# jianfenglihg/Unsupervised_depth_OpticalFlow_egomotion

Measured on AMD Instinct MI355X. Metric: frame-pairs/sec (832x256, geom mode), higher is better.
Workload: dtype f32; 1 GPU; train_step: mode=geom, 832x256, batch=4/GPU, num_scales=3, fwd+bwd+Adam; global_batch=4, parallelism=dp1, hw_queues=4, stream_priorities=auto

## Files before the change

include/dfe_hip.h:

```cpp
#ifndef DFE_HIP_H
#define DFE_HIP_H

#ifdef __cplusplus
extern "C" {
#endif

#define DFE_OK 0
#define DFE_ERR_NULL (-1)
#define DFE_ERR_DIMS (-2)
#define DFE_ERR_LAUNCH (-3)
#define DFE_ERR_UNSUPPORTED (-4)
#define DFE_ERR_WORKSPACE (-5)

#define DFE_MAX_SCALES 8
#define DFE_ABI_VERSION 3

int dfe_abi_version(void);
const char* dfe_error_string(int code);

int dfe_camera_floats(void);
int dfe_prepare_cameras(const float* pose, const float* K, float* cams, int B, int ndir, int nscale,
                        const float* downscale_host, void* stream);

int dfe_pose_vec2mat_fwd(const float* vec, float* T34, float* E, int n, void* stream);
int dfe_pose_vec2mat_bwd(const float* vec, const float* gT34, const float* gE, float* gvec, int n, void* stream);

int dfe_adam_chunk(void);
int dfe_adam_step(const void* table, const int* blockmap, int nblocks, double lr, double beta1, double beta2, double eps,
                  double bias_correction1, double bias_correction2, void* stream);
int dfe_adam_step_dev(const void* table, const int* blockmap, int nblocks, double lr, double beta1, double beta2, double eps,
                      double* step_count, float* coef, void* stream);

long dfe_scatter_ws_bytes(long n);

int dfe_warp_flow_fwd(const float* x, const float* flow, float* out, int B, int C, int H, int W, int use_mask,
                      int align_corners, void* stream);
int dfe_warp_flow_bwd(const float* x, const float* flow, const float* gout, float* gflow, float* gx, void* gx_ws, int B,
                      int C, int H, int W, int use_mask, int align_corners, void* stream);

int dfe_pose_partials_floats(int B, int H, int W);
int dfe_inverse_warp2_fwd(const float* img, const float* depth, const float* ref_depth, const float* cams,
                          float* out_img, float* out_valid, float* out_pdepth, float* out_cdepth, int B, int H, int W,
                          int align_corners, void* stream);
int dfe_inverse_warp2_bwd(const float* img, const float* depth, const float* ref_depth, const float* cams,
                          const float* g_img, const float* g_pdepth, const float* g_cdepth, float* g_depth,
                          float* g_refdepth, void* g_refdepth_ws, float* g_pose, float* partials, int B, int H, int W,
                          int align_corners, void* stream);

int dfe_rigid_flow_fwd(const float* depth, const float* cams, float* out, int B, int H, int W, void* stream);
int dfe_rigid_flow_bwd(const float* depth, const float* cams, const float* gout, float* g_depth, float* g_pose,
                       float* partials, int B, int H, int W, void* stream);

int dfe_occ_masks(const float* from_l, const float* tgt, const float* from_r, float* occ_bwd, float* occ_fwd,
                  float* valid_bwd, float* valid_fwd, int B, int H, int W, void* stream);
int dfe_texture_mask(const float* img, const float* warped, const float* source, float* out, int B, int H, int W,
                     void* stream);
int dfe_dynamic_mask(const float* flow, const float* rigid, float* mask, float* score, float alpha, float beta, int B,
                     int H, int W, void* stream);

int dfe_prepare_triplets(const unsigned char* in_u8, const unsigned char* flip, float* out, int B, int H0, int W0,
                         int H, int W, void* stream);

typedef struct {
  long long offset;
  int h0, w0;
  int xtab, ytab;
  int flip, pad;
} dfe_u8_desc;
// ... 68 lines not shown
                        void* stream);
int dfe_planeconv_wgrad(const float* gy, const float* x, float* gweight, float* ws, int B, int Ci, int Co, int H, int W,
                        void* stream);

long dfe_wino_weight_floats(int Ci, int Co);
long dfe_wino_scratch_floats(int B, int Ci, int Co, int H, int W, int P);
int dfe_wino_conv3x3(const float* x, const float* weight, float* y, long y_batch_stride, float* wbuf, long wbuf_floats, int B, int Ci,
                     int Co, int H, int W, int P, int transposed_weight, void* stream);
long dfe_wino_wgrad_floats(int B, int Ci, int Co, int H, int W, int P);
int dfe_wino_wgrad_tune(int tile, int blocks1, int blocks2, int chunk);
int dfe_wino_wgrad3x3(const float* x, long x_batch_stride, const float* gy, long gy_batch_stride, float* gweight, float* ws, int B,
                      int Ci, int Co, int H, int W, int P, void* stream);
int dfe_sconv_tune(int blocks, int rows);
long dfe_sconv_wgrad_floats(int B, int Ci, int Co, int H, int W, int K, int stride, int P);
int dfe_sconv_wgrad(const float* x, long x_batch_stride, const float* gy, long gy_batch_stride, float* gweight, float* ws, int B,
                    int Ci, int Co, int H, int W, int K, int stride, int P, void* stream);
int dfe_wino_conv3x3_dilated(const float* x, const float* weight, float* y, long y_batch_stride, float* wbuf, int B, int Ci, int Co,
                             int H, int W, int dilation, int transposed_weight, void* stream);
long dfe_wino_transform_blocks(int Ci, int Co);
int dfe_wino_transform_weights_multi(const long* table, const int* blockmap, int n_blocks, void* stream);
int dfe_wino_conv3x3_u(const float* x, const float* U, float* y, long y_batch_stride, float* part, long part_floats, int B, int Ci,
                       int Co, int H, int W, int P, int dilation, void* stream);
int dfe_wino_conv3x3_u_act(const float* x, const float* U, const float* bias, float slope, float* y, long y_batch_stride, float* y2,
                           long y2_batch_stride, float* part, long part_floats, int B, int Ci, int Co, int H, int W, int P,
                           int dilation, void* stream);

int dfe_conv1x1_small_supported(int B, int Ci, int Co, int H, int W);
int dfe_conv1x1_small_fwd(const float* x, const float* weight, const float* bias, float slope, float* y, int B, int Ci, int Co,
                          int H, int W, void* stream);
int dfe_conv1x1_small_bwd(const float* gy, const float* x, const float* weight, float* gx, float* gweight, int B, int Ci, int Co,
                          int H, int W, void* stream);

long dfe_bn_partials_floats(int G, int Bg, int C, int H, int W);
int dfe_bn_fwd(const float* x, const float* residual, const float* weight, const float* bias, float* running_mean,
               float* running_var, float* y, float* save_mean, float* save_invstd, float* partials, int G, int Bg, int C,
               int H, int W, float eps, float momentum, int relu, void* stream);
int dfe_bn_bwd(const float* x, const float* y, const float* gy, const float* weight, const float* save_mean,
               const float* save_invstd, float* gx, float* gres, float* gweight, float* gbias, float* partials,
               float* scratch_means, int G, int Bg, int C, int H, int W, int relu, void* stream);

long dfe_bias_act_partials_floats(int B, int C, int H, int W);
int dfe_bias_act_fwd(float* z, const float* bias, int B, int C, int H, int W, float slope, void* stream);
int dfe_bias_act_bwd(const float* y, const float* gy, long gy_batch_stride, float* gz, float* gbias, float* partials,
                     int B, int C, int H, int W, float slope, void* stream);

int dfe_bias_act_fwd2(const float* z, const float* bias, float* dst1, long dst1_batch_stride, float* dst2,
                      long dst2_batch_stride, int B, int C, int H, int W, float slope, void* stream);
int dfe_bias_act_bwd2(const float* y, long y_batch_stride, const float* g1, long g1_batch_stride, const float* g2,
                      long g2_batch_stride, float* gz, float* gbias, float* partials, int B, int C, int H, int W,
                      float slope, void* stream);
int dfe_bias_grad_final_multi(const float* const* partials, float* const* gbias, const int* C, int n, int B, int H, int W,
                              void* stream);

#define DFE_LOSS_DEPTH_PIXEL 0
#define DFE_LOSS_DEPTH_SMOOTH 1
#define DFE_LOSS_FLOW_PIXEL 2
#define DFE_LOSS_FLOW_SSIM 3
#define DFE_LOSS_FLOW_SMOOTH 4
#define DFE_LOSS_FLOW_CONSIS 5
#define DFE_LOSS_DEPTH_FLOW_CONSIS 6
#define DFE_LOSS_EPIPOLAR 7
#define DFE_LOSS_DEPTH_SSIM 8
#define DFE_LOSS_DEPTH_CONSIS 9
#define DFE_NUM_LOSSES 10
#define DFE_DEPTH_TERM_SSIM 1
#define DFE_DEPTH_TERM_CONSIS 2

#define DFE_MASK_VALID_BWD 0x01
#define DFE_MASK_VALID_FWD 0x02
#define DFE_MASK_OCC_BWD 0x04
#define DFE_MASK_OCC_FWD 0x08
#define DFE_MASK_DYNA_BWD 0x10
#define DFE_MASK_DYNA_FWD 0x20
#define DFE_MASK_TEX_BWD 0x40
#define DFE_MASK_TEX_FWD 0x80

typedef struct dfe_geom_args {
  int B, H, W;
  int num_scales;
  int align_corners;
  int mode;
  float alpha, beta;
  const float* img[3];
  const float* disp[3][DFE_MAX_SCALES];
  const float* flow[2][DFE_MAX_SCALES];
  const float* pose;
  const float* K;
  const float* K_inv;
  float* workspace;
  long workspace_floats;
  float* losses;
  const float* grad_losses;
  float* grad_disp[3][DFE_MAX_SCALES];
  float* grad_flow[2][DFE_MAX_SCALES];
  float* grad_pose;
  int depth_terms;
} dfe_geom_args;

long dfe_geom_workspace_floats(const dfe_geom_args* args);
long dfe_geom_maskpack_offset_bytes(const dfe_geom_args* args, int scale);
int dfe_geom_loss_fwd(const dfe_geom_args* args, void* stream);
int dfe_geom_loss_bwd(const dfe_geom_args* args, void* stream);

#define DFE_GEOM_FWD_SEGMENTS 7
#define DFE_GEOM_BWD_SEGMENTS 6
int dfe_geom_loss_fwd_profiled(const dfe_geom_args* args, void* stream, float* ms_host);
// ... 11 lines not shown
```

unsupervised_depth_opticalflow_egomotion_amd/_lib.py:

```python
from __future__ import annotations

import ctypes
import os
import re
import threading

import torch

_HERE = os.path.dirname(os.path.abspath(__file__))
LIB_PATH = os.environ.get("DFE_HIP_LIB") or os.path.join(_HERE, "libdfe_hip.so")
HEADER_PATH = os.path.join(os.path.dirname(_HERE), "include", "dfe_hip.h")

_lib = None
_lock = threading.Lock()

_P = ctypes.c_void_p
_I = ctypes.c_int

_SIGNATURES = {
    "dfe_abi_version": [],
    "dfe_error_string": [_I],
    "dfe_camera_floats": [],
    "dfe_prepare_cameras": [_P, _P, _P, _I, _I, _I, _P, _P],
    "dfe_pose_vec2mat_fwd": [_P, _P, _P, _I, _P],
    "dfe_pose_vec2mat_bwd": [_P, _P, _P, _P, _I, _P],
    "dfe_warp_flow_fwd": [_P, _P, _P, _I, _I, _I, _I, _I, _I, _P],
    "dfe_scatter_ws_bytes": [ctypes.c_long],
    "dfe_adam_chunk": [],
    "dfe_adam_step": [_P, _P, _I, ctypes.c_double, ctypes.c_double, ctypes.c_double, ctypes.c_double, ctypes.c_double, ctypes.c_double, _P],
    "dfe_adam_step_dev": [_P, _P, _I, ctypes.c_double, ctypes.c_double, ctypes.c_double, ctypes.c_double, _P, _P, _P],
    "dfe_warp_flow_bwd": [_P, _P, _P, _P, _P, _P, _I, _I, _I, _I, _I, _I, _P],
    "dfe_pose_partials_floats": [_I, _I, _I],
    "dfe_inverse_warp2_fwd": [_P, _P, _P, _P, _P, _P, _P, _P, _I, _I, _I, _I, _P],
    "dfe_inverse_warp2_bwd": [_P, _P, _P, _P, _P, _P, _P, _P, _P, _P, _P, _P, _I, _I, _I, _I, _P],
    "dfe_wgrad3x3_partials_floats": [_I, _I, _I, _I, _I],
    "dfe_wgrad3x3_fwd": [_P, _P, _P, _P, _I, _I, _I, _I, _I, _P],
    "dfe_wino_weight_floats": [_I, _I],
    "dfe_wino_conv3x3": [_P, _P, _P, ctypes.c_long, _P, ctypes.c_long, _I, _I, _I, _I, _I, _I, _I, _P],
    "dfe_wino_scratch_floats": [_I, _I, _I, _I, _I, _I],
    "dfe_wino_wgrad_floats": [_I, _I, _I, _I, _I, _I],
    "dfe_wino_wgrad_tune": [_I, _I, _I, _I],
    "dfe_sconv_tune": [_I, _I],
    "dfe_sconv_wgrad_floats": [_I, _I, _I, _I, _I, _I, _I, _I],
    "dfe_sconv_wgrad": [_P, ctypes.c_long, _P, ctypes.c_long, _P, _P, _I, _I, _I, _I, _I, _I, _I, _I, _P],
    "dfe_wino_wgrad3x3": [_P, ctypes.c_long, _P, ctypes.c_long, _P, _P, _I, _I, _I, _I, _I, _I, _P],
    "dfe_wino_conv3x3_dilated": [_P, _P, _P, ctypes.c_long, _P, _I, _I, _I, _I, _I, _I, _I, _P],
    "dfe_wino_transform_blocks": [_I, _I],
    "dfe_wino_transform_weights_multi": [_P, _P, _I, _P],
    "dfe_wino_conv3x3_u": [_P, _P, _P, ctypes.c_long, _P, ctypes.c_long, _I, _I, _I, _I, _I, _I, _I, _P],
    "dfe_wino_conv3x3_u_act": [_P, _P, _P, ctypes.c_float, _P, ctypes.c_long, _P, ctypes.c_long, _P, ctypes.c_long, _I, _I, _I, _I, _I, _I, _I, _P],
    "dfe_conv1x1_small_supported": [_I, _I, _I, _I, _I],
    "dfe_conv1x1_small_fwd": [_P, _P, _P, ctypes.c_float, _P, _I, _I, _I, _I, _I, _P],
    "dfe_conv1x1_small_bwd": [_P, _P, _P, _P, _P, _I, _I, _I, _I, _I, _P],
    "dfe_planeconv_supported": [_I, _I, _I, _I, _I],
    "dfe_planeconv_ws_floats": [_I, _I, _I, _I, _I],
    "dfe_planeconv_fwd": [_P, _P, _P, ctypes.c_float, _P, ctypes.c_long, _P, ctypes.c_long, _P, _I, _I, _I, _I, _I, _P],
    "dfe_planeconv_dgrad": [_P, _P, _P, _P, _I, _I, _I, _I, _I, _P],
    "dfe_planeconv_wgrad": [_P, _P, _P, _P, _I, _I, _I, _I, _I, _P],
    "dfe_disp_head_partials_floats": [_I, _I, _I, _I],
    "dfe_disp_head_fwd": [_P, _P, _P, _P, _I, _I, _I, _I, _P],
    "dfe_disp_head_bwd": [_P, _P, _P, _P, _P, _P, _P, _P, _I, _I, _I, _I, _P],
    "dfe_flow_head_partials_floats": [_I, _I, _I, _I],
    "dfe_flow_head_fwd": [_P, _P, _P, _P, _I, _I, _I, _I, _P],
    "dfe_flow_head_bwd": [_P, _P, _P, _P, _P, _P, _P, _I, _I, _I, _I, _P],
    "dfe_bn_partials_floats": [_I, _I, _I, _I, _I],
    "dfe_bn_fwd": [_P] * 10 + [_I] * 5 + [ctypes.c_float, ctypes.c_float, _I, _P],
    "dfe_bn_bwd": [_P] * 12 + [_I] * 6 + [_P],
    "dfe_bias_act_partials_floats": [_I, _I, _I, _I],
    "dfe_bias_act_fwd": [_P, _P, _I, _I, _I, _I, ctypes.c_float, _P],
    "dfe_bias_act_bwd": [_P, _P, ctypes.c_long, _P, _P, _P, _I, _I, _I, _I, ctypes.c_float, _P],
    "dfe_bias_act_fwd2": [_P, _P, _P, ctypes.c_long, _P, ctypes.c_long, _I, _I, _I, _I, ctypes.c_float, _P],
    "dfe_bias_act_bwd2": [_P, ctypes.c_long, _P, ctypes.c_long, _P, ctypes.c_long, _P, _P, _P, _I, _I, _I, _I, ctypes.c_float, _P],
    "dfe_bias_grad_final_multi": [_P, _P, _P, _I, _I, _I, _I, _P],
    "dfe_glue_partials_floats": [_I, _I, _I, _I],
    "dfe_elu_pad_fwd": [_P, _P, _P, _I, _I, _I, _I, _I, _P],
    "dfe_elu_pad_bwd": [_P, _P, _P, _P, _P, _P, _I, _I, _I, _I, _I, _P],
    "dfe_elu_up2_cat_pad_fwd": [_P, _P, _P, _P, _I, _I, _I, _I, _I, _P],
    "dfe_elu_up2_cat_pad_bwd": [_P, _P, _P, _P, _P, _P, _P, _I, _I, _I, _I, _I, _P],
    "dfe_rigid_flow_fwd": [_P, _P, _P, _I, _I, _I, _P],
    "dfe_rigid_flow_bwd": [_P, _P, _P, _P, _P, _P, _I, _I, _I, _P],
    "dfe_occ_masks": [_P] * 7 + [_I, _I, _I, _P],
    "dfe_texture_mask": [_P, _P, _P, _P, _I, _I, _I, _P],
    "dfe_dynamic_mask": [_P, _P, _P, _P, ctypes.c_float, ctypes.c_float, _I, _I, _I, _P],
    "dfe_exact_math_selftest": [_P, ctypes.c_ulonglong, _P],
    "dfe_prepare_triplets": [_P, _P, _P, _I, _I, _I, _I, _I, _P],
    "dfe_prepare_triplets_u8": [_P, _P, _P, _P, _P, _P, _I, _I, _I, _I, _I, _P],
    "dfe_forward_splat_ones": [_P, _P, _P, _I, _I, _I, _I, _P],
    "dfe_ssim_fwd": [_P, _P, _P, _I, _I, _I, _I, _P],
    "dfe_ssim_bwd": [_P, _P, _P, _P, _P, _I, _I, _I, _I, _P],
    "dfe_corr_fwd": [_P, _P, _P, _I, _I, _I, _I, _I, _P],
    "dfe_corr_bwd": [_P, _P, _P, _P, _P, _I, _I, _I, _I, _I, _P],
    "dfe_maxpool3x3s2_out": [_I],
    "dfe_maxpool3x3s2_fwd": [_P, _P, _P, _I, _I, _I, _P],
    "dfe_maxpool3x3s2_bwd": [_P, _P, _P, _I, _I, _I, _P],
    "dfe_pwc_level_channels": [_I],
    "dfe_pwc_level_fwd": [_P, _P, _P, _P, _P, _I, _I, _I, _I, _I, _P],
    "dfe_pwc_level_bwd": [_P, _P, _P, _P, _P, _P, _P, _P, _P, _P, _I, _I, _I, _I, _I, _P],
    "dfe_pwc_level_map_bytes": [_I, _I, _I],
    "dfe_pwc_level_fwd_map": [_P, _P, _P, _P, _P, _P, _I, _I, _I, _I, _I, _P],
    "dfe_pwc_level_bwd_map": [_P, _P, _P, _P, _P, _P, _P, _P, _P, _P, _I, _I, _I, _I, _I, _P],
    "dfe_resize": [_P, _P, _I, _I, _I, _I, _I, _I, _P],
    "dfe_resize_bilinear_fwd": [_P, _P, _I, _I, _I, _I, _I, ctypes.c_float, _I, _P],
    "dfe_resize_bilinear_bwd": [_P, _P, _I, _I, _I, _I, _I, ctypes.c_float, _I, _P],
    "dfe_geom_workspace_floats": [_P],
    "dfe_geom_maskpack_offset_bytes": [_P, _I],
    "dfe_geom_loss_fwd": [_P, _P],
    "dfe_geom_loss_bwd": [_P, _P],
    "dfe_geom_loss_fwd_profiled": [_P, _P, _P],
    "dfe_geom_loss_bwd_profiled": [_P, _P, _P],
    "dfe_geom_loss_fwd_timed": [_P, _P, _P],
    "dfe_geom_loss_bwd_timed": [_P, _P, _P],
    "dfe_geom_timed_collect": [_P, _P],
}
_RESTYPES = {"dfe_error_string": ctypes.c_char_p, "dfe_geom_workspace_floats": ctypes.c_long,
             "dfe_bias_act_partials_floats": ctypes.c_long, "dfe_glue_partials_floats": ctypes.c_long,
             "dfe_bn_partials_floats": ctypes.c_long, "dfe_disp_head_partials_floats": ctypes.c_long,
             "dfe_flow_head_partials_floats": ctypes.c_long, "dfe_pwc_level_map_bytes": ctypes.c_long,
             "dfe_wgrad3x3_partials_floats": ctypes.c_long, "dfe_planeconv_ws_floats": ctypes.c_long, "dfe_wino_weight_floats": ctypes.c_long, "dfe_wino_scratch_floats": ctypes.c_long, "dfe_wino_wgrad_floats": ctypes.c_long, "dfe_sconv_wgrad_floats": ctypes.c_long, "dfe_wino_transform_blocks": ctypes.c_long,
             "dfe_geom_maskpack_offset_bytes": ctypes.c_long, "dfe_scatter_ws_bytes": ctypes.c_long}


class DfeError(RuntimeError):
    pass


def header_symbols(path: str = HEADER_PATH):
    with open(path) as fh:
        text = re.sub(r"/\*.*?\*/", "", fh.read(), flags=re.S)
    return sorted(set(re.findall(r"\b(dfe_[a-z0-9_]+)\s*\(", text)))


def header_abi_version(path: str = HEADER_PATH) -> int:
    with open(path) as fh:
        return int(re.search(r"#define\s+DFE_ABI_VERSION\s+(\d+)", fh.read()).group(1))


def get_lib():
    global _lib
    if _lib is not None:
        return _lib
    with _lock:
        if _lib is None:
            if not os.path.exists(LIB_PATH):
                raise DfeError(
                    "libdfe_hip.so not found at %s: build it with `python -c 'import __graft_entry__ as g; "
                    "g.build()'` (hipcc --offload-arch=gfx950). There is no CPU fallback." % LIB_PATH)
            lib = ctypes.CDLL(LIB_PATH)
            for name in header_symbols():
                fn = getattr(lib, name)
                if name in _SIGNATURES:
                    fn.argtypes = _SIGNATURES[name]
                fn.restype = _RESTYPES.get(name, ctypes.c_int)
            if lib.dfe_abi_version() != header_abi_version():
                raise DfeError("libdfe_hip.so ABI version %d != include/dfe_hip.h's DFE_ABI_VERSION %d: a stale build; "
                               "rebuild with __graft_entry__.build()" % (lib.dfe_abi_version(), header_abi_version()))
            _lib = lib
    return _lib


def check(code: int, what: str = ""):
    if code != 0:
        msg = get_lib().dfe_error_string(code)
        raise DfeError("%s failed: %s (code %d)" % (what or "dfe call", msg.decode() if msg else "?", code))


def ptr(t, strided=False):
    if t is None:
        return None
    if not isinstance(t, torch.Tensor):
        raise DfeError("expected a torch.Tensor, got %r" % type(t))
    if not t.is_cuda:
        raise DfeError("the HIP loss stack only accepts tensors on a HIP device (got %s); there is no CPU "
# ... 21 lines not shown
```

unsupervised_depth_opticalflow_egomotion_amd/csrc/dfe_wgrad_sum.h:

```cpp
#pragma once
#include <hip/hip_runtime.h>

namespace dfe {

template <int SG>
__global__ void __launch_bounds__(32 * SG) k_wgrad_sum(const float* __restrict__ part, float* __restrict__ gw, int S, long n) {
  __shared__ float sm[SG][32];
  const int o = threadIdx.x & 31, g = threadIdx.x >> 5;
  const long idx = static_cast<long>(blockIdx.x) * 32 + o;
  const int per = (S + SG - 1) / SG, s0 = g * per, s1 = min(S, s0 + per);
  float s = 0.0f;
  if (idx < n)
    for (int k = s0; k < s1; ++k) s += part[k * n + idx];
  sm[g][o] = s;
  __syncthreads();
  if (g == 0 && idx < n) {
    float t = sm[0][o];
#pragma unroll
    for (int j = 1; j < SG; ++j) t += sm[j][o];
    gw[idx] = t;
  }
}

}
```

unsupervised_depth_opticalflow_egomotion_amd/csrc/ops_decoder.hip:

```cpp
#include "dfe_internal.h"
#include "dfe_device.h"
#include <hip/hip_runtime.h>
#include <cstdlib>

namespace dfe {

__device__ __forceinline__ float elu1(float v) { return v > 0.0f ? v : __expf(v) - 1.0f; }
__device__ __forceinline__ float elu1_grad(float v) { return v > 0.0f ? 1.0f : __expf(v); }
__device__ __forceinline__ int reflect1(int i, int n) { return i < 0 ? -i : (i >= n ? 2 * n - 2 - i : i); }

__device__ __forceinline__ void up2_tap(int d, int n, int& i0, int& i1, float& l0, float& l1) {
  const float s = fmaxf(0.5f * (static_cast<float>(d) + 0.5f) - 0.5f, 0.0f);
  i0 = static_cast<int>(s);
  i1 = min(i0 + 1, n - 1);
  l1 = s - static_cast<float>(i0);
  l0 = 1.0f - l1;
}

__device__ __forceinline__ float pad_adjoint(const float* __restrict__ gp, int y, int x, int H, int W) {
  const int Wp = W + 2;
  int ry[3], rx[3], ny = 1, nx = 1;
  ry[0] = y + 1; rx[0] = x + 1;
  if (y == 1) ry[ny++] = 0;
  if (y == H - 2) ry[ny++] = H + 1;
  if (x == 1) rx[nx++] = 0;
  if (x == W - 2) rx[nx++] = W + 1;
  float s = 0.0f;
  for (int a = 0; a < ny; ++a)
    for (int b = 0; b < nx; ++b) s += gp[static_cast<long>(ry[a]) * Wp + rx[b]];
  return s;
}

__global__ void __launch_bounds__(256) k_elu_pad_fwd(const float* __restrict__ x, const float* __restrict__ bias,
                                                     float* __restrict__ out, int C, int H, int W, int elu) {
  const unsigned e = blockIdx.x * blockDim.x + threadIdx.x;
  if (e >= static_cast<unsigned>((H + 2) * (W + 2))) return;
  const int oy = e / static_cast<unsigned>(W + 2), ox = e - oy * (W + 2);
  const long pl = plane_id();
  const float v = x[(pl * H + reflect1(oy - 1, H)) * W + reflect1(ox - 1, W)] + (bias ? bias[plane_id() % C] : 0.0f);
  out[(pl * (H + 2) + oy) * (W + 2) + ox] = elu ? elu1(v) : v;
}

__global__ void __launch_bounds__(256) k_elu_pad_bwd(const float* __restrict__ x, const float* __restrict__ bias,
                                                     const float* __restrict__ gp, float* __restrict__ gx,
                                                     float* __restrict__ part, int C, int H, int W, int elu) {
  __shared__ float red[4 * 4];
  const unsigned e = blockIdx.x * blockDim.x + threadIdx.x;
  float acc[1] = {0.0f};
  if (e < static_cast<unsigned>(H * W)) {
    const int iy = e / static_cast<unsigned>(W), ix = e - iy * W;
    const long pl = plane_id();
    float g = pad_adjoint(gp + pl * (H + 2) * (W + 2), iy, ix, H, W);
    const long o = (pl * H + iy) * W + ix;
    if (elu) g *= elu1_grad(x[o] + (bias ? bias[plane_id() % C] : 0.0f));
// ... 293 lines not shown
        const int xq = 2 * j0 - 1 + t;
        if (xq >= 0 && xq < W) tile[rs[k] * LW + t] = pad_adjoint(g, ys[k], xq, H, W);
      }
      if (cs[k] >= 0 && cs[k] < LW && t < LH) {
        const int y = 2 * i0 - 1 + t;
        if (y >= 0 && y < H) tile[t * LW + cs[k]] = pad_adjoint(g, y, xs[k], H, W);
      }
    }
  }
  __syncthreads();
  float wx[4] = {0.25f, 0.75f, 0.75f, 0.25f};
  if (!inner) up2_adjoint_weights(min(j, w - 1), w, wx);
  float f[2 * R + 2];
  const float* trow = tile + (2 * grp * R) * LW + 2 * jl;
#pragma unroll
  for (int rr = 0; rr < 2 * R + 2; ++rr) {
    const AF2 a = *reinterpret_cast<const AF2*>(trow + rr * LW), d = *reinterpret_cast<const AF2*>(trow + rr * LW + 2);
    if (inner) f[rr] = ((0.25f * a.a + 0.75f * a.b) + 0.75f * d.a) + 0.25f * d.b;
    else {
      float s = 0.0f;
      if (wx[0] != 0.0f) s += wx[0] * a.a;
      if (wx[1] != 0.0f) s += wx[1] * a.b;
      if (wx[2] != 0.0f) s += wx[2] * d.a;
      if (wx[3] != 0.0f) s += wx[3] * d.b;
      f[rr] = s;
    }
  }
  const float bv = bias ? bias[c] : 0.0f;
  float acc[1] = {0.0f};
#pragma unroll
  for (int q = 0; q < R; ++q) {
    const int i = i0 + grp * R + q;
    float total = 0.0f;
    if (inner) {
      total += 0.25f * f[2 * q]; total += 0.75f * f[2 * q + 1]; total += 0.75f * f[2 * q + 2]; total += 0.25f * f[2 * q + 3];
    } else {
      float wy[4];
      up2_adjoint_weights(min(i, h - 1), h, wy);
#pragma unroll
      for (int ky = 0; ky < 4; ++ky)
        if (wy[ky] != 0.0f) total += wy[ky] * f[2 * q + ky];
    }
    if (i < h && j < w) {
      const float v = total * elu1_grad(xv[q] + bv);
      gx[obase + static_cast<long>(i) * w + j] = v;
      acc[0] += v;
    }
  }
  if (part) block_sum<1>(acc, red, part + static_cast<long>(plane_id()) * gridDim.x + blockIdx.x);
}

__global__ void __launch_bounds__(64) k_glue_bias_final(const float* __restrict__ part, float* __restrict__ gbias,
                                                        int B, int C, int nblk) {
  const int c = blockIdx.x, lane = threadIdx.x;
  float s = 0.0f;
  for (int b = 0; b < B; ++b) {
    const float* p = part + (static_cast<long>(b) * C + c) * nblk;
    for (int k = lane; k < nblk; k += 64) s += p[k];
  }
  s = dpp_add<0xB1>(s); s = dpp_add<0x4E>(s); s = dpp_add<0x141>(s); s = dpp_add<0x140>(s);
  const float r0 = __int_as_float(__builtin_amdgcn_readlane(__float_as_int(s), 0));
  const float r1 = __int_as_float(__builtin_amdgcn_readlane(__float_as_int(s), 16));
  const float r2 = __int_as_float(__builtin_amdgcn_readlane(__float_as_int(s), 32));
  const float r3 = __int_as_float(__builtin_amdgcn_readlane(__float_as_int(s), 48));
  if (lane == 0) gbias[c] = (r0 + r1) + (r2 + r3);
}

__global__ void __launch_bounds__(256) k_cat_pad_bwd_skip(const float* __restrict__ gp, float* __restrict__ gskip,
                                                          int C1, int C2, int H, int W) {
  const unsigned e = blockIdx.x * blockDim.x + threadIdx.x;
  if (e >= static_cast<unsigned>(H * W)) return;
  const int iy = e / static_cast<unsigned>(W), ix = e - iy * W;
  const int b = plane_id() / C2, c = plane_id() - b * C2;
  const float* g = gp + (static_cast<long>(b) * (C1 + C2) + C1 + c) * (H + 2) * (W + 2);
  gskip[(static_cast<long>(plane_id()) * H + iy) * W + ix] = pad_adjoint(g, iy, ix, H, W);
}

}

#define DFE_LAUNCH_CHECK() do { if (hipGetLastError() != hipSuccess) return DFE_ERR_LAUNCH; } while (0)

using namespace dfe;

static inline bool grid_ok(long plane_elems, long batch, long channels) { return plane_elems < (1L << 31) && batch <= 65535 && channels <= 65535; }
static inline bool al8(const void* p) { return (reinterpret_cast<uintptr_t>(p) & 7) == 0; }
static inline bool al16(const void* p) { return (reinterpret_cast<uintptr_t>(p) & 15) == 0; }
static inline unsigned nblk(long n) { return static_cast<unsigned>((n + 255) / 256); }

extern "C" long dfe_glue_partials_floats(int B, int C, int H, int W) {
  if (B <= 0 || C <= 0 || H <= 0 || W <= 0) return 0;
  return static_cast<long>(B) * C * nblk(static_cast<long>(H) * W);
}

extern "C" int dfe_elu_pad_fwd(const float* x, const float* bias, float* out, int B, int C, int H, int W, int apply_elu,
                               void* stream) {
  if (!x || !out) return DFE_ERR_NULL;
  if (B <= 0 || C <= 0 || H < 2 || W < 2 || !grid_ok((H + 2L) * (W + 2L), B, C)) return DFE_ERR_DIMS;
  hipStream_t st = static_cast<hipStream_t>(stream);
  if (W % 2 == 0 && W >= 4 && al8(out)) k_elu_pad_fwd_pair<<<dim3(nblk((H + 2L) * ((W + 2L) / 2)), C, B), 256, 0, st>>>(x, bias, out, C, H, W, apply_elu);
  else k_elu_pad_fwd<<<dim3(nblk((H + 2L) * (W + 2L)), C, B), 256, 0, st>>>(x, bias, out, C, H, W, apply_elu);
  DFE_LAUNCH_CHECK();
  return DFE_OK;
}

extern "C" int dfe_elu_pad_bwd(const float* x, const float* bias, const float* gout, float* gx, float* gbias, float* partials,
                               int B, int C, int H, int W, int apply_elu, void* stream) {
  if (!gout || !gx || (apply_elu && !x) || (gbias && !partials)) return DFE_ERR_NULL;
  if (B <= 0 || C <= 0 || H < 2 || W < 2 || !grid_ok((H + 2L) * (W + 2L), B, C)) return DFE_ERR_DIMS;
  hipStream_t st = static_cast<hipStream_t>(stream);
  const bool pair = W % 2 == 0 && W >= 4 && al8(gx) && (!apply_elu || al8(x));
  const bool quad = W % 4 == 0 && W >= 8 && al16(gx) && (!apply_elu || al16(x));
  const unsigned nb = nblk(quad ? static_cast<long>(H) * (W / 4) : pair ? static_cast<long>(H) * (W / 2) : static_cast<long>(H) * W);
  if (quad) k_elu_pad_bwd_quad<<<dim3(nb, C, B), 256, 0, st>>>(x, bias, gout, gx, gbias ? partials : nullptr, C, H, W, apply_elu);
  else if (pair) k_elu_pad_bwd_pair<<<dim3(nb, C, B), 256, 0, st>>>(x, bias, gout, gx, gbias ? partials : nullptr, C, H, W, apply_elu);
  else k_elu_pad_bwd<<<dim3(nb, C, B), 256, 0, st>>>(x, bias, gout, gx, gbias ? partials : nullptr, C, H, W, apply_elu);
  DFE_LAUNCH_CHECK();
  if (gbias) {
    k_glue_bias_final<<<C, 64, 0, st>>>(partials, gbias, B, C, static_cast<int>(nb));
    DFE_LAUNCH_CHECK();
  }
  return DFE_OK;
}

extern "C" int dfe_elu_up2_cat_pad_fwd(const float* x, const float* bias, const float* skip, float* out, int B, int C1, int C2,
                                       int h, int w, void* stream) {
  if (!x || !out || (C2 > 0 && !skip)) return DFE_ERR_NULL;
  if (B <= 0 || C1 <= 0 || C2 < 0 || h < 1 || w < 1 || !grid_ok((2L * h + 2) * (2L * w + 2), B, C1 + C2)) return DFE_ERR_DIMS;
  hipStream_t st = static_cast<hipStream_t>(stream);
  if (w >= 2 && al8(out)) k_elu_up2_cat_pad_fwd_pair<<<dim3(nblk((2L * h + 2) * (w + 1L)), C1 + C2, B), 256, 0, st>>>(x, bias, skip, out, C1, C2, h, w);
  else k_elu_up2_cat_pad_fwd<<<dim3(nblk((2L * h + 2) * (2L * w + 2)), C1 + C2, B), 256, 0, st>>>(x, bias, skip, out, C1, C2, h, w);
  DFE_LAUNCH_CHECK();
  return DFE_OK;
}

extern "C" int dfe_elu_up2_cat_pad_bwd(const float* x, const float* bias, const float* gout, float* gx, float* gskip,
                                       float* gbias, float* partials, int B, int C1, int C2, int h, int w, void* stream) {
  if (!x || !gout || (!gx && !gskip) || (gbias && (!partials || !gx))) return DFE_ERR_NULL;
  if (B <= 0 || C1 <= 0 || C2 < 0 || h < 1 || w < 1 || !grid_ok((2L * h + 2) * (2L * w + 2), B, C1 + C2)) return DFE_ERR_DIMS;
  hipStream_t st = static_cast<hipStream_t>(stream);
  if (gx) {
    unsigned nb = nblk(static_cast<long>(h) * w);
    const int tw = w <= 32 ? 32 : 64;
    const int tiles_x = (w + tw - 1) / tw, tiles_y = (h + UT_H - 1) / UT_H;
    if (al8(gout) && static_cast<unsigned>(tiles_x * tiles_y) <= nb) {
      nb = static_cast<unsigned>(tiles_x * tiles_y);
      if (tw == 32) k_elu_up2_cat_pad_bwd_x_tile<32><<<dim3(nb, C1, B), 256, 0, st>>>(x, bias, gout, gx, gbias ? partials : nullptr, C1, C2, h, w, tiles_x);
      else k_elu_up2_cat_pad_bwd_x_tile<64><<<dim3(nb, C1, B), 256, 0, st>>>(x, bias, gout, gx, gbias ? partials : nullptr, C1, C2, h, w, tiles_x);
    } else {
      k_elu_up2_cat_pad_bwd_x<<<dim3(nb, C1, B), 256, 0, st>>>(x, bias, gout, gx, gbias ? partials : nullptr, C1, C2, h, w);
    }
    DFE_LAUNCH_CHECK();
    if (gbias) {
      k_glue_bias_final<<<C1, 64, 0, st>>>(partials, gbias, B, C1, static_cast<int>(nb));
      DFE_LAUNCH_CHECK();
    }
  }
  if (gskip && C2 > 0) {
    if (w % 2 == 0 && w >= 4 && al16(gskip)) k_cat_pad_bwd_skip_quad<<<dim3(nblk(1L * h * w), C2, B), 256, 0, st>>>(gout, gskip, C1, C2, 2 * h, 2 * w);
    else if (w >= 2 && al8(gskip)) k_cat_pad_bwd_skip_pair<<<dim3(nblk(2L * h * w), C2, B), 256, 0, st>>>(gout, gskip, C1, C2, 2 * h, 2 * w);
    else k_cat_pad_bwd_skip<<<dim3(nblk(4L * h * w), C2, B), 256, 0, st>>>(gout, gskip, C1, C2, 2 * h, 2 * w);
    DFE_LAUNCH_CHECK();
  }
  return DFE_OK;
}
```

unsupervised_depth_opticalflow_egomotion_amd/csrc/ops_disphead.hip:

```cpp
#include "dfe_internal.h"
#include "dfe_device.h"
#include <hip/hip_runtime.h>

namespace dfe {

constexpr int DH_COLS = 62;
constexpr int DH_ROWS = 16;
constexpr int DH_CI = 16;
constexpr int FH_CI = 8;


template <bool VPAD>
__device__ __forceinline__ float head_load(const float* __restrict__ pc, int r, int xx, int H, int W, bool ld) {
  if (VPAD) return (ld && r >= 1 && r <= H && xx >= 1 && xx <= W) ? pc[static_cast<long>(r - 1) * W + (xx - 1)] : 0.0f;
  return ld ? pc[static_cast<long>(r) * (W + 2) + xx] : 0.0f;
}

template <int CO, bool SIG, bool VPAD, int CI>
__global__ void __launch_bounds__(64) k_head_fwd(const float* __restrict__ p, const float* __restrict__ w,
                                                 const float* __restrict__ bias, float* __restrict__ out, int C, int H,
                                                 int W, int nstrips, int R) {
  const int lane = threadIdx.x, b = blockIdx.y;
  const int strip = blockIdx.x % nstrips, rb = blockIdx.x / nstrips;
  const int Hp = H + 2, Wp = W + 2;
  const int xx = strip * DH_COLS + lane;
  const bool ld = xx < Wp, st = lane < DH_COLS && xx < W;
  const int y0 = rb * R;
  const long plane = VPAD ? static_cast<long>(H) * W : static_cast<long>(Hp) * Wp;
  const float* pb = p + static_cast<long>(b) * C * plane;
  float acc[CO][3];
#pragma unroll
  for (int co = 0; co < CO; ++co) { acc[co][0] = 0.0f; acc[co][1] = 0.0f; acc[co][2] = 0.0f; }
  const int rend = min(y0 + R + 2, Hp);
  for (int r = y0; r < rend; ++r) {
    for (int c0 = 0; c0 < C; c0 += CI) {
      float v[CI];
#pragma unroll
      for (int k = 0; k < CI; ++k) v[k] = head_load<VPAD>(pb + (c0 + k) * plane, r, xx, H, W, ld);
#pragma unroll
      for (int k = 0; k < CI; ++k) {
        const float v1 = wave_shl1(v[k]), v2 = wave_shl1(v1);
#pragma unroll
        for (int co = 0; co < CO; ++co) {
          const float* wp = w + (static_cast<long>(co) * C + c0 + k) * 9;
          acc[co][0] = fmaf(wp[0], v[k], acc[co][0]); acc[co][0] = fmaf(wp[1], v1, acc[co][0]); acc[co][0] = fmaf(wp[2], v2, acc[co][0]);
          acc[co][1] = fmaf(wp[3], v[k], acc[co][1]); acc[co][1] = fmaf(wp[4], v1, acc[co][1]); acc[co][1] = fmaf(wp[5], v2, acc[co][1]);
          acc[co][2] = fmaf(wp[6], v[k], acc[co][2]); acc[co][2] = fmaf(wp[7], v1, acc[co][2]); acc[co][2] = fmaf(wp[8], v2, acc[co][2]);
        }
      }
    }
    const int yo = r - 2;
    if (st && yo >= y0 && yo < H) {
#pragma unroll
      for (int co = 0; co < CO; ++co) {
        const float z = acc[co][2] + (bias ? bias[co] : 0.0f);
        out[((static_cast<long>(b) * CO + co) * H + yo) * W + xx] = SIG ? 1.0f / (1.0f + __expf(-z)) : z;
      }
    }
#pragma unroll
    for (int co = 0; co < CO; ++co) { acc[co][2] = acc[co][1]; acc[co][1] = acc[co][0]; acc[co][0] = 0.0f; }
  }
}
// ... 25 lines not shown
  for (int rr = 0; rr < FP_R + 2; ++rr) {
    const int r = y0 + rr;
    if (r < Hp) {
      float v[CI];
#pragma unroll
      for (int k = 0; k < CI; ++k) v[k] = head_load<VPAD>(pb + k * plane, r, xx, H, W, ld);
#pragma unroll
      for (int k = 0; k < CI; ++k) {
        const float v1 = wave_shl1(v[k]), v2 = wave_shl1(v1);
#pragma unroll
        for (int co = 0; co < CO; ++co) {
          const float* wp = w + (static_cast<long>(co) * C + c0 + k) * 9;
          acc[co][0] = fmaf(wp[0], v[k], acc[co][0]); acc[co][0] = fmaf(wp[1], v1, acc[co][0]); acc[co][0] = fmaf(wp[2], v2, acc[co][0]);
          acc[co][1] = fmaf(wp[3], v[k], acc[co][1]); acc[co][1] = fmaf(wp[4], v1, acc[co][1]); acc[co][1] = fmaf(wp[5], v2, acc[co][1]);
          acc[co][2] = fmaf(wp[6], v[k], acc[co][2]); acc[co][2] = fmaf(wp[7], v1, acc[co][2]); acc[co][2] = fmaf(wp[8], v2, acc[co][2]);
        }
      }
    }
    if (rr >= 2) {
#pragma unroll
      for (int co = 0; co < CO; ++co) res[rr - 2][co] = acc[co][2];
    }
#pragma unroll
    for (int co = 0; co < CO; ++co) { acc[co][2] = acc[co][1]; acc[co][1] = acc[co][0]; acc[co][0] = 0.0f; }
  }
#pragma unroll
  for (int q = 0; q < FP_R; ++q)
#pragma unroll
    for (int co = 0; co < CO; ++co) red[((wv * FP_R + q) * CO + co) * 64 + lane] = res[q][co];
  __syncthreads();
  if (wv < FP_R) {
    const int yo = y0 + wv;
    if (st && yo < H) {
#pragma unroll
      for (int co = 0; co < CO; ++co) {
        float z = red[((0 * FP_R + wv) * CO + co) * 64 + lane];
        for (int k = 1; k < nwv; ++k) z += red[((k * FP_R + wv) * CO + co) * 64 + lane];
        z += bias ? bias[co] : 0.0f;
        out[((static_cast<long>(b) * CO + co) * H + yo) * W + xx] = SIG ? 1.0f / (1.0f + __expf(-z)) : z;
      }
    }
  }
}

template <bool SIG>
__device__ __forceinline__ float dh_grad(const float* __restrict__ gout, const float* __restrict__ out, int y, int x, int H, int W) {
  if (y < 0 || y >= H || x < 0 || x >= W) return 0.0f;
  const long o = static_cast<long>(y) * W + x;
  if (!SIG) return gout[o];
  const float d = out[o];
  return gout[o] * (d * (1.0f - d));
}

__device__ __forceinline__ float wave_total(float v) {
  v = dpp_add<0xB1>(v); v = dpp_add<0x4E>(v); v = dpp_add<0x141>(v); v = dpp_add<0x140>(v);
  const float r0s = __int_as_float(__builtin_amdgcn_readlane(__float_as_int(v), 0));
  const float r1s = __int_as_float(__builtin_amdgcn_readlane(__float_as_int(v), 16));
  const float r2s = __int_as_float(__builtin_amdgcn_readlane(__float_as_int(v), 32));
  const float r3s = __int_as_float(__builtin_amdgcn_readlane(__float_as_int(v), 48));
  return (r0s + r1s) + (r2s + r3s);
}

template <int CO, bool SIG, bool VPAD, int CI>
__global__ void __launch_bounds__(64) k_head_bwd(const float* __restrict__ p, const float* __restrict__ w,
                                                 const float* __restrict__ out, const float* __restrict__ gout,
                                                 float* __restrict__ gp, float* __restrict__ part, int C, int H, int W,
                                                 int nstrips) {
  constexpr int NACC = CI * CO * 9 + CO;
  const int lane = threadIdx.x, b = blockIdx.y, c0 = blockIdx.z * CI;
  const int strip = blockIdx.x % nstrips, rb = blockIdx.x / nstrips;
  const int Hp = H + 2, Wp = W + 2;
  const int xx = strip * DH_COLS + lane - 2;
  const bool own = lane >= 2 && xx < Wp;
  const int r0 = rb * DH_ROWS, rend = min(r0 + DH_ROWS, Hp);
  const long oplane = static_cast<long>(H) * W;
  const long plane = VPAD ? oplane : static_cast<long>(Hp) * Wp;
  const float* pb = p + (static_cast<long>(b) * C + c0) * plane;
  float* gb_ = gp + (static_cast<long>(b) * C + c0) * plane;
  float acc[CI][CO][9];
#pragma unroll
  for (int k = 0; k < CI; ++k)
#pragma unroll
    for (int co = 0; co < CO; ++co)
#pragma unroll
      for (int t = 0; t < 9; ++t) acc[k][co][t] = 0.0f;
  float accb[CO];
  float G[CO][9];
#pragma unroll
  for (int co = 0; co < CO; ++co) {
    const float* go = gout + (static_cast<long>(b) * CO + co) * oplane;
    const float* oo = SIG ? out + (static_cast<long>(b) * CO + co) * oplane : nullptr;
    accb[co] = 0.0f;
    G[co][3] = dh_grad<SIG>(go, oo, r0 - 1, xx, H, W); G[co][6] = dh_grad<SIG>(go, oo, r0 - 2, xx, H, W);
    G[co][4] = wave_shr1(G[co][3]); G[co][5] = wave_shr1(G[co][4]); G[co][7] = wave_shr1(G[co][6]); G[co][8] = wave_shr1(G[co][7]);
  }
  float pn1[CI], pn2[CI];
#pragma unroll
  for (int k = 0; k < CI; ++k) {
    pn1[k] = head_load<VPAD>(pb + k * plane, r0, xx, H, W, own);
    pn2[k] = head_load<VPAD>(pb + k * plane, r0 + 1 < rend ? r0 + 1 : r0, xx, H, W, own);
  }
  for (int r = r0; r < rend; ++r) {
#pragma unroll
    for (int co = 0; co < CO; ++co) {
      const float* go = gout + (static_cast<long>(b) * CO + co) * oplane;
      const float* oo = SIG ? out + (static_cast<long>(b) * CO + co) * oplane : nullptr;
      G[co][0] = dh_grad<SIG>(go, oo, r, xx, H, W);
      G[co][1] = wave_shr1(G[co][0]); G[co][2] = wave_shr1(G[co][1]);
    }
    float pv[CI];
    const int rn = r + 2 < rend ? r + 2 : r0;
#pragma unroll
    for (int k = 0; k < CI; ++k) { pv[k] = pn1[k]; pn1[k] = pn2[k]; pn2[k] = head_load<VPAD>(pb + k * plane, rn, xx, H, W, own); }
    const bool wr = VPAD ? (own && r >= 1 && r <= H && xx >= 1 && xx <= W) : own;
#pragma unroll
    for (int k = 0; k < CI; ++k) {
      float s = 0.0f;
#pragma unroll
      for (int co = 0; co < CO; ++co) {
        const float* wp = w + (static_cast<long>(co) * C + c0 + k) * 9;
        if (co == 0) s = wp[0] * G[co][0]; else s = fmaf(wp[0], G[co][0], s);
#pragma unroll
        for (int t = 1; t < 9; ++t) s = fmaf(wp[t], G[co][t], s);
#pragma unroll
        for (int t = 0; t < 9; ++t) acc[k][co][t] = fmaf(pv[k], G[co][t], acc[k][co][t]);
      }
      if (wr) {
        if (VPAD) gb_[k * plane + static_cast<long>(r - 1) * W + (xx - 1)] = s;
        else gb_[k * plane + static_cast<long>(r) * Wp + xx] = s;
      }
    }
#pragma unroll
    for (int co = 0; co < CO; ++co) {
      if (own) accb[co] += G[co][0];
      G[co][6] = G[co][3]; G[co][7] = G[co][4]; G[co][8] = G[co][5]; G[co][3] = G[co][0]; G[co][4] = G[co][1]; G[co][5] = G[co][2];
    }
  }
  float* po = part + ((static_cast<long>(b) * gridDim.x + blockIdx.x) * gridDim.z + blockIdx.z) * NACC;
#pragma unroll
  for (int k = 0; k < CI; ++k)
#pragma unroll
    for (int co = 0; co < CO; ++co)
#pragma unroll
      for (int t = 0; t < 9; ++t) {
        const float v = wave_total(acc[k][co][t]);
        if (lane == 0) po[(k * CO + co) * 9 + t] = v;
      }
#pragma unroll
  for (int co = 0; co < CO; ++co) {
    const float v = wave_total(accb[co]);
    if (lane == 0) po[CI * CO * 9 + co] = v;
  }
}

template <int CO, int CI>
__global__ void __launch_bounds__(64) k_head_final(const float* __restrict__ part, float* __restrict__ gw,
                                                   float* __restrict__ gb, int C, int nunits, int nz) {
  constexpr int NACC = CI * CO * 9 + CO;
  const int o = blockIdx.x, lane = threadIdx.x;
  const bool isb = o >= CO * C * 9;
  int z = 0, idx;
  if (isb) idx = CI * CO * 9 + (o - CO * C * 9);
  else {
    const int co = o / (C * 9), c = (o - co * C * 9) / 9, t = o % 9;
    z = c / CI;
    idx = ((c - z * CI) * CO + co) * 9 + t;
  }
  float s = 0.0f;
  for (int u = lane; u < nunits; u += 64) s += part[(static_cast<long>(u) * nz + z) * NACC + idx];
  const float tot = wave_total(s);
  if (lane == 0) {
    if (isb) { if (gb) gb[o - CO * C * 9] = tot; } else if (gw) gw[o] = tot;
  }
}

}

#define DFE_LAUNCH_CHECK() do { if (hipGetLastError() != hipSuccess) return DFE_ERR_LAUNCH; } while (0)
using namespace dfe;

static int dh_dims(int B, int C, int H, int W, int ci = DH_CI) {
  if (B <= 0 || C <= 0 || H < 1 || W < 1 || B > 65535) return DFE_ERR_DIMS;
  if (C % ci != 0 || C / ci > 65535) return DFE_ERR_UNSUPPORTED;
  if ((static_cast<long>(H) + 2) * (W + 2) * C >= (1L << 31)) return DFE_ERR_DIMS;
  return DFE_OK;
}
static inline int dh_strips(int cols) { return (cols + DH_COLS - 1) / DH_COLS; }
static inline int dh_rowblocks(int rows) { return (rows + DH_ROWS - 1) / DH_ROWS; }

extern "C" long dfe_disp_head_partials_floats(int B, int C, int H, int W) {
  if (dh_dims(B, C, H, W) != DFE_OK) return 0;
  return static_cast<long>(B) * dh_strips(W + 2) * dh_rowblocks(H + 2) * (C / DH_CI) * (DH_CI * 9 + 1);
}

extern "C" int dfe_disp_head_fwd(const float* p, const float* weight, const float* bias, float* out, int B, int C, int H, int W,
                                 void* stream) {
  if (!p || !weight || !out) return DFE_ERR_NULL;
  const int rc = dh_dims(B, C, H, W);
  if (rc != DFE_OK) return rc;
  const int ns = dh_strips(W);
  int R = DH_ROWS;
  while (R > 2 && static_cast<long>(B) * ns * ((H + R - 1) / R) < 2048) R /= 2;
  k_head_fwd<1, true, false, DH_CI><<<dim3(ns * ((H + R - 1) / R), B), 64, 0, static_cast<hipStream_t>(stream)>>>(p, weight, bias, out, C, H, W, ns, R);
  DFE_LAUNCH_CHECK();
  return DFE_OK;
}

extern "C" int dfe_disp_head_bwd(const float* p, const float* weight, const float* out, const float* gout, float* gp,
                                 float* gweight, float* gbias, float* partials, int B, int C, int H, int W, void* stream) {
  if (!p || !weight || !out || !gout || !gp || !partials) return DFE_ERR_NULL;
  const int rc = dh_dims(B, C, H, W);
  if (rc != DFE_OK) return rc;
  hipStream_t st = static_cast<hipStream_t>(stream);
  const int ns = dh_strips(W + 2), nrb = dh_rowblocks(H + 2), nz = C / DH_CI;
  k_head_bwd<1, true, false, DH_CI><<<dim3(ns * nrb, B, nz), 64, 0, st>>>(p, weight, out, gout, gp, partials, C, H, W, ns);
  DFE_LAUNCH_CHECK();
  if (gweight || gbias) {
    k_head_final<1, DH_CI><<<C * 9 + 1, 64, 0, st>>>(partials, gweight, gbias, C, B * ns * nrb, nz);
    DFE_LAUNCH_CHECK();
  }
  return DFE_OK;
}

extern "C" long dfe_flow_head_partials_floats(int B, int C, int H, int W) {
  if (dh_dims(B, C, H, W, FH_CI) != DFE_OK) return 0;
  return static_cast<long>(B) * dh_strips(W + 2) * dh_rowblocks(H + 2) * (C / FH_CI) * (FH_CI * 2 * 9 + 2);
}

extern "C" int dfe_flow_head_fwd(const float* x, const float* weight, const float* bias, float* out, int B, int C, int H, int W,
                                 void* stream) {
  if (!x || !weight || !out) return DFE_ERR_NULL;
  const int rc = dh_dims(B, C, H, W, FH_CI);
  if (rc != DFE_OK) return rc;
  const int ns = dh_strips(W), nwv = C / FH_CI;
  if (nwv >= FP_R && nwv <= 16) {
    const size_t lds = sizeof(float) * nwv * FP_R * 2 * 64;
    k_head_fwd_par<2, false, true, FH_CI><<<dim3(ns * ((H + FP_R - 1) / FP_R), B), 64 * nwv, lds, static_cast<hipStream_t>(stream)>>>(x, weight, bias, out, C, H, W, ns);
  } else {
    int R = DH_ROWS;
    while (R > 2 && static_cast<long>(B) * ns * ((H + R - 1) / R) < 2048) R /= 2;
    k_head_fwd<2, false, true, FH_CI><<<dim3(ns * ((H + R - 1) / R), B), 64, 0, static_cast<hipStream_t>(stream)>>>(x, weight, bias, out, C, H, W, ns, R);
  }
  DFE_LAUNCH_CHECK();
  return DFE_OK;
}

extern "C" int dfe_flow_head_bwd(const float* x, const float* weight, const float* gout, float* gx, float* gweight, float* gbias,
                                 float* partials, int B, int C, int H, int W, void* stream) {
  if (!x || !weight || !gout || !gx || !partials) return DFE_ERR_NULL;
  const int rc = dh_dims(B, C, H, W, FH_CI);
  if (rc != DFE_OK) return rc;
  hipStream_t st = static_cast<hipStream_t>(stream);
  const int ns = dh_strips(W + 2), nrb = dh_rowblocks(H + 2), nz = C / FH_CI;
  k_head_bwd<2, false, true, FH_CI><<<dim3(ns * nrb, B, nz), 64, 0, st>>>(x, weight, nullptr, gout, gx, partials, C, H, W, ns);
  DFE_LAUNCH_CHECK();
  if (gweight || gbias) {
    k_head_final<2, FH_CI><<<2 * C * 9 + 2, 64, 0, st>>>(partials, gweight, gbias, C, B * ns * nrb, nz);
    DFE_LAUNCH_CHECK();
  }
  return DFE_OK;
}
```

unsupervised_depth_opticalflow_egomotion_amd/csrc/ops_epilogue.hip:

```cpp
#include "dfe_internal.h"
#include "dfe_device.h"
#include <hip/hip_runtime.h>

namespace dfe {

constexpr int EP_BLOCK = 256;
constexpr int EP_PER_THREAD = 8;
constexpr int EP_CHUNK = EP_BLOCK * EP_PER_THREAD;

template <bool VEC>
__global__ void __launch_bounds__(EP_BLOCK) k_bias_act_fwd(float* __restrict__ z, const float* __restrict__ bias,
                                                           int C, int HW, float slope) {
  const int c = plane_id() % C;
  const float bv = bias ? bias[c] : 0.0f;
  float* p = z + static_cast<long>(plane_id()) * HW;
  const int base = blockIdx.x * EP_CHUNK;
  if (VEC) {
#pragma unroll
    for (int k = 0; k < EP_PER_THREAD / 4; ++k) {
      const int e = base + (k * EP_BLOCK + threadIdx.x) * 4;
      if (e < HW) {
        float4 v = *reinterpret_cast<float4*>(p + e);
        v.x += bv; v.y += bv; v.z += bv; v.w += bv;
        v.x = v.x > 0.0f ? v.x : v.x * slope; v.y = v.y > 0.0f ? v.y : v.y * slope;
        v.z = v.z > 0.0f ? v.z : v.z * slope; v.w = v.w > 0.0f ? v.w : v.w * slope;
        *reinterpret_cast<float4*>(p + e) = v;
      }
    }
  } else {
#pragma unroll
    for (int k = 0; k < EP_PER_THREAD; ++k) {
      const int e = base + k * EP_BLOCK + threadIdx.x;
      if (e < HW) { const float v = p[e] + bv; p[e] = v > 0.0f ? v : v * slope; }
    }
  }
}

template <bool VEC>
__global__ void __launch_bounds__(EP_BLOCK) k_bias_act_bwd(const float* __restrict__ y, const float* __restrict__ gy,
                                                           float* __restrict__ gz, float* __restrict__ part,
                                                           int HW, long gy_plane_stride, long gy_batch_stride, int C,
                                                           float slope) {
  __shared__ float red[4 * (EP_BLOCK / 64)];
  const int b = plane_id() / C, c = plane_id() - b * C;
  const float* py = y + static_cast<long>(plane_id()) * HW;
  const float* pg = gy + b * gy_batch_stride + c * gy_plane_stride;
  float* pz = gz + static_cast<long>(plane_id()) * HW;
  const int base = blockIdx.x * EP_CHUNK;
  float acc[1] = {0.0f};
  if (VEC) {
#pragma unroll
    for (int k = 0; k < EP_PER_THREAD / 4; ++k) {
      const int e = base + (k * EP_BLOCK + threadIdx.x) * 4;
      if (e < HW) {
        const float4 yv = *reinterpret_cast<const float4*>(py + e);
        float4 g = *reinterpret_cast<const float4*>(pg + e);
        g.x = yv.x > 0.0f ? g.x : g.x * slope; g.y = yv.y > 0.0f ? g.y : g.y * slope;
        g.z = yv.z > 0.0f ? g.z : g.z * slope; g.w = yv.w > 0.0f ? g.w : g.w * slope;
        *reinterpret_cast<float4*>(pz + e) = g;
        acc[0] += (g.x + g.y) + (g.z + g.w);
      }
    }
  } else {
#pragma unroll
    for (int k = 0; k < EP_PER_THREAD; ++k) {
      const int e = base + k * EP_BLOCK + threadIdx.x;
      if (e < HW) { const float g = py[e] > 0.0f ? pg[e] : pg[e] * slope; pz[e] = g; acc[0] += g; }
    }
  }
  if (part) block_sum<1>(acc, red, part + static_cast<long>(plane_id()) * gridDim.x + blockIdx.x);
}

__global__ void __launch_bounds__(64) k_bias_grad_final(const float* __restrict__ part, float* __restrict__ gbias,
                                                        int B, int C, int nchunk) {
  const int c = blockIdx.x, lane = threadIdx.x;
  float s = 0.0f;
  for (int b = 0; b < B; ++b) {
    const float* p = part + (static_cast<long>(b) * C + c) * nchunk;
    for (int k = lane; k < nchunk; k += 64) s += p[k];
  }
  s = dpp_add<0xB1>(s); s = dpp_add<0x4E>(s); s = dpp_add<0x141>(s); s = dpp_add<0x140>(s);
  const float r0 = __int_as_float(__builtin_amdgcn_readlane(__float_as_int(s), 0));
  const float r1 = __int_as_float(__builtin_amdgcn_readlane(__float_as_int(s), 16));
  const float r2 = __int_as_float(__builtin_amdgcn_readlane(__float_as_int(s), 32));
  const float r3 = __int_as_float(__builtin_amdgcn_readlane(__float_as_int(s), 48));
  if (lane == 0) gbias[c] = (r0 + r1) + (r2 + r3);
}

constexpr int EP_MAXL = 8;
struct BiasFinalJobs { const float* part[EP_MAXL]; float* gbias[EP_MAXL]; int C[EP_MAXL]; int nchunk[EP_MAXL]; int first[EP_MAXL + 1]; int n; };

__global__ void __launch_bounds__(64) k_bias_grad_final_multi(BiasFinalJobs j, int B) {
  int l = 0;
  while (l + 1 < j.n && static_cast<int>(blockIdx.x) >= j.first[l + 1]) ++l;
  const int c = blockIdx.x - j.first[l], lane = threadIdx.x, C = j.C[l], nchunk = j.nchunk[l];
  float s = 0.0f;
  for (int b = 0; b < B; ++b) {
    const float* p = j.part[l] + (static_cast<long>(b) * C + c) * nchunk;
    for (int k = lane; k < nchunk; k += 64) s += p[k];
  }
  s = dpp_add<0xB1>(s); s = dpp_add<0x4E>(s); s = dpp_add<0x141>(s); s = dpp_add<0x140>(s);
  const float r0 = __int_as_float(__builtin_amdgcn_readlane(__float_as_int(s), 0));
  const float r1 = __int_as_float(__builtin_amdgcn_readlane(__float_as_int(s), 16));
  const float r2 = __int_as_float(__builtin_amdgcn_readlane(__float_as_int(s), 32));
  const float r3 = __int_as_float(__builtin_amdgcn_readlane(__float_as_int(s), 48));
  if (lane == 0) j.gbias[l][c] = (r0 + r1) + (r2 + r3);
}

template <bool VEC>
__global__ void __launch_bounds__(EP_BLOCK) k_bias_act_fwd2(const float* z, const float* __restrict__ bias,
                                                            float* d1, long d1_bs, float* d2,
                                                            long d2_bs, int C, int HW, float slope) {
  const int b = plane_id() / C, c = plane_id() - b * C;
  const float bv = bias ? bias[c] : 0.0f;
  const float* p = z + static_cast<long>(plane_id()) * HW;
  float* o1 = d1 + b * d1_bs + static_cast<long>(c) * HW;
  float* o2 = d2 ? d2 + b * d2_bs + static_cast<long>(c) * HW : nullptr;
  const int base = blockIdx.x * EP_CHUNK;
  if (VEC) {
#pragma unroll
    for (int k = 0; k < EP_PER_THREAD / 4; ++k) {
      const int e = base + (k * EP_BLOCK + threadIdx.x) * 4;
      if (e < HW) {
        float4 v = *reinterpret_cast<const float4*>(p + e);
        v.x += bv; v.y += bv; v.z += bv; v.w += bv;
        v.x = v.x > 0.0f ? v.x : v.x * slope; v.y = v.y > 0.0f ? v.y : v.y * slope;
        v.z = v.z > 0.0f ? v.z : v.z * slope; v.w = v.w > 0.0f ? v.w : v.w * slope;
        *reinterpret_cast<float4*>(o1 + e) = v;
        if (o2) *reinterpret_cast<float4*>(o2 + e) = v;
      }
    }
  } else {
#pragma unroll
    for (int k = 0; k < EP_PER_THREAD; ++k) {
      const int e = base + k * EP_BLOCK + threadIdx.x;
      if (e < HW) { float v = p[e] + bv; v = v > 0.0f ? v : v * slope; o1[e] = v; if (o2) o2[e] = v; }
    }
  }
}

template <bool VEC>
__global__ void __launch_bounds__(EP_BLOCK) k_bias_act_bwd2(const float* y, long y_bs, const float* g1,
                                                            long g1_bs, const float* g2, long g2_bs,
                                                            float* gz, float* __restrict__ part, int C, int HW,
                                                            float slope) {
  __shared__ float red[4 * (EP_BLOCK / 64)];
  const int b = plane_id() / C, c = plane_id() - b * C;
  const long co = static_cast<long>(c) * HW;
  const float* py = y + b * y_bs + co;
  const float* pa = g1 + b * g1_bs + co;
  const float* pb = g2 ? g2 + b * g2_bs + co : nullptr;
  float* pz = gz + static_cast<long>(plane_id()) * HW;
  const int base = blockIdx.x * EP_CHUNK;
  float acc[1] = {0.0f};
  if (VEC) {
#pragma unroll
    for (int k = 0; k < EP_PER_THREAD / 4; ++k) {
      const int e = base + (k * EP_BLOCK + threadIdx.x) * 4;
      if (e < HW) {
// ... 11 lines not shown
    for (int k = 0; k < EP_PER_THREAD; ++k) {
      const int e = base + k * EP_BLOCK + threadIdx.x;
      if (e < HW) {
        float g = pa[e];
        if (pb) g += pb[e];
        g = py[e] > 0.0f ? g : g * slope;
        pz[e] = g; acc[0] += g;
      }
    }
  }
  if (part) block_sum<1>(acc, red, part + static_cast<long>(plane_id()) * gridDim.x + blockIdx.x);
}

}

#define DFE_LAUNCH_CHECK() do { if (hipGetLastError() != hipSuccess) return DFE_ERR_LAUNCH; } while (0)
using namespace dfe;

static inline bool aligned16(const void* p) { return (reinterpret_cast<uintptr_t>(p) & 15) == 0; }

extern "C" long dfe_bias_act_partials_floats(int B, int C, int H, int W) {
  if (B <= 0 || C <= 0 || H <= 0 || W <= 0) return 0;
  const long hw = static_cast<long>(H) * W;
  return static_cast<long>(B) * C * ((hw + EP_CHUNK - 1) / EP_CHUNK);
}

extern "C" int dfe_bias_act_fwd(float* z, const float* bias, int B, int C, int H, int W, float slope, void* stream) {
  if (!z) return DFE_ERR_NULL;
  const long hw = static_cast<long>(H) * W;
  if (B <= 0 || C <= 0 || H <= 0 || W <= 0 || hw >= (1L << 31) || C > 65535 || B > 65535) return DFE_ERR_DIMS;
  const dim3 g(static_cast<unsigned>((hw + EP_CHUNK - 1) / EP_CHUNK), C, B);
  hipStream_t st = static_cast<hipStream_t>(stream);
  if (hw % 4 == 0 && aligned16(z)) k_bias_act_fwd<true><<<g, EP_BLOCK, 0, st>>>(z, bias, C, static_cast<int>(hw), slope);
  else k_bias_act_fwd<false><<<g, EP_BLOCK, 0, st>>>(z, bias, C, static_cast<int>(hw), slope);
  DFE_LAUNCH_CHECK();
  return DFE_OK;
}

extern "C" int dfe_bias_act_bwd(const float* y, const float* gy, long gy_batch_stride, float* gz, float* gbias,
                                float* partials, int B, int C, int H, int W, float slope, void* stream) {
  if (!y || !gy || !gz || (gbias && !partials)) return DFE_ERR_NULL;
  const long hw = static_cast<long>(H) * W;
  if (B <= 0 || C <= 0 || H <= 0 || W <= 0 || hw >= (1L << 31) || C > 65535 || B > 65535) return DFE_ERR_DIMS;
  if (gy_batch_stride < static_cast<long>(C) * hw) return DFE_ERR_DIMS;
  const int nchunk = static_cast<int>((hw + EP_CHUNK - 1) / EP_CHUNK);
  const dim3 g(nchunk, C, B);
  hipStream_t st = static_cast<hipStream_t>(stream);
  float* part = partials;
  const bool vec = hw % 4 == 0 && aligned16(y) && aligned16(gy) && aligned16(gz) && gy_batch_stride % 4 == 0;
  if (vec) k_bias_act_bwd<true><<<g, EP_BLOCK, 0, st>>>(y, gy, gz, part, static_cast<int>(hw), hw, gy_batch_stride, C, slope);
  else k_bias_act_bwd<false><<<g, EP_BLOCK, 0, st>>>(y, gy, gz, part, static_cast<int>(hw), hw, gy_batch_stride, C, slope);
  DFE_LAUNCH_CHECK();
  if (gbias) {
    k_bias_grad_final<<<C, 64, 0, st>>>(partials, gbias, B, C, nchunk);
    DFE_LAUNCH_CHECK();
  }
  return DFE_OK;
}

extern "C" int dfe_bias_act_fwd2(const float* z, const float* bias, float* dst1, long dst1_batch_stride, float* dst2,
                                 long dst2_batch_stride, int B, int C, int H, int W, float slope, void* stream) {
  if (!z || !dst1) return DFE_ERR_NULL;
  const long hw = static_cast<long>(H) * W;
  if (B <= 0 || C <= 0 || H <= 0 || W <= 0 || hw >= (1L << 31) || C > 65535 || B > 65535) return DFE_ERR_DIMS;
  if (dst1_batch_stride < C * hw || (dst2 && dst2_batch_stride < C * hw)) return DFE_ERR_DIMS;
  const dim3 g(static_cast<unsigned>((hw + EP_CHUNK - 1) / EP_CHUNK), C, B);
  hipStream_t st = static_cast<hipStream_t>(stream);
  const bool vec = hw % 4 == 0 && aligned16(z) && aligned16(dst1) && dst1_batch_stride % 4 == 0 &&
                   (!dst2 || (aligned16(dst2) && dst2_batch_stride % 4 == 0));
  if (vec) k_bias_act_fwd2<true><<<g, EP_BLOCK, 0, st>>>(z, bias, dst1, dst1_batch_stride, dst2, dst2_batch_stride, C, static_cast<int>(hw), slope);
  else k_bias_act_fwd2<false><<<g, EP_BLOCK, 0, st>>>(z, bias, dst1, dst1_batch_stride, dst2, dst2_batch_stride, C, static_cast<int>(hw), slope);
  DFE_LAUNCH_CHECK();
  return DFE_OK;
}

extern "C" int dfe_bias_act_bwd2(const float* y, long y_batch_stride, const float* g1, long g1_batch_stride, const float* g2,
                                 long g2_batch_stride, float* gz, float* gbias, float* partials, int B, int C, int H, int W,
                                 float slope, void* stream) {
  if (!y || !g1 || !gz || (gbias && !partials)) return DFE_ERR_NULL;
  const long hw = static_cast<long>(H) * W;
  if (B <= 0 || C <= 0 || H <= 0 || W <= 0 || hw >= (1L << 31) || C > 65535 || B > 65535) return DFE_ERR_DIMS;
  if (y_batch_stride < C * hw || g1_batch_stride < C * hw || (g2 && g2_batch_stride < C * hw)) return DFE_ERR_DIMS;
  const int nchunk = static_cast<int>((hw + EP_CHUNK - 1) / EP_CHUNK);
  const dim3 g(nchunk, C, B);
  hipStream_t st = static_cast<hipStream_t>(stream);
  float* part = partials;
  const bool vec = hw % 4 == 0 && aligned16(y) && aligned16(g1) && aligned16(gz) && y_batch_stride % 4 == 0 &&
                   g1_batch_stride % 4 == 0 && (!g2 || (aligned16(g2) && g2_batch_stride % 4 == 0));
  if (vec) k_bias_act_bwd2<true><<<g, EP_BLOCK, 0, st>>>(y, y_batch_stride, g1, g1_batch_stride, g2, g2_batch_stride, gz, part, C, static_cast<int>(hw), slope);
  else k_bias_act_bwd2<false><<<g, EP_BLOCK, 0, st>>>(y, y_batch_stride, g1, g1_batch_stride, g2, g2_batch_stride, gz, part, C, static_cast<int>(hw), slope);
  DFE_LAUNCH_CHECK();
  if (gbias) {
    k_bias_grad_final<<<C, 64, 0, st>>>(partials, gbias, B, C, nchunk);
    DFE_LAUNCH_CHECK();
  }
  return DFE_OK;
}

extern "C" int dfe_bias_grad_final_multi(const float* const* partials, float* const* gbias, const int* C, int n, int B, int H, int W,
                                         void* stream) {
  if (!partials || !gbias || !C) return DFE_ERR_NULL;
  const long hw = static_cast<long>(H) * W;
  if (n <= 0 || n > EP_MAXL || B <= 0 || H <= 0 || W <= 0 || hw >= (1L << 31)) return DFE_ERR_DIMS;
  BiasFinalJobs j;
  j.n = n; j.first[0] = 0;
  for (int l = 0; l < n; ++l) {
    if (!partials[l] || !gbias[l]) return DFE_ERR_NULL;
    if (C[l] <= 0 || C[l] > 65535) return DFE_ERR_DIMS;
    j.part[l] = partials[l]; j.gbias[l] = gbias[l]; j.C[l] = C[l];
    j.nchunk[l] = static_cast<int>((hw + EP_CHUNK - 1) / EP_CHUNK);
    j.first[l + 1] = j.first[l] + C[l];
  }
  k_bias_grad_final_multi<<<j.first[n], 64, 0, static_cast<hipStream_t>(stream)>>>(j, B);
  DFE_LAUNCH_CHECK();
  return DFE_OK;
}
```

unsupervised_depth_opticalflow_egomotion_amd/csrc/ops_planeconv.hip:

```cpp
#include "dfe_internal.h"
#include <hip/hip_runtime.h>
#include <algorithm>
#include <cstdlib>

namespace dfe {

typedef float f32x4 __attribute__((ext_vector_type(4)));

constexpr int PC_CC = 16;
constexpr int PC_MT = 64;
constexpr int PC_KW = PC_CC * 9;
constexpr int PC_XT_MAX = 18;
constexpr int PW_U = 8;

__device__ __forceinline__ int fdiv(int idx, float inv) { return static_cast<int>((static_cast<float>(idx) + 0.5f) * inv); }

template <int NSUB, bool DGRAD, int XT>
__global__ void __launch_bounds__(256) k_planeconv(const float* __restrict__ x, const float* __restrict__ w, float* __restrict__ part,
                                                   int B, int Ck, int N, int H, int W, int KS, int cps, int RB, int XP, int KP,
                                                   float inv_wp) {
  extern __shared__ float lds[];
  constexpr int NT = 16 * NSUB, WT = NT * PC_KW / 256;
  float* xs = lds;
  float* wl = lds + PC_CC * XP;
  const int tid = threadIdx.x, lane = tid & 63, wv = tid >> 6, m = lane & 15, kq = lane >> 4;
  const int HW = H * W, Wp = W + 2;
  const int m0 = blockIdx.x * PC_MT, n0 = blockIdx.y * NT;
  const int b = blockIdx.z / KS, ks = blockIdx.z - b * KS;
  const int cbeg = ks * cps, cend = min(Ck, cbeg + cps);
  const int r0 = m0 / W;
  const int p = min(m0 + 16 * wv + m, HW - 1);
  const int py = p / W, px = p - py * W;
  const int abase = kq * XP + (py - r0) * Wp + px;
  const int bbase = m * KP + kq * 9;
  f32x4 acc[NSUB][2];
#pragma unroll
  for (int s = 0; s < NSUB; ++s) { acc[s][0] = f32x4{0.0f, 0.0f, 0.0f, 0.0f}; acc[s][1] = f32x4{0.0f, 0.0f, 0.0f, 0.0f}; }
  const int rbwp = RB * Wp;
  const int sc = tid >> 4, l16 = tid & 15;
  int xoff[XT];
#pragma unroll
  for (int i = 0; i < XT; ++i) {
    const int rem = l16 + 16 * i;
    const int r = fdiv(rem, inv_wp), col = rem - r * Wp;
    const int gy = r0 - 1 + r, gx = col - 1;
    xoff[i] = (rem < rbwp && gy >= 0 && gy < H && gx >= 0 && gx < W) ? gy * W + gx : -1;
  }
  const unsigned xbase = static_cast<unsigned>(b) * Ck * HW;
  float xv[XT], wr[WT];
  auto fetch = [&](int c0) {
    const int nc = min(PC_CC, cend - c0);
    const unsigned cb = xbase + static_cast<unsigned>(c0 + min(sc, nc - 1)) * HW;
#pragma unroll
// ... 26 lines not shown
        for (int i = 0; i < 9; ++i)
          wl[(sc + 16 * q) * KP + l16 + 16 * i] = (okn && l16 + 16 * i < nc * 9) ? wr[q * 9 + i] : 0.0f;
      }
    } else {
#pragma unroll
      for (int i = 0; i < WT; ++i) {
        const int r = l16 + 16 * i, n = r / 9, t = r - n * 9;
        wl[n * KP + sc * 9 + 8 - t] = (sc < nc && n0 + n < N) ? wr[i] : 0.0f;
      }
    }
  };
  if (cbeg < cend) fetch(cbeg);
  for (int c0 = cbeg; c0 < cend; c0 += PC_CC) {
    const int nc = min(PC_CC, cend - c0);
    stage(c0);
    __syncthreads();
    if (c0 + PC_CC < cend) fetch(c0 + PC_CC);
#pragma unroll
    for (int cq = 0; cq < PC_CC / 4; ++cq) {
      if (cq * 4 < nc) {
        const float* xa = xs + abase + cq * 4 * XP;
        const float* wb = wl + bbase + cq * 36;
#pragma unroll
        for (int t = 0; t < 9; ++t) {
          const float a = xa[(t / 3) * Wp + (t % 3)];
#pragma unroll
          for (int s = 0; s < NSUB; ++s)
            acc[s][t & 1] = __builtin_amdgcn_mfma_f32_16x16x4f32(a, wb[s * 16 * KP + t], acc[s][t & 1], 0, 0, 0);
        }
      }
    }
    __syncthreads();
  }
  float* po = part + (static_cast<long>(ks) * B + b) * N * HW;
#pragma unroll
  for (int s = 0; s < NSUB; ++s) {
    const int n = n0 + 16 * s + m;
    if (n < N) {
#pragma unroll
      for (int r = 0; r < 4; ++r) {
        const int pp = m0 + 16 * wv + 4 * kq + r;
        if (pp < HW) po[static_cast<long>(n) * HW + pp] = acc[s][0][r] + acc[s][1][r];
      }
    }
  }
}

__global__ void __launch_bounds__(256) k_planeconv_finish(const float* __restrict__ part, const float* __restrict__ bias,
                                                          float* __restrict__ d1, long bs1, float* __restrict__ d2, long bs2,
                                                          int total, int NHW, int HW, int KS, float slope, float inv_nhw,
                                                          float inv_hw) {
  const int idx = blockIdx.x * 256 + threadIdx.x;
  if (idx >= total) return;
  float s = part[idx];
#pragma unroll 4
  for (int k = 1; k < KS; ++k) s += part[static_cast<long>(k) * total + idx];
  int b = fdiv(idx, inv_nhw);
  int r = idx - b * NHW;
  if (bias) s += bias[fdiv(r, inv_hw)];
  s = s > 0.0f ? s : s * slope;
  d1[b * bs1 + r] = s;
  if (d2) d2[b * bs2 + r] = s;
}

__global__ void __launch_bounds__(256) k_planeconv_wgrad(const float* __restrict__ gy, const float* __restrict__ x,
                                                         float* __restrict__ part, int Ci, int Co, int H, int W, int RS, int nband,
                                                         int Q4, int GP, int XE, int XP, float inv_q4, float inv_xe, float inv_wp) {
  extern __shared__ float lds[];
  float* gs = lds;
  float* xs = lds + 32 * GP;
  const int tid = threadIdx.x, lane = tid & 63, wv = tid >> 6, m = lane & 15, kq = lane >> 4;
  const int HW = H * W, Wp = W + 2;
  const int b = blockIdx.x / nband, band = blockIdx.x - b * nband;
  const int ci0 = blockIdx.y * 32, co0 = blockIdx.z * 32;
  const int y0 = band * RS, y1 = min(H, y0 + RS), Q = (y1 - y0) * Wp;
  const float* gb = gy + static_cast<long>(b) * Co * HW;
  const float* xb = x + static_cast<long>(b) * Ci * HW;
  auto gsite = [&](int idx, long& src, int& dst) -> bool {
    const int c = fdiv(idx, inv_q4), q = idx - c * Q4;
    const int yy = fdiv(q, inv_wp), xx = q - yy * Wp;
    const bool ok = co0 + c < Co && q < Q && xx < W;
    src = ok ? static_cast<long>(co0 + c) * HW + (y0 + yy) * W + xx : 0L;
    dst = c * GP + q;
    return ok;
  };
  auto xsite = [&](int idx, long& src, int& dst) -> bool {
    const int c = fdiv(idx, inv_xe), e = idx - c * XE;
    const int r = fdiv(e, inv_wp), col = e - r * Wp;
    const int yy = y0 - 1 + r, xx = col - 1;
    const bool ok = ci0 + c < Ci && yy >= 0 && yy < H && xx >= 0 && xx < W;
    src = ok ? static_cast<long>(ci0 + c) * HW + yy * W + xx : 0L;
    dst = c * XP + e;
    return ok;
  };
  const int EG = 32 * Q4, EX = 32 * XE;
  for (int base = tid; base < EG; base += 256 * PW_U) {
    float v[PW_U];
#pragma unroll
    for (int u = 0; u < PW_U; ++u) {
      long src; int dst;
      gsite(min(base + u * 256, EG - 1), src, dst);
      v[u] = gb[src];
    }
#pragma unroll
    for (int u = 0; u < PW_U; ++u) {
      long src; int dst;
      const bool ok = gsite(min(base + u * 256, EG - 1), src, dst);
      if (base + u * 256 < EG) gs[dst] = ok ? v[u] : 0.0f;
    }
// ... 171 lines not shown

extern "C" int dfe_planeconv_supported(int B, int Ci, int Co, int H, int W) {
  if (pc_dims(B, Ci, Co, H, W) != DFE_OK) return 0;
  return static_cast<long>(B) * Co * H * W < (1L << 20) && static_cast<long>(B) * Ci * H * W < (1L << 20) &&
         static_cast<long>(Co) * Ci * 9 < (1L << 20);
}

extern "C" long dfe_planeconv_ws_floats(int B, int Ci, int Co, int H, int W) {
  if (!dfe_planeconv_supported(B, Ci, Co, H, W)) return 0;
  const long HW = static_cast<long>(H) * W;
  const long f = pc_cfg(B, Ci, Co, H, W).KS * static_cast<long>(B) * Co * HW;
  const long d = pc_cfg(B, Co, Ci, H, W).KS * static_cast<long>(B) * Ci * HW;
  const long wg = pw_cfg(B, H, W).units * Co * Ci * 9;
  return std::max(f, std::max(d, wg));
}

extern "C" int dfe_planeconv_fwd(const float* x, const float* weight, const float* bias, float slope, float* dst1,
                                 long dst1_batch_stride, float* dst2, long dst2_batch_stride, float* ws, int B, int Ci, int Co,
                                 int H, int W, void* stream) {
  if (!x || !weight || !dst1 || !ws) return DFE_ERR_NULL;
  const int rc = pc_dims(B, Ci, Co, H, W);
  if (rc != DFE_OK) return rc;
  if (!dfe_planeconv_supported(B, Ci, Co, H, W)) return DFE_ERR_UNSUPPORTED;
  const long chw = static_cast<long>(Co) * H * W;
  if (dst1_batch_stride < chw || (dst2 && dst2_batch_stride < chw)) return DFE_ERR_DIMS;
  return pc_run(false, x, weight, bias, slope, dst1, dst1_batch_stride, dst2, dst2_batch_stride, ws, B, Ci, Co, H, W,
                static_cast<hipStream_t>(stream));
}

extern "C" int dfe_planeconv_dgrad(const float* gy, const float* weight, float* gx, float* ws, int B, int Ci, int Co, int H, int W,
                                   void* stream) {
  if (!gy || !weight || !gx || !ws) return DFE_ERR_NULL;
  const int rc = pc_dims(B, Ci, Co, H, W);
  if (rc != DFE_OK) return rc;
  if (!dfe_planeconv_supported(B, Ci, Co, H, W)) return DFE_ERR_UNSUPPORTED;
  return pc_run(true, gy, weight, nullptr, 1.0f, gx, static_cast<long>(Ci) * H * W, nullptr, 0, ws, B, Co, Ci, H, W,
                static_cast<hipStream_t>(stream));
}

extern "C" int dfe_planeconv_wgrad(const float* gy, const float* x, float* gweight, float* ws, int B, int Ci, int Co, int H, int W,
                                   void* stream) {
  if (!gy || !x || !gweight || !ws) return DFE_ERR_NULL;
  const int rc = pc_dims(B, Ci, Co, H, W);
  if (rc != DFE_OK) return rc;
  if (!dfe_planeconv_supported(B, Ci, Co, H, W)) return DFE_ERR_UNSUPPORTED;
  hipStream_t st = static_cast<hipStream_t>(stream);
  const PwCfg g = pw_cfg(B, H, W);
  const dim3 grid(static_cast<unsigned>(g.units), (Ci + 31) / 32, (Co + 31) / 32);
  k_planeconv_wgrad<<<grid, 256, g.lds, st>>>(gy, x, ws, Ci, Co, H, W, g.RS, g.nband, g.Q4, g.GP, g.XE, g.XP,
                                              1.0f / static_cast<float>(g.Q4), 1.0f / static_cast<float>(g.XE),
                                              1.0f / static_cast<float>(W + 2));
  DFE_LAUNCH_CHECK();
  const int total = Co * Ci * 9;
  k_planeconv_finish<<<(total + 255) / 256, 256, 0, st>>>(ws, nullptr, gweight, 0, nullptr, 0, total, total, total,
                                                          static_cast<int>(g.units), 1.0f, 1.0f / static_cast<float>(total),
                                                          1.0f / static_cast<float>(total));
  DFE_LAUNCH_CHECK();
  return DFE_OK;
}

static int c1_dims(int B, int Ci, int Co, int H, int W) {
  if (B <= 0 || Ci <= 0 || Co <= 0 || H <= 0 || W <= 0) return DFE_ERR_DIMS;
  if (static_cast<long>(H) * W > 256 || static_cast<long>(B) * H * W > 4096 || Ci > 4096 || Co > 4096) return DFE_ERR_UNSUPPORTED;
  return DFE_OK;
}

extern "C" int dfe_conv1x1_small_supported(int B, int Ci, int Co, int H, int W) { return c1_dims(B, Ci, Co, H, W) == DFE_OK; }

extern "C" int dfe_conv1x1_small_fwd(const float* x, const float* weight, const float* bias, float slope, float* y, int B, int Ci,
                                     int Co, int H, int W, void* stream) {
  if (!x || !weight || !y) return DFE_ERR_NULL;
  const int rc = c1_dims(B, Ci, Co, H, W);
  if (rc != DFE_OK) return rc;
  const int total = B * Co * H * W;
  k_conv1x1_small<false><<<(total + 255) / 256, 256, 0, static_cast<hipStream_t>(stream)>>>(x, weight, bias, y, Ci, Co, H * W, total, slope);
  DFE_LAUNCH_CHECK();
  return DFE_OK;
}

extern "C" int dfe_conv1x1_small_bwd(const float* gy, const float* x, const float* weight, float* gx, float* gweight, int B, int Ci,
                                     int Co, int H, int W, void* stream) {
  if (!gy || !x || !weight) return DFE_ERR_NULL;
  const int rc = c1_dims(B, Ci, Co, H, W);
  if (rc != DFE_OK) return rc;
  hipStream_t st = static_cast<hipStream_t>(stream);
  if (gx) {
    const int total = B * Ci * H * W;
    k_conv1x1_small<true><<<(total + 255) / 256, 256, 0, st>>>(gy, weight, nullptr, gx, Co, Ci, H * W, total, 1.0f);
    DFE_LAUNCH_CHECK();
  }
  if (gweight) {
    k_conv1x1_small_wgrad<<<(Co * Ci + 255) / 256, 256, 0, st>>>(gy, x, gweight, B, Ci, Co, H * W);
    DFE_LAUNCH_CHECK();
  }
  return DFE_OK;
}
```

unsupervised_depth_opticalflow_egomotion_amd/csrc/ops_sconv.hip:

```cpp
#include "dfe_internal.h"
#include "dfe_device.h"
#include "dfe_wgrad_sum.h"
#include <hip/hip_runtime.h>
#include <algorithm>
#include <cstdlib>

namespace dfe {

typedef float sc_f32x4 __attribute__((ext_vector_type(4)));
typedef float sc_f32x2 __attribute__((ext_vector_type(2)));
struct __attribute__((packed, aligned(4))) ScQuadU { float a, b, c, d; };

struct ScWg {
  long xbs, gbs;
  int Ci, Co, H, W, Ho, Wo, KH, KW, S, D, P, flat;
  int TH, TW;
  int RI, NSLOT, QW;
  int XRS, XCS, GCS;
  int DX;
  int CIB, COB;
  int XCH, GCH;
  int cpr, rpi, nchunks, cps, ncit, ntb;
};

template <int MT, int NT, int WM, int WN, int XSH, int NXL, int GSH, int NGL>
__global__ void __launch_bounds__(256, (NT <= 7 && NXL <= 9) ? 3 : 2)
k_sconv_wgrad(const float* __restrict__ x, const float* __restrict__ gy, float* __restrict__ part, const ScWg g) {
  extern __shared__ float lds[];
  const int tid = threadIdx.x, lane = tid & 63, wv = tid >> 6, i = lane & 15, kq = lane >> 4;
  const int wm = wv / WN, wn = wv % WN;
  const unsigned lid = xcd_swizzle(blockIdx.x, gridDim.x);
  const int tb = static_cast<int>(lid % static_cast<unsigned>(g.ntb)), split = static_cast<int>(lid / static_cast<unsigned>(g.ntb));
  const int cob0 = (tb / g.ncit) * g.COB, cib0 = (tb % g.ncit) * g.CIB;
  const int c_beg = split * g.cps, c_end = min(g.nchunks, c_beg + g.cps);
  const int KK = g.KH * g.KW, HW = g.H * g.W, gHW = g.Ho * g.Wo;
  const int XTOT = g.XCH * g.XCS;

  int boff[NT], oidx[NT], aoff[MT];
  bool any_col = false;
#pragma unroll
  for (int j = 0; j < NT; ++j) {
    const int tile = wn * NT + j;
    int ci_l, t;
    bool ok;
    if (g.flat) { const int col = tile * 16 + i; ci_l = col / KK; t = col - ci_l * KK; ok = ci_l < g.CIB; }
    else { t = tile % KK; ci_l = (tile / KK) * 16 + i; ok = ci_l < g.CIB; }
    ok = ok && cib0 + ci_l < g.Ci;
    const int ky = t / g.KW, kx = t - ky * g.KW, dk = g.D * kx + g.DX;
    const int o = ci_l * g.XCS + g.D * ky * g.XRS + (g.S == 2 ? (dk & 1) * g.QW + (dk >> 1) : dk) + kq;
    boff[j] = ok ? o : kq;
    oidx[j] = ok ? (cib0 + ci_l) * KK + t : -1;
    any_col = any_col || ok;
  }
#pragma unroll
  for (int mt = 0; mt < MT; ++mt) aoff[mt] = XTOT + ((wm * MT + mt) * 16 + i) * g.GCS + kq;
// ... 238 lines not shown
  const int ncot = (Co + g.COB - 1) / g.COB;
  g.ncit = (Ci + g.CIB - 1) / g.CIB;
  g.ntb = ncot * g.ncit;
  const int target = g_sc_blocks > 0 ? g_sc_blocks : ((c == 1 || c == 2) ? 768 : 512);
  long Sp = (target + g.ntb / 2) / g.ntb;
  Sp = std::max(1L, std::min<long>(Sp, g.nchunks));
  g.cps = static_cast<int>((g.nchunks + Sp - 1) / Sp);
  *nsplit = (g.nchunks + g.cps - 1) / g.cps;
  *out = g; *cfg = c;
  return true;
}

template <int MT, int NT, int WM, int WN, int XSH, int NXL, int GSH, int NGL>
void sc_wg_launch(const ScWg& g, int nsplit, const float* x, const float* gy, float* ws, hipStream_t st) {
  const size_t lds_bytes = sizeof(float) * (static_cast<size_t>(g.XCH) * g.XCS + static_cast<size_t>(g.GCH) * g.GCS + 16);
  auto kern = k_sconv_wgrad<MT, NT, WM, WN, XSH, NXL, GSH, NGL>;
  static bool attr_set = false;
  if (!attr_set) { (void)hipFuncSetAttribute(reinterpret_cast<const void*>(kern), hipFuncAttributeMaxDynamicSharedMemorySize, 80 * 1024); attr_set = true; }
  kern<<<static_cast<unsigned>(g.ntb) * nsplit, 256, lds_bytes, st>>>(x, gy, ws, g);
}
}

extern "C" int dfe_sconv_tune(int blocks, int rows) {
  if (blocks >= 0) g_sc_blocks = blocks;
  if (rows >= 0) g_sc_th = rows;
  return DFE_OK;
}

extern "C" long dfe_sconv_wgrad_floats(int B, int Ci, int Co, int H, int W, int K, int stride, int P) {
  ScWg g; int cfg, ns;
  if (!sc_wg_plan(B, Ci, Co, H, W, K, stride, P, &g, &cfg, &ns)) return 0;
  return static_cast<long>(ns) * Co * Ci * K * K;
}

extern "C" int dfe_sconv_wgrad(const float* x, long x_batch_stride, const float* gy, long gy_batch_stride, float* gweight, float* ws, int B,
                               int Ci, int Co, int H, int W, int K, int stride, int P, void* stream) {
  if (!x || !gy || !gweight || !ws) return DFE_ERR_NULL;
  if (B <= 0 || Ci <= 0 || Co <= 0 || H <= 0 || W <= 0) return DFE_ERR_DIMS;
  ScWg g; int cfg, ns;
  if (!sc_wg_plan(B, Ci, Co, H, W, K, stride, P, &g, &cfg, &ns)) return DFE_ERR_UNSUPPORTED;
  const long gplane = static_cast<long>(g.Ho) * g.Wo;
  if (x_batch_stride < static_cast<long>(Ci) * H * W || gy_batch_stride < Co * gplane) return DFE_ERR_DIMS;
  if (static_cast<long>(Ci) * H * W >= (1L << 30) || Co * gplane >= (1L << 30) || static_cast<long>(Co) * Ci * K * K >= (1L << 30)) return DFE_ERR_DIMS;
  g.xbs = x_batch_stride; g.gbs = gy_batch_stride;
  hipStream_t st = static_cast<hipStream_t>(stream);
  switch (cfg) {
    case 0: sc_wg_launch<1, 9, 4, 1, 7, 8, 4, 4>(g, ns, x, gy, ws, st); break;
    case 1: sc_wg_launch<2, 5, 2, 2, 8, 3, 4, 4>(g, ns, x, gy, ws, st); break;
    case 2: sc_wg_launch<1, 7, 1, 4, 8, 9, 4, 1>(g, ns, x, gy, ws, st); break;
    default: sc_wg_launch<2, 7, 1, 4, 8, 16, 4, 2>(g, ns, x, gy, ws, st); break;
  }
  DFE_LAUNCH_CHECK();
  const long n = static_cast<long>(Co) * Ci * K * K;
  if (ns > 64) k_wgrad_sum<32><<<static_cast<unsigned>((n + 31) / 32), 1024, 0, st>>>(ws, gweight, ns, n);
  else k_wgrad_sum<8><<<static_cast<unsigned>((n + 31) / 32), 256, 0, st>>>(ws, gweight, ns, n);
  DFE_LAUNCH_CHECK();
  return DFE_OK;
}
```

unsupervised_depth_opticalflow_egomotion_amd/csrc/ops_wgrad.hip:

```cpp
#include "dfe_internal.h"
#include <hip/hip_runtime.h>

namespace dfe {

typedef float f32x4 __attribute__((ext_vector_type(4)));
struct __attribute__((packed, aligned(8))) F2 { float a, b; };

template <int NCO, int NCI>
__global__ void __launch_bounds__(64) k_wgrad3x3_thin(const float* __restrict__ p, const float* __restrict__ gy,
                                                      float* __restrict__ part, int Ci, int Co, int H, int W, int R, int nrg,
                                                      int nseg) {
  const int lane = threadIdx.x, m = lane & 15, kq = lane >> 4;
  const int seg = blockIdx.x % nseg, br = blockIdx.x / nseg;
  const int b = br / nrg, rg = br - b * nrg;
  const int ci0 = blockIdx.y * 16 * NCI, co0 = blockIdx.z * 16 * NCO;
  const int Hp = H + 2, Wp = W + 2;
  const int y0 = rg * R, y1 = min(y0 + R, H);
  const int nch = W / 16, cps = (nch + nseg - 1) / nseg;
  const int xa = seg * cps * 16, xb = min((seg + 1) * cps, nch) * 16;
  const float* ga = gy + (static_cast<long>(b) * Co + co0 + m) * H * W + 4 * kq;
  const float* pa = p + (static_cast<long>(b) * Ci + ci0 + m) * Hp * Wp + 4 * kq;
  const long gtile = 16L * H * W, ptile = 16L * Hp * Wp;
  f32x4 acc[NCO][NCI][9];
#pragma unroll
  for (int o = 0; o < NCO; ++o)
#pragma unroll
    for (int t = 0; t < NCI; ++t)
#pragma unroll
      for (int k = 0; k < 9; ++k) acc[o][t][k] = f32x4{0.0f, 0.0f, 0.0f, 0.0f};
  const int per_row = (xb - xa) / 16, nsteps = max(y1 - y0, 0) * per_row;
  f32x4 a4[NCO];
  F2 e[NCI][3][3];
  auto fetch = [&](int step, f32x4 (&av)[NCO], F2 (&ev)[NCI][3][3]) {
    const int yy = y0 + step / per_row, x0 = xa + (step % per_row) * 16;
#pragma unroll
    for (int o = 0; o < NCO; ++o) av[o] = *reinterpret_cast<const f32x4*>(ga + o * gtile + static_cast<long>(yy) * W + x0);
#pragma unroll
    for (int t = 0; t < NCI; ++t)
#pragma unroll
      for (int ky = 0; ky < 3; ++ky) {
        const float* q = pa + t * ptile + static_cast<long>(yy + ky) * Wp + x0;
        ev[t][ky][0] = *reinterpret_cast<const F2*>(q); ev[t][ky][1] = *reinterpret_cast<const F2*>(q + 2);
        ev[t][ky][2] = *reinterpret_cast<const F2*>(q + 4);
      }
  };
#pragma unroll
  for (int o = 0; o < NCO; ++o) a4[o] = f32x4{0.0f, 0.0f, 0.0f, 0.0f};
  if (nsteps > 0) fetch(0, a4, e);
  for (int step = 0; step < nsteps; ++step) {
    f32x4 an[NCO];
    F2 en[NCI][3][3];
#pragma unroll
    for (int o = 0; o < NCO; ++o) an[o] = a4[o];
#pragma unroll
    for (int t = 0; t < NCI; ++t)
#pragma unroll
      for (int ky = 0; ky < 3; ++ky)
#pragma unroll
        for (int j = 0; j < 3; ++j) en[t][ky][j] = e[t][ky][j];
    if (step + 1 < nsteps) fetch(step + 1, an, en);
#pragma unroll
    for (int s = 0; s < 4; ++s)
#pragma unroll
      for (int t = 0; t < NCI; ++t)
#pragma unroll
        for (int ky = 0; ky < 3; ++ky) {
          const float v[6] = {e[t][ky][0].a, e[t][ky][0].b, e[t][ky][1].a, e[t][ky][1].b, e[t][ky][2].a, e[t][ky][2].b};
#pragma unroll
          for (int kx = 0; kx < 3; ++kx)
#pragma unroll
            for (int o = 0; o < NCO; ++o)
              acc[o][t][ky * 3 + kx] = __builtin_amdgcn_mfma_f32_16x16x4f32(a4[o][s], v[s + kx], acc[o][t][ky * 3 + kx], 0, 0, 0);
        }
#pragma unroll
    for (int o = 0; o < NCO; ++o) a4[o] = an[o];
#pragma unroll
    for (int t = 0; t < NCI; ++t)
#pragma unroll
      for (int ky = 0; ky < 3; ++ky)
#pragma unroll
        for (int j = 0; j < 3; ++j) e[t][ky][j] = en[t][ky][j];
  }
  float* po = part + static_cast<long>(blockIdx.x) * Co * Ci * 9;
#pragma unroll
  for (int o = 0; o < NCO; ++o)
#pragma unroll
    for (int t = 0; t < NCI; ++t)
#pragma unroll
      for (int k = 0; k < 9; ++k)
#pragma unroll
        for (int r = 0; r < 4; ++r)
          po[(static_cast<long>(k) * Co + co0 + 16 * o + 4 * kq + r) * Ci + ci0 + 16 * t + m] = acc[o][t][k][r];
}

constexpr int WF_LANES = 64;
__global__ void __launch_bounds__(16 * WF_LANES) k_wgrad_final(const float* __restrict__ part, float* __restrict__ gw, int n,
                                                               int nunits, int coci) {
  __shared__ float sm[WF_LANES][17];
  const int ii = threadIdx.x & 15, ul = threadIdx.x >> 4;
  const int i = blockIdx.x * 16 + ii;
  float s0 = 0.0f, s1 = 0.0f, s2 = 0.0f, s3 = 0.0f;
  if (i < n) {
    const float* q = part + i;
    int u = ul;
    for (; u + 3 * WF_LANES < nunits; u += 4 * WF_LANES) {
      s0 += q[static_cast<long>(u) * n]; s1 += q[static_cast<long>(u + WF_LANES) * n];
      s2 += q[static_cast<long>(u + 2 * WF_LANES) * n]; s3 += q[static_cast<long>(u + 3 * WF_LANES) * n];
    }
    for (; u < nunits; u += WF_LANES) s0 += q[static_cast<long>(u) * n];
  }
  sm[ul][ii] = (s0 + s1) + (s2 + s3);
  __syncthreads();
  if (ul == 0 && i < n) {
    float t = 0.0f;
    for (int k = 0; k < WF_LANES; ++k) t += sm[k][ii];
    const int tap = i / coci, cc = i - tap * coci;
    gw[static_cast<long>(cc) * 9 + tap] = t;
  }
}

}

#define DFE_LAUNCH_CHECK() do { if (hipGetLastError() != hipSuccess) return DFE_ERR_LAUNCH; } while (0)
using namespace dfe;

struct WgSplit { int R, nrg, nseg; long units; };
static WgSplit wg_split(int B, int H, int W, int tiles) {
  WgSplit s{1, H, 1, 0};
  const long total = tiles <= 2 ? 1024 : 4096;
  const long target = total / tiles > 0 ? total / tiles : 1;
  while (s.R < H && static_cast<long>(B) * ((H + s.R - 1) / s.R) > target) s.R *= 2;
  s.nrg = (H + s.R - 1) / s.R;
  while (s.nseg < 4 && s.nseg * 2 <= W / 16 && static_cast<long>(B) * s.nrg * s.nseg * 2 <= target) s.nseg *= 2;
  s.units = static_cast<long>(B) * s.nrg * s.nseg;
  return s;
}

static int wg_dims(int B, int Ci, int Co, int H, int W) {
  if (B <= 0 || Ci <= 0 || Co <= 0 || H <= 0 || W <= 0) return DFE_ERR_DIMS;
  if (Ci % 16 != 0 || Co % 16 != 0 || W % 16 != 0 || Ci / 16 > 65535 || Co / 16 > 65535) return DFE_ERR_UNSUPPORTED;
  if ((static_cast<long>(H) + 2) * (W + 2) * Ci >= (1L << 31) || static_cast<long>(H) * W * Co >= (1L << 31)) return DFE_ERR_DIMS;
  return DFE_OK;
}

static void wg_group(int Ci, int Co, int& nco, int& nci) {
  const int tci = Ci / 16, tco = Co / 16;
  nco = 1; nci = 1;
  if (tci * tco >= 6 && tco % 2 == 0 && tci % 3 == 0) { nco = 2; nci = 3; }
  else if (tci * tco >= 4 && tco % 2 == 0 && tci % 2 == 0) { nco = 2; nci = 2; }
}

extern "C" long dfe_wgrad3x3_partials_floats(int B, int Ci, int Co, int H, int W) {
  if (wg_dims(B, Ci, Co, H, W) != DFE_OK) return 0;
  int nco, nci;
  wg_group(Ci, Co, nco, nci);
  return wg_split(B, H, W, (Ci / (16 * nci)) * (Co / (16 * nco))).units * Co * Ci * 9;
}

extern "C" int dfe_wgrad3x3_fwd(const float* p, const float* gy, float* gweight, float* partials, int B, int Ci, int Co, int H,
                                int W, void* stream) {
  if (!p || !gy || !gweight || !partials) return DFE_ERR_NULL;
  const int rc = wg_dims(B, Ci, Co, H, W);
  if (rc != DFE_OK) return rc;
  if ((reinterpret_cast<uintptr_t>(p) & 7) || (reinterpret_cast<uintptr_t>(gy) & 15)) return DFE_ERR_UNSUPPORTED;
  hipStream_t st = static_cast<hipStream_t>(stream);
  int nco, nci;
  wg_group(Ci, Co, nco, nci);
  const WgSplit sp = wg_split(B, H, W, (Ci / (16 * nci)) * (Co / (16 * nco)));
  const dim3 grid(static_cast<unsigned>(sp.units), Ci / (16 * nci), Co / (16 * nco));
  if (nco == 2 && nci == 3) k_wgrad3x3_thin<2, 3><<<grid, 64, 0, st>>>(p, gy, partials, Ci, Co, H, W, sp.R, sp.nrg, sp.nseg);
  else if (nco == 2) k_wgrad3x3_thin<2, 2><<<grid, 64, 0, st>>>(p, gy, partials, Ci, Co, H, W, sp.R, sp.nrg, sp.nseg);
  else k_wgrad3x3_thin<1, 1><<<grid, 64, 0, st>>>(p, gy, partials, Ci, Co, H, W, sp.R, sp.nrg, sp.nseg);
  DFE_LAUNCH_CHECK();
  const int n = Co * Ci * 9;
  k_wgrad_final<<<(n + 15) / 16, 16 * WF_LANES, 0, st>>>(partials, gweight, n, static_cast<int>(sp.units), Co * Ci);
  DFE_LAUNCH_CHECK();
  return DFE_OK;
}
```

unsupervised_depth_opticalflow_egomotion_amd/csrc/ops_wino_wgrad.hip:

```cpp
#include "dfe_internal.h"
#include "dfe_device.h"
#include "dfe_wgrad_sum.h"
#include <hip/hip_runtime.h>
#include <algorithm>
#include <cstdlib>

namespace dfe {

typedef float wg_f32x4 __attribute__((ext_vector_type(4)));
typedef float wg_f32x2 __attribute__((ext_vector_type(2)));
struct __attribute__((packed, aligned(4))) WgQuadU { float a, b, c, d; };

template <int MH, int NH, int WM, int WN, int TWC>
struct WgCfg {
  static constexpr int COB = 16 * MH * WM, CIB = 16 * NH * WN;
  static constexpr int XU = TWC == 8 ? 6 : 8;
  static constexpr int XP = 4 * XU;
  static constexpr int XCS = 4 * XP + 4;
  static constexpr int GU = TWC / 2;
  static constexpr int GSL = TWC == 8 ? 4 : 8;
  static constexpr int GP = 2 * TWC;
  static constexpr int GCS = 2 * GP + 4;
  static constexpr int BUF = CIB * XCS + COB * GCS;
  static constexpr int GCH = 256 / (2 * GSL);
  static constexpr int NXT = (CIB + 7) / 8, NGT = (COB + GCH - 1) / GCH;
};

template <int MH, int NH, int WM, int WN, int TWC, int PP>
__global__ void __launch_bounds__(256, 2)
k_wino_wgrad2(const float* __restrict__ x, long xbs, const float* __restrict__ gy, long gbs, float* __restrict__ part, int C, int K,
              int W, int HW, int Hq, int Wq, int Ho, int Wo, int gW, int gHW, int TH, int cpr, int TWn, int nchunks, int cps, int ncit,
              int ntb) {
  typedef WgCfg<MH, NH, WM, WN, TWC> Cfg;
  constexpr int WG_XP = Cfg::XP, WG_XCS = Cfg::XCS, WG_GP = Cfg::GP, WG_GCS = Cfg::GCS, WG_TWC = TWC;
  constexpr int S = PP == 1 ? 3 : 0;
  constexpr int CS = PP == 1 ? 4 : 0;
  extern __shared__ float lds[];
  const int tid = threadIdx.x, lane = tid & 63, wv = tid >> 6, i = lane & 15, kq = lane >> 4;
  const int wm = wv / WN, wn = wv % WN;
  const unsigned lid = xcd_swizzle(blockIdx.x, gridDim.x);
  const int tb = static_cast<int>(lid % static_cast<unsigned>(ntb)), split = static_cast<int>(lid / static_cast<unsigned>(ntb));
  const int cob0 = (tb / ncit) * Cfg::COB, cib0 = (tb % ncit) * Cfg::CIB;
  const int c_beg = split * cps, c_end = min(nchunks, c_beg + cps);

  const int xq_ = tid & 7, xr_ = (tid >> 3) & 3, xc_ = tid >> 5;
  const int gq_ = tid & (Cfg::GSL - 1), gr_ = (tid / Cfg::GSL) & 1, gc_ = tid / (2 * Cfg::GSL);
  const int xl0 = xc_ * WG_XCS + xr_ * WG_XP + 4 * xq_;
  const int gl0 = Cfg::CIB * WG_XCS + gc_ * WG_GCS + gr_ * WG_GP + 4 * gq_;
  const int xg0 = (cib0 + xc_) * HW + (xr_ - PP) * W + (4 * xq_ - CS);
  const int gg0 = (cob0 + gc_) * gHW + gr_ * gW + 4 * gq_;
  wg_f32x4 xr[Cfg::NXT], gr[Cfg::NGT];
  int cx = c_beg % cpr, ty = (c_beg / cpr) % TH, img = c_beg / cpr / TH;
  auto load_chunk = [&]() {
    const long xb = img * xbs + static_cast<long>(2 * ty) * W + 2 * TWC * cx;
    const long gb = img * gbs + static_cast<long>(2 * ty) * gW + 2 * TWC * cx;
// ... 211 lines not shown
}

extern "C" int dfe_wino_wgrad_tune(int tile, int blocks1, int blocks2, int chunk) {
  if (tile != 0 && tile != 11 && tile != 12 && tile != 21) return DFE_ERR_UNSUPPORTED;
  if (chunk != 0 && chunk != 8 && chunk != 12) return DFE_ERR_UNSUPPORTED;
  g_wg_tune[0] = tile;
  if (blocks1 > 0) g_wg_tune[1] = blocks1;
  if (blocks2 > 0) g_wg_tune[2] = blocks2;
  if (chunk > 0) g_wg_tune[3] = chunk;
  return DFE_OK;
}

extern "C" long dfe_wino_wgrad_floats(int B, int Ci, int Co, int H, int W, int P) {
  WgPlan p;
  if (!wg_plan(B, Ci, Co, H, W, P, &p)) return 0;
  return static_cast<long>(p.S) * Co * Ci * 9;
}

template <int MH, int NH, int TWC, int PP>
static void wg_launch(const WgPlan& p, const float* x, long xbs, const float* gy, long gbs, float* ws, int Ci, int Co, int H, int W,
                      hipStream_t st) {
  typedef WgCfg<MH, NH, 2, 2, TWC> Cfg;
  const int ntb = p.ncot * p.ncit;
  const size_t lds_bytes = sizeof(float) * 2 * Cfg::BUF;
  auto kern = k_wino_wgrad2<MH, NH, 2, 2, TWC, PP>;
  static bool attr_set = false;
  if (!attr_set) { (void)hipFuncSetAttribute(reinterpret_cast<const void*>(kern), hipFuncAttributeMaxDynamicSharedMemorySize, static_cast<int>(lds_bytes)); attr_set = true; }
  kern<<<static_cast<unsigned>(ntb) * p.S, 256, lds_bytes, st>>>(x, xbs, gy, gbs, ws, Ci, Co, W, H * W, H, W, p.Ho, p.Wo, p.Wo, p.Ho * p.Wo, p.TH,
                                                                   p.cpr, p.TWn, p.nchunks, p.cps, p.ncit, ntb);
}

extern "C" int dfe_wino_wgrad3x3(const float* x, long x_batch_stride, const float* gy, long gy_batch_stride, float* gweight, float* ws, int B,
                                 int Ci, int Co, int H, int W, int P, void* stream) {
  if (!x || !gy || !gweight || !ws) return DFE_ERR_NULL;
  if (B <= 0 || Ci <= 0 || Co <= 0 || H <= 0 || W <= 0) return DFE_ERR_DIMS;
  if (P < 0 || P > 1) return DFE_ERR_UNSUPPORTED;
  WgPlan p;
  if (!wg_plan(B, Ci, Co, H, W, P, &p)) return DFE_ERR_DIMS;
  const long gplane = static_cast<long>(p.Ho) * p.Wo;
  if (x_batch_stride < static_cast<long>(Ci) * H * W || gy_batch_stride < Co * gplane) return DFE_ERR_DIMS;
  if (static_cast<long>(Ci) * H * W >= (1L << 30) || Co * gplane >= (1L << 30) || static_cast<long>(Co) * Ci * 9 >= (1L << 30)) return DFE_ERR_DIMS;
  hipStream_t st = static_cast<hipStream_t>(stream);
#define WG_GO(MHV, NHV, TWV) do { \
    if (P == 1) wg_launch<MHV, NHV, TWV, 1>(p, x, x_batch_stride, gy, gy_batch_stride, ws, Ci, Co, H, W, st); \
    else wg_launch<MHV, NHV, TWV, 0>(p, x, x_batch_stride, gy, gy_batch_stride, ws, Ci, Co, H, W, st); } while (0)
  if (p.mh == 2 && p.twc == 12) WG_GO(2, 1, 12);
  else if (p.mh == 2) WG_GO(2, 1, 8);
  else if (p.nh == 2) WG_GO(1, 2, 8);
  else if (p.twc == 12) WG_GO(1, 1, 12);
  else WG_GO(1, 1, 8);
#undef WG_GO
  DFE_LAUNCH_CHECK();
  const long n = static_cast<long>(Co) * Ci * 9;
  if (p.S > 64) k_wgrad_sum<32><<<static_cast<unsigned>((n + 31) / 32), 1024, 0, st>>>(ws, gweight, p.S, n);
  else k_wgrad_sum<8><<<static_cast<unsigned>((n + 31) / 32), 256, 0, st>>>(ws, gweight, p.S, n);
  DFE_LAUNCH_CHECK();
  return DFE_OK;
}
```

unsupervised_depth_opticalflow_egomotion_amd/ddp.py:

```python
import os

import torch
import torch.distributed as dist


def env_world():
    return int(os.environ.get("WORLD_SIZE", "1")), int(os.environ.get("RANK", "0")), int(os.environ.get("LOCAL_RANK", "0"))


def rccl_options():
    try:
        opts = dist.ProcessGroupNCCL.Options()
        opts.is_high_priority_stream = True
        return opts
    except AttributeError:
        return None


def init_process_group(backend=None, force=False):
    world, rank, local = env_world()
    if (world > 1 or force) and not dist.is_initialized():
        os.environ.setdefault("MASTER_ADDR", "127.0.0.1")
        os.environ.setdefault("MASTER_PORT", "29500")
        if backend is None:
# ... 83 lines not shown
    def _issue(self, k):
        idx = self._members[k]
        grads = [self._params[i].grad for i in idx]
        ref = next((g for g in grads if g is not None), self._params[idx[0]])
        flat, views = self._buffers_for(ref)
        ev = self._events.pop(k, None)
        if ev is not None:
            torch.cuda.current_stream().wait_event(ev)
        have = [j for j, g in enumerate(grads) if g is not None]
        if len(have) == len(idx):
            torch._foreach_copy_([views[i] for i in idx], grads)
            self._present[k].fill_(1.0)
        else:
            present = torch.zeros(len(idx))
            for j in have:
                present[j] = 1.0
            self._present[k].copy_(present)
            for j, i in enumerate(idx):
                if grads[j] is None:
                    views[i].zero_()
            if have:
                torch._foreach_copy_([views[idx[j]] for j in have], [grads[j] for j in have])
        beg, n = self._seg[k]
        seg = flat[beg:beg + n]
        if self.backend == "nccl":
            self._work[k] = (dist.all_reduce(seg, op=dist.ReduceOp.AVG, async_op=True), seg, len(have) == len(idx))
        else:
            self._work[k] = (dist.all_reduce(seg, async_op=True), seg, len(have) == len(idx))
        self._sig[k] = self._signature(k)
        self._issued.append(k)

    def _signature(self, k):
        idx = self._members[k]
        return tuple((id(g), g._version) if g is not None else None for g in (self._params[idx[0]].grad, self._params[idx[-1]].grad))

    def _pump(self):
        for k in self._order:
            if k in self._issued:
                continue
            if k not in self._ready:
                break
            self._issue(k)
            self.early_hits += 1

    def _trigger(self, k):
        if k in self._issued:
            self._dirty.add(k)
            return
        if any(self._params[i].grad is None for i in self._members[k]):
            return
        self._ready.add(k)
        g = self._params[self._members[k][0]].grad
        if g.is_cuda:
            ev = torch.cuda.Event()
            ev.record()
            self._events[k] = ev
        self._pump()

    def _agree(self):
        self.calibration_steps += 1
        pos = {i: n for n, i in enumerate(self._arrival)}
        last = {}
        for k in self.branches:
            seen = [i for i in self._members[k] if i in pos]
            if len(seen) == len(self._members[k]):
                last[k] = max(seen, key=lambda i: pos[i])
        dev = self._params[0].device if self.backend == "nccl" else torch.device("cpu")
        flag = torch.tensor([1 if len(last) == len(self.branches) else 0], dtype=torch.int64, device=dev)
        dist.all_reduce(flag, op=dist.ReduceOp.MIN)
        if int(flag.item()) == 0:
            self._arrival.clear()
            return
        mine = sorted(range(len(self.branches)), key=lambda b: pos[last[self.branches[b]]])
        order = torch.tensor(mine, dtype=torch.int64, device=dev)
        dist.broadcast(order, src=0)
        self._arm([self.branches[b] for b in order.tolist()], last)

    def _arm(self, order, last):
        for h in self._hooks:
            h.remove()
        self._hooks = []
        self._order = list(order)
        self.triggers = {k: self._names[i] for k, i in last.items()}
        for k, i in last.items():
            self._hooks.append(self._params[i].register_post_accumulate_grad_hook(lambda _p, k=k: self._trigger(k)))
        self._arrival = None

    @torch.no_grad()
    def reduce_gradients(self):
        if self.overlap and self._order is None:
            self._agree()
            armed_now = self._order is not None
        else:
            armed_now = False
        order = self.branches if (self._order is None or armed_now) else self._order
        for k in order:
            stale = False
            if k in self._issued:
                stale = k in self._dirty or self._signature(k) != self._sig[k]
                if stale:
                    self._work.pop(k)[0].wait()
                    self._issued.remove(k)
            if k not in self._issued:
                self._issue(k)
        for k in order:
            work, seg, complete = self._work.pop(k)
            work.wait()
            if self.backend != "nccl":
                seg.div_(self.world)
            idx = self._members[k]
            if complete:
                for i in idx:
                    self._params[i].grad = self._views[i]
            else:
                present = self._present[k].cpu()
                for j, i in enumerate(idx):
                    if float(present[j]) > 0.0:
                        self._params[i].grad = self._views[i]
        self._ready, self._issued, self._sig = set(), [], {}
        self._dirty, self._events = set(), {}


def wrap(model, device=None, bucket_cap_mb=25, force=False, strategy=None):
    world, _, local = env_world()
    if world == 1 and not force:
        return model
    strategy = os.environ.get("DFE_DP_STRATEGY", strategy or "flat")
    if strategy == "flat":
        return FlatAllReduce(model, unused_parameter_names(model))
    from torch.nn.parallel import DistributedDataParallel as DDP
    DDP._set_params_and_buffers_to_ignore_for_model(model, unused_parameter_names(model))
    kw = dict(bucket_cap_mb=bucket_cap_mb, static_graph=False, broadcast_buffers=False)
    for item in filter(None, os.environ.get("DFE_DDP_OPTS", "").split(",")):
        k, v = item.split("=")
        kw[k] = float(v) if k == "bucket_cap_mb" else bool(int(v))
    if device is not None and device.type == "cuda":
        kw.setdefault("gradient_as_bucket_view", True)
        return DDP(model, device_ids=[device.index], output_device=device.index, **kw)
    return DDP(model, **kw)


def shard_indices(n, world, rank):
# ... 6 lines not shown
```

unsupervised_depth_opticalflow_egomotion_amd/ops.py:

```python
from __future__ import annotations

import ctypes
import os
import threading

import torch

from . import _lib, convs
from ._lib import DfeError, check, f32c, get_lib, ptr, stream_ptr

_ALIGN_CORNERS = False


def set_align_corners(flag: bool):
    global _ALIGN_CORNERS
    _ALIGN_CORNERS = bool(flag)


def get_align_corners() -> bool:
    return _ALIGN_CORNERS


def _ac(flag):
    return int(_ALIGN_CORNERS if flag is None else bool(flag))


def scatter_ws(n, device):
    return torch.empty(get_lib().dfe_scatter_ws_bytes(int(n)), device=device, dtype=torch.uint8)


def prepare_cameras(pose, K, downscales):
    lib = get_lib()
    pose = f32c(pose.detach())
    if pose.dim() == 2:
        pose = pose.unsqueeze(1)
    B, ndir = pose.shape[0], pose.shape[1]
    K = f32c(K.detach())
    n = len(downscales)
    cams = torch.empty(B * ndir * n, lib.dfe_camera_floats(), device=pose.device, dtype=torch.float32)
    ds = (ctypes.c_float * n)(*[float(d) for d in downscales])
    check(lib.dfe_prepare_cameras(ptr(pose), ptr(K), ptr(cams), B, ndir, n, ctypes.cast(ds, ctypes.c_void_p),
                                  stream_ptr()), "dfe_prepare_cameras")
    return cams


class WarpFlowFn(torch.autograd.Function):
    @staticmethod
    def forward(ctx, x, flow, use_mask, align_corners):
        lib = get_lib()
        x, flow = f32c(x), f32c(flow)
        B, C, H, W = x.shape
        out = torch.empty_like(x)
        check(lib.dfe_warp_flow_fwd(ptr(x), ptr(flow), ptr(out), B, C, H, W, int(use_mask), align_corners,
                                    stream_ptr()), "dfe_warp_flow_fwd")
        ctx.save_for_backward(x, flow)
        ctx.cfg = (int(use_mask), align_corners)
        return out

    @staticmethod
    def backward(ctx, gout):
        lib = get_lib()
# ... 464 lines not shown

def texture_mask(img, warped, source):
    lib = get_lib()
    a, b, c = (f32c(t.detach()) for t in (img, warped, source))
    B, C, H, W = a.shape
    if C != 3 or b.shape != a.shape or c.shape != a.shape:
        raise ValueError("texture_mask expects three [B,3,H,W] tensors")
    out = torch.empty(B, 1, H, W, device=a.device)
    check(lib.dfe_texture_mask(ptr(a), ptr(b), ptr(c), ptr(out), B, H, W, stream_ptr()), "dfe_texture_mask")
    return out


def dynamic_mask(flow, rigid, alpha, beta):
    lib = get_lib()
    f, r = f32c(flow.detach()), f32c(rigid.detach())
    B, C, H, W = f.shape
    if C != 2 or r.shape != f.shape:
        raise ValueError("dynamic_mask expects two [B,2,H,W] tensors")
    mask, score = torch.empty(B, 1, H, W, device=f.device), torch.empty(B, 1, H, W, device=f.device)
    check(lib.dfe_dynamic_mask(ptr(f), ptr(r), ptr(mask), ptr(score), float(alpha), float(beta), B, H, W, stream_ptr()),
          "dfe_dynamic_mask")
    return mask, score


class EluPadFn(torch.autograd.Function):

    @staticmethod
    def forward(ctx, x, bias, apply_elu):
        lib = get_lib()
        x = f32c(x)
        bias = f32c(bias) if bias is not None else None
        B, C, H, W = x.shape
        out = torch.empty(B, C, H + 2, W + 2, device=x.device)
        check(lib.dfe_elu_pad_fwd(ptr(x), ptr(bias), ptr(out), B, C, H, W, int(apply_elu), stream_ptr()), "dfe_elu_pad_fwd")
        ctx.apply_elu = int(apply_elu)
        ctx.shape = (B, C, H, W)
        ctx.has_bias = bias is not None
        ctx.save_for_backward(x if apply_elu else x.new_empty(0), bias if bias is not None else x.new_empty(0))
        return out

    @staticmethod
    def backward(ctx, gout):
        lib = get_lib()
        x, bias = ctx.saved_tensors
        B, C, H, W = ctx.shape
        gout = f32c(gout)
        gx = torch.empty(B, C, H, W, device=gout.device)
        gb = part = None
        if ctx.has_bias and ctx.needs_input_grad[1]:
            gb = torch.empty(C, device=gout.device)
            part = torch.empty(lib.dfe_glue_partials_floats(B, C, H, W), device=gout.device)
        check(lib.dfe_elu_pad_bwd(ptr(x) if ctx.apply_elu else None, ptr(bias) if ctx.has_bias else None, ptr(gout), ptr(gx),
                                  ptr(gb), ptr(part), B, C, H, W, ctx.apply_elu, stream_ptr()), "dfe_elu_pad_bwd")
        return gx, gb, None


class EluUp2CatPadFn(torch.autograd.Function):

    @staticmethod
    def forward(ctx, x, bias, skip):
        lib = get_lib()
        x = f32c(x)
        bias = f32c(bias) if bias is not None else None
        B, C1, h, w = x.shape
        C2 = 0
        if skip is not None:
            skip = f32c(skip)
            C2 = skip.shape[1]
            if tuple(skip.shape) != (B, C2, 2 * h, 2 * w):
                raise ValueError("skip must be [B,C2,2h,2w] = %s, got %s" % ((B, C2, 2 * h, 2 * w), tuple(skip.shape)))
        out = torch.empty(B, C1 + C2, 2 * h + 2, 2 * w + 2, device=x.device)
        check(lib.dfe_elu_up2_cat_pad_fwd(ptr(x), ptr(bias), ptr(skip), ptr(out), B, C1, C2, h, w, stream_ptr()),
              "dfe_elu_up2_cat_pad_fwd")
        ctx.has_bias = bias is not None
        ctx.save_for_backward(x, bias if bias is not None else x.new_empty(0))
        ctx.dims = (B, C1, C2, h, w)
        return out

    @staticmethod
    def backward(ctx, gout):
        lib = get_lib()
        x, bias = ctx.saved_tensors
        B, C1, C2, h, w = ctx.dims
        gout = f32c(gout)
        want_b = ctx.has_bias and ctx.needs_input_grad[1]
        gx = torch.empty_like(x) if (ctx.needs_input_grad[0] or want_b) else None
        gskip = torch.empty(B, C2, 2 * h, 2 * w, device=x.device) if (C2 > 0 and ctx.needs_input_grad[2]) else None
        if gx is None and gskip is None:
            return None, None, None
        gb = part = None
        if want_b:
            gb = torch.empty(C1, device=x.device)
            part = torch.empty(lib.dfe_glue_partials_floats(B, C1, h, w), device=x.device)
        check(lib.dfe_elu_up2_cat_pad_bwd(ptr(x), ptr(bias) if ctx.has_bias else None, ptr(gout), ptr(gx), ptr(gskip), ptr(gb),
                                          ptr(part), B, C1, C2, h, w, stream_ptr()), "dfe_elu_up2_cat_pad_bwd")
        return gx, gb, gskip


def elu_pad(x, bias=None, apply_elu=True):
    return EluPadFn.apply(x, bias, bool(apply_elu))


def elu_up2_cat_pad(x, bias=None, skip=None):
    return EluUp2CatPadFn.apply(x, bias, skip)


class BiasActFn(torch.autograd.Function):

    @staticmethod
    def forward(ctx, z, bias, slope):
        lib = get_lib()
        if not z.is_contiguous() or z.dtype != torch.float32:
            raise _lib.DfeError("bias_act expects a contiguous fp32 convolution output")
        B, C, H, W = z.shape
        b = f32c(bias) if bias is not None else None
        check(lib.dfe_bias_act_fwd(ptr(z), ptr(b), B, C, H, W, float(slope), stream_ptr()), "dfe_bias_act_fwd")
        ctx.mark_dirty(z)
        ctx.save_for_backward(z)
        ctx.slope = float(slope)
        ctx.has_bias = bias is not None
        return z

    @staticmethod
    def backward(ctx, gy):
        lib = get_lib()
        (y,) = ctx.saved_tensors
        B, C, H, W = y.shape
        if gy.dtype != torch.float32:
            gy = gy.float()
        if not (gy.stride(3) == 1 and gy.stride(2) == W and gy.stride(1) == H * W and gy.stride(0) >= C * H * W):
            gy = gy.contiguous()
        gz = torch.empty_like(y)
        gb = part = None
        if ctx.has_bias and ctx.needs_input_grad[1]:
            gb = torch.empty(C, device=y.device, dtype=torch.float32)
            part = torch.empty(lib.dfe_bias_act_partials_floats(B, C, H, W), device=y.device, dtype=torch.float32)
        check(lib.dfe_bias_act_bwd(ptr(y), ptr(gy, strided=True), gy.stride(0), ptr(gz), ptr(gb), ptr(part), B, C, H, W, ctx.slope,
                                   stream_ptr()), "dfe_bias_act_bwd")
        return gz, gb, None


def bias_act(z, bias, slope):
    return BiasActFn.apply(z, bias, float(slope))


PLANECONV_MAX_HW = int(os.environ.get("DFE_PLANECONV_MAX_HW", "208"))
WINO_EPILOGUE = os.environ.get("DFE_WINO_EPILOGUE", "1") != "0"
FLOW_HEAD = os.environ.get("DFE_FLOW_HEAD", "1") != "0"
PWC_LEVEL_MAP = os.environ.get("DFE_PWC_LEVEL_MAP", "1") != "0"


def planeconv_eligible(x, w):
    if PLANECONV_MAX_HW <= 0 or not x.is_cuda or x.dim() != 4:
        return False
    B, Ci, H, W = x.shape
    return (x.dtype == torch.float32 and w.dtype == torch.float32 and tuple(w.shape[1:]) == (Ci, 3, 3)
            and H * W <= PLANECONV_MAX_HW and get_lib().dfe_planeconv_supported(B, Ci, int(w.shape[0]), H, W) == 1)


def _planeconv_ws(B, Ci, Co, H, W, dev):
    return torch.empty(get_lib().dfe_planeconv_ws_floats(B, Ci, Co, H, W), device=dev, dtype=torch.float32)


def planeconv_fwd_into(x, w, bias, slope, d1, d1_off=0, d2=None, d2_off=0):
    B, Ci, H, W = x.shape
    Co, HW = int(w.shape[0]), H * W
    p1 = ctypes.c_void_p(d1.data_ptr() + 4 * d1_off * HW)
    p2 = ctypes.c_void_p(d2.data_ptr() + 4 * d2_off * HW) if d2 is not None else None
    ws = _planeconv_ws(B, Ci, Co, H, W, x.device)
    check(get_lib().dfe_planeconv_fwd(ptr(x), ptr(w), ptr(bias), float(slope), p1, d1.stride(0), p2,
                                      d2.stride(0) if d2 is not None else 0, ptr(ws), B, Ci, Co, H, W, stream_ptr()),
          "dfe_planeconv_fwd")


def planeconv_forward(x, w, bias=None, slope=1.0):
    x, w = f32c(x), f32c(w)
    y = torch.empty(x.shape[0], w.shape[0], x.shape[2], x.shape[3], device=x.device, dtype=torch.float32)
    planeconv_fwd_into(x, w, None if bias is None else f32c(bias), slope, y)
    return y


def planeconv_backward(gy, x, w, want_x=True, want_w=True):
    gy, x, w = f32c(gy), f32c(x), f32c(w)
    B, Ci, H, W = x.shape
    Co = int(w.shape[0])
    lib = get_lib()
    ws = _planeconv_ws(B, Ci, Co, H, W, x.device)
    gx = gw = None
    if want_x:
        gx = torch.empty_like(x)
        check(lib.dfe_planeconv_dgrad(ptr(gy), ptr(w), ptr(gx), ptr(ws), B, Ci, Co, H, W, stream_ptr()), "dfe_planeconv_dgrad")
    if want_w:
        gw = torch.empty_like(w)
        check(lib.dfe_planeconv_wgrad(ptr(gy), ptr(x), ptr(gw), ptr(ws), B, Ci, Co, H, W, stream_ptr()), "dfe_planeconv_wgrad")
    return gx, gw


class WinoWeightCache:

    def __init__(self):
        self.enabled = os.environ.get("DFE_WINO_CACHE", "1") != "0"
        self.verify = os.environ.get("DFE_WINO_CACHE_VERIFY", "0") == "1"
        self.entries = {}
        self.table = None
        self.blockmap = None
        self.members = None
        self.hits = self.misses = 0
        if os.environ.get("DFE_WINO_CACHE_STATS"):
            import atexit
            import sys
            atexit.register(lambda: sys.stderr.write("[dfe] wino weight cache: %d filters, %d hits, %d misses\n"
                                                     % (len(self.entries), self.hits, self.misses)))

    def lookup(self, w, transposed):
        if not self.enabled or not w.is_cuda or w.dim() != 4:
            return None
        key = (w.data_ptr(), int(w.shape[0]), int(w.shape[1]))
        e = self.entries.get(key)
        if e is None:
            if isinstance(w, torch.nn.Parameter) and w.dtype == torch.float32 and w.is_contiguous():
                import weakref
                self.entries[key] = {"ref": weakref.ref(w), "version": -1, "U": None, "device": w.device}
                self.members = None
            self.misses += 1
            return None
        p = e["ref"]()
        if p is None or p.data_ptr() != key[0]:
            del self.entries[key]
            self.members = None
            self.misses += 1
            return None
        if e["U"] is None or e["version"] != w._version or e["version"] != p._version:
            self.misses += 1
            return None
        self.hits += 1
        U = e["U"][1 if transposed else 0]
        if self.verify and not torch.equal(U, self.transform_now(w, transposed)):
            raise _lib.DfeError("WinoWeightCache: the cached filters of a %s parameter are stale -- it was written without a version "
                                "bump (p.data.mul_/copy_, a raw-pointer kernel) after the last refresh; call "
                                "ops.wino_weights.invalidate() after such writes" % (tuple(w.shape),))
        return U

    @staticmethod
    def transform_now(w, transposed):
        lib = get_lib()
        Co, Ci = int(w.shape[0]), int(w.shape[1])
        K, C = (Ci, Co) if transposed else (Co, Ci)
# ... 72 lines not shown
            raise _lib.DfeError("wino_conv3x3: the output channels do not fit the destination buffer")
        p1 = ctypes.c_void_p(y.data_ptr() + 4 * int(out_off) * HWo)
        p2 = ctypes.c_void_p(out2.data_ptr() + 4 * int(out2_off) * HWo) if out2 is not None else None
        npart = 0 if d > 1 else lib.dfe_wino_scratch_floats(B, Ci, Co, H, W, P) - lib.dfe_wino_weight_floats(Ci, Co)
        part = torch.empty(npart, device=x.device, dtype=torch.float32) if npart > 0 else None
        check(lib.dfe_wino_conv3x3_u_act(ptr(x), ptr(U), ptr(f32c(bias)) if bias is not None else None, float(slope), p1, y.stride(0), p2,
                                         out2.stride(0) if out2 is not None else 0, ptr(part), npart, B, Ci, Co, H, W, P, d, stream_ptr()),
              "dfe_wino_conv3x3_u_act")
        return y
    y = torch.empty(B, Co, Ho, Wo, device=x.device, dtype=torch.float32)
    if U is not None:
        npart = 0 if d > 1 else lib.dfe_wino_scratch_floats(B, Ci, Co, H, W, P) - lib.dfe_wino_weight_floats(Ci, Co)
        part = torch.empty(npart, device=x.device, dtype=torch.float32) if npart > 0 else None
        check(lib.dfe_wino_conv3x3_u(ptr(x), ptr(U), ptr(y), y.stride(0), ptr(part), npart, B, Ci, Co, H, W, P, d, stream_ptr()),
              "dfe_wino_conv3x3_u")
        return y
    nws = lib.dfe_wino_weight_floats(Ci, Co) if d > 1 else lib.dfe_wino_scratch_floats(B, Ci, Co, H, W, P)
    wbuf = torch.empty(nws, device=x.device, dtype=torch.float32)
    if d > 1:
        check(lib.dfe_wino_conv3x3_dilated(ptr(x), ptr(w), ptr(y), y.stride(0), ptr(wbuf), B, Ci, Co, H, W, d, int(bool(transposed)),
                                           stream_ptr()), "dfe_wino_conv3x3_dilated")
        return y
    check(lib.dfe_wino_conv3x3(ptr(x), ptr(w), ptr(y), y.stride(0), ptr(wbuf), nws, B, Ci, Co, H, W, P, int(bool(transposed)),
                               stream_ptr()), "dfe_wino_conv3x3")
    return y


class ConvBiasActFn(torch.autograd.Function):

    @staticmethod
    def forward(ctx, x, w, bias, slope, padding, dilation):
        y = wino_conv3x3(x, w, padding, dilation=dilation, bias=bias, slope=slope)
        ctx.save_for_backward(x, w, y)
        ctx.cfg = (float(slope), int(padding), int(dilation), bias is not None)
        return y

    @staticmethod
    def backward(ctx, gy):
        lib = get_lib()
        x, w, y = ctx.saved_tensors
        slope, P, d, has_bias = ctx.cfg
        B, C, H, W = y.shape
        if gy.dtype != torch.float32:
            gy = gy.float()
        if not (gy.stride(3) == 1 and gy.stride(2) == W and gy.stride(1) == H * W and gy.stride(0) >= C * H * W):
            gy = gy.contiguous()
        gz = torch.empty_like(y)
        gb = part = None
        if has_bias and ctx.needs_input_grad[2]:
            gb = torch.empty(C, device=y.device, dtype=torch.float32)
            part = torch.empty(lib.dfe_bias_act_partials_floats(B, C, H, W), device=y.device, dtype=torch.float32)
        check(lib.dfe_bias_act_bwd(ptr(y), ptr(gy, strided=True), gy.stride(0), ptr(gz), ptr(gb), ptr(part), B, C, H, W, slope,
                                   stream_ptr()), "dfe_bias_act_bwd")
        pad = (d, d) if d > 1 else (P, P)
        gx, gw, _ = convs.raw_backward(gz, x, w, (1, 1), pad, (d, d), ctx.needs_input_grad[0], ctx.needs_input_grad[1])
        return gx, gw, gb, None, None, None


def conv_bias_act_eligible(x, conv):
    return (WINO_EPILOGUE and conv.bias is not None and conv.groups == 1
            and convs._wino_eligible(x, conv.weight.shape, conv.in_channels, conv.stride, conv.padding, conv.dilation, conv.groups)
            and conv.padding == ((1, 1) if conv.dilation == (1, 1) else conv.dilation))


def conv_bias_act(x, conv, slope):
    return ConvBiasActFn.apply(x, conv.weight, conv.bias, float(slope), int(conv.padding[0]), int(conv.dilation[0]))


def phase_images(t, d):
    B, C, H, W = t.shape
    return t.reshape(B, C, H // d, d, W // d, d).permute(0, 3, 5, 1, 2, 4).reshape(B * d * d, C, H // d, W // d)


def wino_wgrad3x3(x, gy, padding=1, dilation=1):
    d = int(dilation)
    if d > 1:
        if x.shape[2] % d or x.shape[3] % d or gy.shape[2:] != x.shape[2:]:
            raise _lib.DfeError("wino_wgrad3x3: a dilated layer needs H and W to be multiples of the dilation and padding = dilation")
        x, gy, padding = phase_images(x, d), phase_images(gy, d), 1
    def dense_chw(t):
        return t.dtype == torch.float32 and t.stride(3) == 1 and t.stride(2) == t.shape[3] and t.stride(1) == t.shape[2] * t.shape[3]
    x = x if dense_chw(x) else f32c(x)
    gy = gy if dense_chw(gy) else f32c(gy)
    B, Ci, H, W = x.shape
    Co, P = int(gy.shape[1]), int(padding)
    lib = get_lib()
    gw = torch.empty(Co, Ci, 3, 3, device=x.device, dtype=torch.float32)
    n = lib.dfe_wino_wgrad_floats(B, Ci, Co, H, W, P)
    if n <= 0:
        raise _lib.DfeError("dfe_wino_wgrad3x3: unsupported shape %s padding %d" % (tuple(x.shape), P))
    ws = torch.empty(n, device=x.device, dtype=torch.float32)
    check(lib.dfe_wino_wgrad3x3(ptr(x, strided=True), x.stride(0), ptr(gy, strided=True), gy.stride(0), ptr(gw), ptr(ws), B, Ci, Co, H, W, P,
                                stream_ptr()), "dfe_wino_wgrad3x3")
    return gw


def _dense_chw(t):
    return t.dtype == torch.float32 and t.stride(3) == 1 and t.stride(2) == t.shape[3] and t.stride(1) == t.shape[2] * t.shape[3]


def sconv_wgrad_supported(x_shape, co, k, stride, padding):
    B, Ci, H, W = (int(v) for v in x_shape)
    return get_lib().dfe_sconv_wgrad_floats(B, Ci, int(co), H, W, int(k), int(stride), int(padding)) > 0


def sconv_wgrad(x, gy, k, stride, padding):
    x = x if _dense_chw(x) else f32c(x)
    gy = gy if _dense_chw(gy) else f32c(gy)
    B, Ci, H, W = x.shape
    Co, k, s, P = int(gy.shape[1]), int(k), int(stride), int(padding)
    if tuple(gy.shape[2:]) != ((H + 2 * P - k) // s + 1, (W + 2 * P - k) // s + 1) or gy.shape[0] != B:
        raise _lib.DfeError("sconv_wgrad: gy %s does not belong to x %s with k %d stride %d padding %d" % (tuple(gy.shape), tuple(x.shape), k, s, P))
    lib = get_lib()
    n = lib.dfe_sconv_wgrad_floats(B, Ci, Co, H, W, k, s, P)
    if n <= 0:
        raise _lib.DfeError("dfe_sconv_wgrad: unsupported layer %s -> %d, k %d stride %d padding %d" % (tuple(x.shape), Co, k, s, P))
    gw = torch.empty(Co, Ci, k, k, device=x.device, dtype=torch.float32)
    ws = torch.empty(n, device=x.device, dtype=torch.float32)
    check(lib.dfe_sconv_wgrad(ptr(x, strided=True), x.stride(0), ptr(gy, strided=True), gy.stride(0), ptr(gw), ptr(ws), B, Ci, Co, H, W, k, s, P,
                              stream_ptr()), "dfe_sconv_wgrad")
    return gw


class PlaneConvActFn(torch.autograd.Function):

    @staticmethod
    def forward(ctx, x, w, bias, slope):
        x, w = f32c(x), f32c(w)
        y = torch.empty(x.shape[0], w.shape[0], x.shape[2], x.shape[3], device=x.device, dtype=torch.float32)
        planeconv_fwd_into(x, w, None if bias is None else f32c(bias), slope, y)
        ctx.save_for_backward(x, w, y)
        ctx.slope, ctx.has_bias = float(slope), bias is not None
        return y

    @staticmethod
    def backward(ctx, gy):
        lib = get_lib()
        x, w, y = ctx.saved_tensors
        B, C, H, W = y.shape
        gy = f32c(gy)
        gz = torch.empty_like(y)
        gb = part = None
        if ctx.has_bias and ctx.needs_input_grad[2]:
            gb = torch.empty(C, device=y.device, dtype=torch.float32)
            part = torch.empty(lib.dfe_bias_act_partials_floats(B, C, H, W), device=y.device, dtype=torch.float32)
        check(lib.dfe_bias_act_bwd(ptr(y), ptr(gy), gy.stride(0), ptr(gz), ptr(gb), ptr(part), B, C, H, W, ctx.slope,
                                   stream_ptr()), "dfe_bias_act_bwd")
        gx, gw = planeconv_backward(gz, x, w, ctx.needs_input_grad[0], ctx.needs_input_grad[1])
        return gx, gw, gb, None


def planeconv_act(x, w, bias, slope):
    return PlaneConvActFn.apply(x, w, bias, float(slope))


class Conv1x1SmallFn(torch.autograd.Function):

    @staticmethod
    def forward(ctx, x, w, bias, slope):
        x, w = f32c(x), f32c(w)
        B, Ci, H, W = x.shape
        Co = int(w.shape[0])
        y = torch.empty(B, Co, H, W, device=x.device, dtype=torch.float32)
        check(get_lib().dfe_conv1x1_small_fwd(ptr(x), ptr(w), ptr(None if bias is None else f32c(bias)), float(slope), ptr(y),
                                              B, Ci, Co, H, W, stream_ptr()), "dfe_conv1x1_small_fwd")
        ctx.save_for_backward(x, w, y)
        ctx.slope, ctx.has_bias = float(slope), bias is not None
        return y

    @staticmethod
    def backward(ctx, gy):
        lib = get_lib()
        x, w, y = ctx.saved_tensors
        B, Co, H, W = y.shape
        Ci = int(x.shape[1])
        gy = f32c(gy)
        gz = torch.empty_like(y)
        gb = part = None
        if ctx.has_bias and ctx.needs_input_grad[2]:
            gb = torch.empty(Co, device=y.device, dtype=torch.float32)
            part = torch.empty(lib.dfe_bias_act_partials_floats(B, Co, H, W), device=y.device, dtype=torch.float32)
        check(lib.dfe_bias_act_bwd(ptr(y), ptr(gy), gy.stride(0), ptr(gz), ptr(gb), ptr(part), B, Co, H, W, ctx.slope,
                                   stream_ptr()), "dfe_bias_act_bwd")
        gx = torch.empty_like(x) if ctx.needs_input_grad[0] else None
        gw = torch.empty_like(w) if ctx.needs_input_grad[1] else None
        check(lib.dfe_conv1x1_small_bwd(ptr(gz), ptr(x), ptr(w), ptr(gx), ptr(gw), B, Ci, Co, H, W, stream_ptr()),
              "dfe_conv1x1_small_bwd")
        return gx, gw, gb, None


def conv1x1_small_eligible(x, conv):
    return (PLANECONV_MAX_HW > 0 and x.is_cuda and x.dim() == 4 and x.dtype == torch.float32
            and conv.kernel_size == (1, 1) and conv.stride == (1, 1) and conv.padding == (0, 0) and conv.groups == 1
            and get_lib().dfe_conv1x1_small_supported(x.shape[0], x.shape[1], conv.out_channels, x.shape[2], x.shape[3]) == 1)


def conv1x1_small(x, conv, slope):
    return Conv1x1SmallFn.apply(x, conv.weight, conv.bias, float(slope))


class DenseDecodeFn(torch.autograd.Function):

    @staticmethod
    def forward(ctx, slope, x, *wb):
        import torch.nn.functional as F
        lib = get_lib()
        x = f32c(x)
        w, b = list(wb[0:12:2]), list(wb[1:12:2])
        B, _, H, W = x.shape
        HW = H * W
        co = [int(t.shape[0]) for t in w[:5]]
        dev = x.device
        cat = [torch.empty(B, co[k] + co[k + 1], H, W, device=dev, dtype=torch.float32) for k in range(4)]
        st = stream_ptr()

        def epilogue(z, k, d1, d1_off, d2, d2_off):
            c = co[k]
            p1 = ctypes.c_void_p(d1.data_ptr() + 4 * d1_off * HW)
            p2 = ctypes.c_void_p(d2.data_ptr() + 4 * d2_off * HW) if d2 is not None else None
            check(lib.dfe_bias_act_fwd2(ptr(z), ptr(b[k]), p1, d1.stride(0), p2, d2.stride(0) if d2 is not None else 0,
                                        B, c, H, W, slope, st), "dfe_bias_act_fwd2")

        plane = planeconv_eligible(x, w[0])
        if plane:
            z0 = torch.empty(B, co[0], H, W, device=dev, dtype=torch.float32)
            x4 = torch.empty(B, co[4], H, W, device=dev, dtype=torch.float32)
            planeconv_fwd_into(x, w[0], b[0], slope, z0, 0, cat[0], 0)
            planeconv_fwd_into(z0, w[1], b[1], slope, cat[0], co[0], cat[1], 0)
            planeconv_fwd_into(cat[0], w[2], b[2], slope, cat[1], co[1], cat[2], 0)
            planeconv_fwd_into(cat[1], w[3], b[3], slope, cat[2], co[2], cat[3], 0)
            planeconv_fwd_into(cat[2], w[4], b[4], slope, x4, 0, cat[3], co[3])
        else:
            fuse = WINO_EPILOGUE

            def layer(inp, k, d1, d1_off, d2, d2_off):
                if fuse and convs._wino_eligible(inp, w[k].shape, w[k].shape[1], (1, 1), (1, 1), (1, 1)):
# ... 27 lines not shown
        st = stream_ptr()
        need = ctx.needs_input_grad
        nw = lambda k: bool(need[2 + 2 * k])
        nb = lambda k: bool(need[3 + 2 * k])
        def cb(g, inp, wt, want_in, want_w, bias_sizes=None, want_b=False):
            if ctx.plane and not want_b:
                return planeconv_backward(g, inp, wt, want_in, want_w) + (None,)
            return convs.raw_backward(g, inp, wt, 1, 1, 1, want_in, want_w, want_b)

        def epilogue_bwd(k, ysrc, y_off, g1, g1_off, g2, g2_off):
            c = co[k]
            gz = torch.empty(B, c, H, W, device=dev, dtype=torch.float32)
            gb = part = None
            if nb(k):
                gb = torch.empty(c, device=dev, dtype=torch.float32)
                part = torch.empty(lib.dfe_bias_act_partials_floats(B, c, H, W), device=dev, dtype=torch.float32)
                pending.append((part, gb, c))
            sl = lambda t, off: ctypes.c_void_p(t.data_ptr() + 4 * off * HW)
            check(lib.dfe_bias_act_bwd2(sl(ysrc, y_off), ysrc.stride(0), sl(g1, g1_off), g1.stride(0),
                                        sl(g2, g2_off) if g2 is not None else None, g2.stride(0) if g2 is not None else 0,
                                        ptr(gz), None, ptr(part), B, c, H, W, slope, st), "dfe_bias_act_bwd2")
            return gz, gb

        pending = []

        gw, gbias = [None] * 6, [None] * 6
        if g_flow is not None:
            g_flow = f32c(g_flow)
            if flow_head_eligible(cat[3], w[5], True):
                g3, gw[5], gbias[5] = flow_head_bwd_raw(cat[3], f32c(w[5]), g_flow, nw(5), nb(5))
            else:
                g3, gw[5], gbias[5] = cb(g_flow, cat[3], w[5], True, nw(5), [2], nb(5))
        else:
            g3 = torch.zeros_like(cat[3])
        if g_x4 is not None:
            if g_x4.dtype != torch.float32 or not (g_x4.stride(3) == 1 and g_x4.stride(2) == W and g_x4.stride(1) == HW
                                                   and g_x4.stride(0) >= co[4] * HW):
                g_x4 = f32c(g_x4)
        gz, gbias[4] = epilogue_bwd(4, cat[3], co[3], g3, co[3], g_x4, 0)
        g2, gw[4], _ = cb(gz, cat[2], w[4], True, nw(4))
        gz, gbias[3] = epilogue_bwd(3, cat[3], 0, g3, 0, g2, co[2])
        g1, gw[3], _ = cb(gz, cat[1], w[3], True, nw(3))
        gz, gbias[2] = epilogue_bwd(2, cat[2], 0, g2, 0, g1, co[1])
        g0, gw[2], _ = cb(gz, cat[0], w[2], True, nw(2))
        gz, gbias[1] = epilogue_bwd(1, cat[1], 0, g1, 0, g0, co[0])
        gx0, gw[1], _ = cb(gz, x0, w[1], True, nw(1))
        gz, gbias[0] = epilogue_bwd(0, cat[0], 0, g0, 0, gx0, 0)
        if pending:
            n = len(pending)
            parts = (ctypes.c_void_p * n)(*[t[0].data_ptr() for t in pending])
            outs = (ctypes.c_void_p * n)(*[t[1].data_ptr() for t in pending])
            chans = (ctypes.c_int * n)(*[t[2] for t in pending])
            check(lib.dfe_bias_grad_final_multi(parts, outs, chans, n, B, H, W, st), "dfe_bias_grad_final_multi")
        gx, gw[0], _ = cb(gz, x, w[0], bool(need[1]), nw(0))
        out = [None, gx]
        for k in range(6):
            out += [gw[k], gbias[k]]
        return tuple(out)


def dense_decode(x, convs, predict_flow, slope=0.1):
    wb = []
    for c in list(convs) + [predict_flow]:
        wb += [c.weight, c.bias]
    return DenseDecodeFn.apply(float(slope), x, *wb)


class GroupedBatchNormFn(torch.autograd.Function):

    @staticmethod
    def forward(ctx, x, residual, weight, bias, running_mean, running_var, groups, eps, momentum, relu):
        lib = get_lib()
        x = f32c(x)
        N, C, H, W = x.shape
        G = int(groups)
        if N % G:
            raise ValueError("batch %d is not divisible into %d groups" % (N, G))
        Bg = N // G
        residual = f32c(residual) if residual is not None else None
        if residual is not None and residual.shape != x.shape:
            raise ValueError("residual must have the shape of x")
        dev = x.device
        y = torch.empty_like(x)
        mean = torch.empty(G * C, device=dev)
        invstd = torch.empty(G * C, device=dev)
        npart = lib.dfe_bn_partials_floats(G, Bg, C, H, W)
        part = torch.empty(max(npart, 1), device=dev)
        check(lib.dfe_bn_fwd(ptr(x), ptr(residual), ptr(weight), ptr(bias), ptr(running_mean), ptr(running_var), ptr(y),
                             ptr(mean), ptr(invstd), ptr(part), G, Bg, C, H, W, float(eps), float(momentum), int(relu),
                             stream_ptr()), "dfe_bn_fwd")
        ctx.save_for_backward(x, y if relu else x.new_empty(0), weight if weight is not None else x.new_empty(0), mean, invstd)
        ctx.cfg = (G, Bg, C, H, W, int(relu), residual is not None, weight is not None)
        ctx.mark_non_differentiable(mean, invstd)
        return y

    @staticmethod
    def backward(ctx, gy):
        lib = get_lib()
        x, y, weight, mean, invstd = ctx.saved_tensors
        G, Bg, C, H, W, relu, has_res, has_w = ctx.cfg
        gy = f32c(gy)
        dev = x.device
        gx = torch.empty_like(x)
        gres = (torch.empty_like(x) if relu else None) if (has_res and ctx.needs_input_grad[1]) else None
        gw = torch.empty(C, device=dev) if (has_w and ctx.needs_input_grad[2]) else None
        gb = torch.empty(C, device=dev) if ctx.needs_input_grad[3] else None
        part = torch.empty(max(lib.dfe_bn_partials_floats(G, Bg, C, H, W), 1), device=dev)
        scratch = torch.empty(2 * G * C, device=dev)
        check(lib.dfe_bn_bwd(ptr(x), ptr(y) if relu else None, ptr(gy), ptr(weight) if has_w else None, ptr(mean), ptr(invstd),
                             ptr(gx), ptr(gres), ptr(gw), ptr(gb), ptr(part), ptr(scratch), G, Bg, C, H, W, relu,
                             stream_ptr()), "dfe_bn_bwd")
        if has_res and ctx.needs_input_grad[1] and not relu:
            gres = gy
        return gx, gres, gw, gb, None, None, None, None, None, None


def grouped_batch_norm(x, weight, bias, running_mean, running_var, groups=1, eps=1e-5, momentum=0.1, residual=None,
                       relu=False):
    return GroupedBatchNormFn.apply(x, residual, weight, bias, running_mean, running_var, int(groups), float(eps),
                                    float(momentum), bool(relu))


class DispHeadFn(torch.autograd.Function):

    @staticmethod
    def forward(ctx, p, weight, bias):
        lib = get_lib()
        p, weight = f32c(p), f32c(weight)
        bias = f32c(bias) if bias is not None else None
        B, C, Hp, Wp = p.shape
        if tuple(weight.shape) != (1, C, 3, 3):
            raise ValueError("weight must be [1,%d,3,3], got %s" % (C, tuple(weight.shape)))
        H, W = Hp - 2, Wp - 2
        out = torch.empty(B, 1, H, W, device=p.device)
        check(lib.dfe_disp_head_fwd(ptr(p), ptr(weight), ptr(bias), ptr(out), B, C, H, W, stream_ptr()), "dfe_disp_head_fwd")
        ctx.save_for_backward(p, weight, out)
        ctx.has_bias = bias is not None
        return out

    @staticmethod
    def backward(ctx, gout):
        lib = get_lib()
        p, weight, out = ctx.saved_tensors
        B, C, Hp, Wp = p.shape
        H, W = Hp - 2, Wp - 2
        gout = f32c(gout)
        gp = torch.empty_like(p)
        gw = torch.empty_like(weight) if ctx.needs_input_grad[1] else None
        gb = torch.empty(1, device=p.device) if (ctx.has_bias and ctx.needs_input_grad[2]) else None
        part = torch.empty(lib.dfe_disp_head_partials_floats(B, C, H, W), device=p.device)
        check(lib.dfe_disp_head_bwd(ptr(p), ptr(weight), ptr(out), ptr(gout), ptr(gp), ptr(gw), ptr(gb), ptr(part), B, C, H, W,
                                    stream_ptr()), "dfe_disp_head_bwd")
        return gp, gw, gb


def disp_head(p, weight, bias):
    return DispHeadFn.apply(p, weight, bias)


def flow_head_fwd_raw(x, weight, bias):
    lib = get_lib()
    B, C, H, W = x.shape
    out = torch.empty(B, 2, H, W, device=x.device, dtype=torch.float32)
    check(lib.dfe_flow_head_fwd(ptr(x), ptr(weight), ptr(bias), ptr(out), B, C, H, W, stream_ptr()), "dfe_flow_head_fwd")
    return out


def flow_head_bwd_raw(x, weight, gout, want_w=True, want_b=True):
    lib = get_lib()
    B, C, H, W = x.shape
    gx = torch.empty_like(x)
    gw = torch.empty_like(weight) if want_w else None
    gb = torch.empty(2, device=x.device, dtype=torch.float32) if want_b else None
    part = torch.empty(lib.dfe_flow_head_partials_floats(B, C, H, W), device=x.device, dtype=torch.float32)
    check(lib.dfe_flow_head_bwd(ptr(x), ptr(weight), ptr(gout), ptr(gx), ptr(gw), ptr(gb), ptr(part), B, C, H, W,
                                stream_ptr()), "dfe_flow_head_bwd")
    return gx, gw, gb


def flow_head_eligible(x, weight, bias=None):
    return (FLOW_HEAD and x.is_cuda
            and x.dtype == torch.float32 and x.dim() == 4 and tuple(weight.shape[2:]) == (3, 3) and weight.shape[0] == 2
            and weight.shape[1] == x.shape[1] and x.shape[1] % 8 == 0 and bias is not None)


class FlowHeadFn(torch.autograd.Function):

    @staticmethod
    def forward(ctx, x, weight, bias):
        x, weight, bias = f32c(x), f32c(weight), f32c(bias)
        ctx.save_for_backward(x, weight)
        return flow_head_fwd_raw(x, weight, bias)

    @staticmethod
    def backward(ctx, gout):
        x, weight = ctx.saved_tensors
        gx, gw, gb = flow_head_bwd_raw(x, weight, f32c(gout), ctx.needs_input_grad[1], ctx.needs_input_grad[2])
        return (gx if ctx.needs_input_grad[0] else None), gw, gb


class ThinConv3x3Fn(torch.autograd.Function):

    @staticmethod
    def forward(ctx, p, weight):
        ctx.save_for_backward(p, weight)
        return convs.raw_forward(p, weight)

    @staticmethod
    def backward(ctx, gy):
        lib = get_lib()
        p, weight = ctx.saved_tensors
        gy = f32c(gy)
        B, Ci, Hp, Wp = p.shape
        Co, H, W = weight.shape[0], Hp - 2, Wp - 2
        gp = gw = None
        if ctx.needs_input_grad[0]:
            gp = convs.raw_backward(gy, p, weight, 1, 0, 1, True, False)[0]
        if ctx.needs_input_grad[1]:
            if Ci >= 32 and convs.WINO_WGRAD:
                gw = wino_wgrad3x3(p, gy, 0)
            else:
                gw = torch.empty_like(weight)
                part = torch.empty(lib.dfe_wgrad3x3_partials_floats(B, Ci, Co, H, W), device=p.device)
                check(lib.dfe_wgrad3x3_fwd(ptr(p), ptr(gy), ptr(gw), ptr(part), B, Ci, Co, H, W, stream_ptr()), "dfe_wgrad3x3_fwd")
        return gp, gw


def thin_conv3x3_eligible(p, weight):
    Co, Ci = weight.shape[0], weight.shape[1]
    H, W = p.shape[2] - 2, p.shape[3] - 2
    return (p.is_cuda and p.dtype == torch.float32 and p.is_contiguous() and tuple(weight.shape[2:]) == (3, 3)
            and Co <= 32 and Co % 16 == 0 and Ci % 16 == 0 and W % 16 == 0 and H * W >= 64 * 208)


def conv3x3_valid(p, weight):
    if thin_conv3x3_eligible(p, weight):
        return ThinConv3x3Fn.apply(p, weight)
    return convs.conv2d(p, weight)
```

unsupervised_depth_opticalflow_egomotion_amd/optim.py:

```python
import ctypes

import torch

from ._lib import check, get_lib, stream_ptr


class FusedAdam(torch.optim.Optimizer):
    def __init__(self, params, lr=1e-3, betas=(0.9, 0.999), eps=1e-8, capturable=False):
        if lr < 0.0 or eps < 0.0 or not (0.0 <= betas[0] < 1.0) or not (0.0 <= betas[1] < 1.0):
            raise ValueError("invalid Adam hyper-parameters")
        defaults = dict(lr=lr, betas=tuple(betas), eps=eps, weight_decay=0, amsgrad=False, maximize=False, foreach=None,
                        capturable=bool(capturable), differentiable=False, fused=None)
        super().__init__(params, defaults)
        self._plans = {}
        self._dev_count = {}
        self._captured = []
        self.capture_epoch = 0

    MAX_PLANS = 8

    def state_dict(self):
        for gi, (count, _) in self._dev_count.items():
            t = float(count.cpu()[0])
            for p in self.param_groups[gi]["params"]:
                st = self.state.get(p)
                if st and "step" in st:
                    st["step"] = torch.tensor(t, dtype=torch.float32)
        sd = super().state_dict()
        sd["state"] = {k: ({**v, "step": v["step"].clone()} if "step" in v else v) for k, v in sd["state"].items()}
        return sd

    def load_state_dict(self, state_dict):
        super().load_state_dict(state_dict)
        self._plans = {}
        self._dev_count = {}
        if self._captured:
            self.capture_epoch += 1

    def _fingerprint(self, params):
        a, b = params[0], params[-1]
        return (a.data_ptr(), b.data_ptr(), self.state[a]["exp_avg"].data_ptr(), self.state[b]["exp_avg_sq"].data_ptr())

    def _plan(self, gi, params):
        key = (gi, tuple(id(p) for p in params))
        plan = self._plans.get(key)
        if plan is not None and plan["fingerprint"] == self._fingerprint(params):
            return plan
        lib = get_lib()
        chunk = lib.dfe_adam_chunk()
        dev = params[0].device
        rows, blocks = [], []
        for t, p in enumerate(params):
            st = self.state[p]
            rows.append([p.data_ptr(), 0, st["exp_avg"].data_ptr(), st["exp_avg_sq"].data_ptr(), p.numel()])
            blocks += [[t, c] for c in range((p.numel() + chunk - 1) // chunk)]
        plan = {"host": torch.tensor(rows, dtype=torch.int64),
                "pinned": [torch.empty(len(rows), 5, dtype=torch.int64).pin_memory() for _ in range(4)],
                "graph_pinned": torch.empty(len(rows), 5, dtype=torch.int64).pin_memory(),
                "events": [None] * 4, "turn": 0,
                "table": torch.empty(len(rows), 5, dtype=torch.int64, device=dev),
                "blockmap": torch.tensor(blocks, dtype=torch.int32).to(dev), "nblocks": len(blocks),
                "fingerprint": self._fingerprint(params)}
        mine = [k for k in self._plans if k[0] == gi]
        for k in mine[:max(0, len(mine) - (self.MAX_PLANS - 1))]:
            del self._plans[k]
        self._plans[key] = plan
        return plan

    @torch.no_grad()
    def step(self, closure=None):
        loss = None
        if closure is not None:
            with torch.enable_grad():
                loss = closure()
        lib = get_lib()
        for gi, group in enumerate(self.param_groups):
            if group.get("weight_decay", 0) or group.get("amsgrad") or group.get("maximize"):
                raise NotImplementedError("FusedAdam implements the reference's plain Adam (no weight decay / amsgrad / maximize)")
            params = [p for p in group["params"] if p.grad is not None]
            if not params:
                continue
            dev = params[0].device
            grads = []
            for p in params:
                g = p.grad
                if (g.is_sparse or g.dtype != torch.float32 or p.dtype != torch.float32 or not p.is_cuda or p.device != dev
                        or not p.is_contiguous()):
                    raise NotImplementedError("FusedAdam needs dense fp32 parameters and gradients on one HIP device")
                grads.append(g if g.is_contiguous() else g.contiguous())
                st = self.state[p]
                if not st:
                    st["step"] = torch.tensor(0.0, dtype=torch.float32)
                    st["exp_avg"] = torch.zeros_like(p, memory_format=torch.preserve_format)
                    st["exp_avg_sq"] = torch.zeros_like(p, memory_format=torch.preserve_format)
            by_step = {}
            for p, g in zip(params, grads):
                by_step.setdefault(float(self.state[p]["step"]), []).append((p, g))
            for t0, pg in by_step.items():
                ps = [p for p, _ in pg]
                plan = self._plan(gi, ps)
                host = plan["host"]
                host[:, 1] = torch.tensor([g.data_ptr() for _, g in pg], dtype=torch.int64)
                capturing = torch.cuda.is_current_stream_capturing()
                if capturing:
                    plan["graph_pinned"].copy_(host)
                    plan["table"].copy_(plan["graph_pinned"], non_blocking=True)
                    self._captured.append(plan)
                else:
                    k = plan["turn"]
                    plan["turn"] = (k + 1) % len(plan["pinned"])
                    if plan["events"][k] is not None:
                        plan["events"][k].synchronize()
                    plan["pinned"][k].copy_(host)
                    plan["table"].copy_(plan["pinned"][k], non_blocking=True)
                    ev = torch.cuda.Event()
                    ev.record()
                    plan["events"][k] = ev
                t = t0 + 1.0
                b1, b2 = group["betas"]
                if group.get("capturable"):
                    if len(by_step) != 1:
                        raise NotImplementedError("FusedAdam(capturable=True): all parameters of a group must step together")
                    dc = self._dev_count.get(gi)
                    if dc is None:
                        dc = self._dev_count[gi] = (torch.full((1,), t0, dtype=torch.float64, device=dev),
                                                    torch.zeros(2, dtype=torch.float32, device=dev))
                    if capturing:
                        self._captured.append(dc)
# ... 26 lines not shown
```

unsupervised_depth_opticalflow_egomotion_amd/train_step.py:

```python
import types

DEFAULT_CFG = dict(
    dataset="kitti_depth", num_scales=3, num_input_frames=3, flow_consist_alpha=0.01, flow_consist_beta=0.5,
    h_flow_consist_alpha=0.01, h_flow_consist_beta=0.5, geometric_ratio=0.3, geometric_num=6000, pose_beta=1,
    w_flow_pixel=0.15, w_flow_ssim=0.85, w_flow_smooth=10.0, w_flow_consis=0.01, w_depth_pixel=1.0, w_depth_ssim=0.85,
    w_depth_smooth=0.5, w_depth_consis=0.1, w_depth_flow_consis=1.0, w_epipolar=0.1, w_triangle=0.001, w_pnp=0.1,
    w_8point=0.1, img_hw=(256, 832), lr=1e-4, mode="geom", enable_depth_ssim=False, enable_depth_consis=False)

LOSS_WEIGHT_ATTR = {
    "loss_flow_pixel": "w_flow_pixel", "loss_flow_ssim": "w_flow_ssim", "loss_flow_smooth": "w_flow_smooth",
    "loss_flow_consis": "w_flow_consis", "loss_depth_pixel": "w_depth_pixel", "loss_depth_ssim": "w_depth_ssim",
    "loss_depth_smooth": "w_depth_smooth", "loss_depth_consis": "w_depth_consis",
    "loss_depth_flow_consis": "w_depth_flow_consis", "loss_epipolar": "w_epipolar", "loss_triangle": "w_triangle",
    "loss_pnp": "w_pnp", "loss_eight_point": "w_8point"}


def make_cfg(**over):
    d = dict(DEFAULT_CFG)
    d.update(over)
    return types.SimpleNamespace(**d)


def make_optimizer(model, lr, capturable=False):
    import os
    import torch
    params = [p for p in model.parameters() if p.requires_grad]
    on_gpu = bool(params) and all(p.is_cuda and p.dtype == torch.float32 for p in params)
    if on_gpu and os.environ.get("DFE_FUSED_ADAM", "1") != "0":
        from .optim import FusedAdam
        opt = FusedAdam(params, lr=lr, capturable=capturable)
    else:
        opt = torch.optim.Adam(params, lr=lr, fused=True, capturable=capturable) if on_gpu else torch.optim.Adam(params, lr=lr)
    if hasattr(model, "reduce_gradients"):
        opt.register_step_pre_hook(lambda _opt, _args, _kwargs: model.reduce_gradients())
    return opt


_WEIGHT_ROWS = {}


def total_loss(loss_pack, cfg):
    import torch
    rows = getattr(loss_pack, "rows", None)
    total, fused = None, {}
    if rows is not None:
        losses, fused = rows
        key = (losses.device, losses.shape, tuple(sorted((i, float(getattr(cfg, LOSS_WEIGHT_ATTR[k]))) for k, i in fused.items())))
        w = _WEIGHT_ROWS.get(key)
        if w is None:
            host = torch.zeros(losses.shape[0])
            for k, i in fused.items():
                host[i] = float(getattr(cfg, LOSS_WEIGHT_ATTR[k])) / losses.shape[1]
            w = _WEIGHT_ROWS[key] = host.to(losses.device)
        total = torch.dot(losses.sum(1), w)
    for k, v in loss_pack.items():
        if k in fused or getattr(v, "_dfe_zero_placeholder", False):
            continue
        term = getattr(cfg, LOSS_WEIGHT_ATTR[k]) * v.mean()
        total = term if total is None else total + term
    return total


def train_step(model, optimizer, inputs, cfg, profiler=None):
    from . import profiling
    optimizer.zero_grad(set_to_none=True)
    with profiling.range("forward"):
        loss_pack, mask_pack = model(inputs)
        loss = total_loss(loss_pack, cfg)
    if profiler is not None:
        profiler.report_process("forward")
    with profiling.range("backward"):
        loss.backward()
    if profiler is not None:
        profiler.report_process("backward")
    with profiling.range("optimizer"):
        optimizer.step()
    if profiler is not None:
        profiler.report_process("optimizer")
    return loss, loss_pack, mask_pack


class GraphedTrainStep:

    def __init__(self, model, optimizer, inputs, cfg, warmup=3, restore=True):
        import torch
        if hasattr(model, "reduce_gradients") or type(model).__name__ == "DistributedDataParallel":
            raise NotImplementedError("GraphedTrainStep: single-process training only (collectives are not captured)")
        self.model, self.optimizer, self.cfg = model, optimizer, cfg
        self.static_inputs = [t.clone() for t in inputs]
        saved = self._snapshot() if restore else None
        side = torch.cuda.Stream()
        side.wait_stream(torch.cuda.current_stream())
        with torch.cuda.stream(side):
            for _ in range(max(int(warmup), 1)):
                train_step(model, optimizer, self.static_inputs, cfg)
        torch.cuda.current_stream().wait_stream(side)
        torch.cuda.synchronize()
        if saved is not None:
            self._restore(saved)
        optimizer.zero_grad(set_to_none=True)
        self.graph = torch.cuda.CUDAGraph()
        with torch.cuda.graph(self.graph):
            self.outputs = train_step(model, optimizer, self.static_inputs, cfg)
        from . import ops
        self._cache_tables = (ops.wino_weights.table, ops.wino_weights.blockmap)
        self._hyper = self._hyper_now()
        self._epoch = getattr(optimizer, "capture_epoch", 0)

    def _hyper_now(self):
        return [(float(g["lr"]), tuple(float(b) for b in g["betas"]), float(g["eps"])) for g in self.optimizer.param_groups]

    def _snapshot(self):
        opt = self.optimizer
        state = {}
        for group in opt.param_groups:
            for p in group["params"]:
                st = opt.state.get(p)
                if st:
                    state[p] = {k: (v.clone() if hasattr(v, "clone") else v) for k, v in st.items()}
        dev_count = {gi: [t.clone() for t in dc] for gi, dc in getattr(opt, "_dev_count", {}).items()}
        return ([p.detach().clone() for p in self.model.parameters()], [b.detach().clone() for b in self.model.buffers()],
                state, dev_count)

    def _restore(self, saved):
# ... 45 lines not shown
```

Before: 430.7 frame-pairs/s.

## Defer gradient-reduction finish kernels and batch them into grouped launches

Adds a deferred finish queue. The small final-reduction kernels for weight and bias gradients (bias sums, head finals, wgrad split sums) are recorded during backward instead of launched one by one, then flushed together in fewer launches before the optimizer step. The goal is to cut the launch count and tail latency of many tiny kernels. In exchange, the partial buffers must be kept alive on the Python side, and a flush is needed before any gradient is read, which adds bookkeeping and ordering risk across streams.

Measured after the change: 431.4 frame-pairs/s, median of 4. No clear change (+0.2%).

```diff
diff --git a/include/dfe_hip.h b/include/dfe_hip.h
--- a/include/dfe_hip.h
+++ b/include/dfe_hip.h
@@ -13,7 +13,7 @@
 #define DFE_ERR_WORKSPACE (-5)
 
 #define DFE_MAX_SCALES 8
-#define DFE_ABI_VERSION 3
+#define DFE_ABI_VERSION 4
 
 int dfe_abi_version(void);
 const char* dfe_error_string(int code);
@@ -188,6 +188,16 @@
 int dfe_bias_grad_final_multi(const float* const* partials, float* const* gbias, const int* C, int n, int B, int H, int W,
                               void* stream);
 
+int dfe_finish_set_deferred(int on);
+int dfe_finish_deferred(void);
+int dfe_finish_set_threshold(long bytes);
+int dfe_finish_flush(void* stream);
+int dfe_finish_flush_all(void* wait_stream);
+long dfe_finish_pending(void* stream);
+long dfe_finish_generation(void* stream);
+long dfe_finish_pending_total(void);
+long dfe_finish_launches(void);
+
 #define DFE_LOSS_DEPTH_PIXEL 0
 #define DFE_LOSS_DEPTH_SMOOTH 1
 #define DFE_LOSS_FLOW_PIXEL 2
diff --git a/unsupervised_depth_opticalflow_egomotion_amd/_lib.py b/unsupervised_depth_opticalflow_egomotion_amd/_lib.py
--- a/unsupervised_depth_opticalflow_egomotion_amd/_lib.py
+++ b/unsupervised_depth_opticalflow_egomotion_amd/_lib.py
@@ -72,6 +72,15 @@
     "dfe_bias_act_fwd2": [_P, _P, _P, ctypes.c_long, _P, ctypes.c_long, _I, _I, _I, _I, ctypes.c_float, _P],
     "dfe_bias_act_bwd2": [_P, ctypes.c_long, _P, ctypes.c_long, _P, ctypes.c_long, _P, _P, _P, _I, _I, _I, _I, ctypes.c_float, _P],
     "dfe_bias_grad_final_multi": [_P, _P, _P, _I, _I, _I, _I, _P],
+    "dfe_finish_set_deferred": [_I],
+    "dfe_finish_deferred": [],
+    "dfe_finish_set_threshold": [ctypes.c_long],
+    "dfe_finish_flush": [_P],
+    "dfe_finish_flush_all": [_P],
+    "dfe_finish_pending": [_P],
+    "dfe_finish_generation": [_P],
+    "dfe_finish_pending_total": [],
+    "dfe_finish_launches": [],
     "dfe_glue_partials_floats": [_I, _I, _I, _I],
     "dfe_elu_pad_fwd": [_P, _P, _P, _I, _I, _I, _I, _I, _P],
     "dfe_elu_pad_bwd": [_P, _P, _P, _P, _P, _P, _I, _I, _I, _I, _I, _P],
@@ -117,7 +126,8 @@
              "dfe_bn_partials_floats": ctypes.c_long, "dfe_disp_head_partials_floats": ctypes.c_long,
              "dfe_flow_head_partials_floats": ctypes.c_long, "dfe_pwc_level_map_bytes": ctypes.c_long,
              "dfe_wgrad3x3_partials_floats": ctypes.c_long, "dfe_planeconv_ws_floats": ctypes.c_long, "dfe_wino_weight_floats": ctypes.c_long, "dfe_wino_scratch_floats": ctypes.c_long, "dfe_wino_wgrad_floats": ctypes.c_long, "dfe_sconv_wgrad_floats": ctypes.c_long, "dfe_wino_transform_blocks": ctypes.c_long,
-             "dfe_geom_maskpack_offset_bytes": ctypes.c_long, "dfe_scatter_ws_bytes": ctypes.c_long}
+             "dfe_geom_maskpack_offset_bytes": ctypes.c_long, "dfe_scatter_ws_bytes": ctypes.c_long,
+             "dfe_finish_pending": ctypes.c_long, "dfe_finish_generation": ctypes.c_long, "dfe_finish_pending_total": ctypes.c_long, "dfe_finish_launches": ctypes.c_long}
 
 
 class DfeError(RuntimeError):
diff --git a/unsupervised_depth_opticalflow_egomotion_amd/csrc/dfe_finish.h b/unsupervised_depth_opticalflow_egomotion_amd/csrc/dfe_finish.h
--- /dev/null
+++ b/unsupervised_depth_opticalflow_egomotion_amd/csrc/dfe_finish.h
@@ -0,0 +1,105 @@
+#pragma once
+#include <hip/hip_runtime.h>
+#include "dfe_device.h"
+#include "dfe_wgrad_sum.h"
+
+namespace dfe {
+
+constexpr int DH_CI = 16;
+constexpr int FH_CI = 8;
+constexpr int WF_LANES = 64;
+
+__device__ __forceinline__ float wave_total(float v) {
+  v = dpp_add<0xB1>(v); v = dpp_add<0x4E>(v); v = dpp_add<0x141>(v); v = dpp_add<0x140>(v);
+  const float r0s = __int_as_float(__builtin_amdgcn_readlane(__float_as_int(v), 0));
+  const float r1s = __int_as_float(__builtin_amdgcn_readlane(__float_as_int(v), 16));
+  const float r2s = __int_as_float(__builtin_amdgcn_readlane(__float_as_int(v), 32));
+  const float r3s = __int_as_float(__builtin_amdgcn_readlane(__float_as_int(v), 48));
+  return (r0s + r1s) + (r2s + r3s);
+}
+
+__device__ __forceinline__ void bias_final_wave(const float* __restrict__ part, float* __restrict__ gbias, int B, int C, int nchunk,
+                                                int c, int lane) {
+  float s = 0.0f;
+  for (int b = 0; b < B; ++b) {
+    const float* p = part + (static_cast<long>(b) * C + c) * nchunk;
+    for (int k = lane; k < nchunk; k += 64) s += p[k];
+  }
+  const float tot = wave_total(s);
+  if (lane == 0) gbias[c] = tot;
+}
+
+template <int CO, int CI>
+__device__ __forceinline__ void head_final_wave(const float* __restrict__ part, float* __restrict__ gw, float* __restrict__ gb,
+                                                int C, int nunits, int nz, int o, int lane) {
+  constexpr int NACC = CI * CO * 9 + CO;
+  const bool isb = o >= CO * C * 9;
+  int z = 0, idx;
+  if (isb) idx = CI * CO * 9 + (o - CO * C * 9);
+  else {
+    const int co = o / (C * 9), c = (o - co * C * 9) / 9, t = o % 9;
+    z = c / CI;
+    idx = ((c - z * CI) * CO + co) * 9 + t;
+  }
+  float s = 0.0f;
+  for (int u = lane; u < nunits; u += 64) s += part[(static_cast<long>(u) * nz + z) * NACC + idx];
+  const float tot = wave_total(s);
+  if (lane == 0) {
+    if (isb) { if (gb) gb[o - CO * C * 9] = tot; } else if (gw) gw[o] = tot;
+  }
+}
+
+__device__ __forceinline__ void wgrad_final_block(const float* __restrict__ part, float* __restrict__ gw, int n, int nunits, int coci,
+                                                  int block, float (*sm)[17]) {
+  const int ii = threadIdx.x & 15, ul = threadIdx.x >> 4;
+  const int i = block * 16 + ii;
+  float s0 = 0.0f, s1 = 0.0f, s2 = 0.0f, s3 = 0.0f;
+  if (i < n) {
+    const float* q = part + i;
+    int u = ul;
+    for (; u + 3 * WF_LANES < nunits; u += 4 * WF_LANES) {
+      s0 += q[static_cast<long>(u) * n]; s1 += q[static_cast<long>(u + WF_LANES) * n];
+      s2 += q[static_cast<long>(u + 2 * WF_LANES) * n]; s3 += q[static_cast<long>(u + 3 * WF_LANES) * n];
+    }
+    for (; u < nunits; u += WF_LANES) s0 += q[static_cast<long>(u) * n];
+  }
+  sm[ul][ii] = (s0 + s1) + (s2 + s3);
+  __syncthreads();
+  if (ul == 0 && i < n) {
+    float t = 0.0f;
+    for (int k = 0; k < WF_LANES; ++k) t += sm[k][ii];
+    const int tap = i / coci, cc = i - tap * coci;
+    gw[static_cast<long>(cc) * 9 + tap] = t;
+  }
+}
+
+__device__ __forceinline__ float planeconv_slot_sum(const float* __restrict__ part, int total, int KS, int idx) {
+  float s = part[idx];
+#pragma unroll 4
+  for (int k = 1; k < KS; ++k) s += part[static_cast<long>(k) * total + idx];
+  return s;
+}
+
+enum FinishKind : int {
+  FIN_SUM8 = 0,
+  FIN_PLANE = 1,
+  FIN_SUM32 = 2,
+  FIN_WFINAL = 3,
+  FIN_BIAS = 4,
+  FIN_HEAD1 = 5,
+  FIN_HEAD2 = 6,
+};
+
+struct FinishJob {
+  const float* part;
+  float* out;
+  float* out2;
+  long n;
+  int kind, i0, i1, i2;
+};
+
+int finish_defer(const FinishJob& job, hipStream_t st, bool* taken);
+
+int finish_wgrad_sum(const float* ws, float* gw, int S, long n, hipStream_t st);
+
+}
diff --git a/unsupervised_depth_opticalflow_egomotion_amd/csrc/dfe_wgrad_sum.h b/unsupervised_depth_opticalflow_egomotion_amd/csrc/dfe_wgrad_sum.h
--- a/unsupervised_depth_opticalflow_egomotion_amd/csrc/dfe_wgrad_sum.h
+++ b/unsupervised_depth_opticalflow_egomotion_amd/csrc/dfe_wgrad_sum.h
@@ -4,10 +4,10 @@
 namespace dfe {
 
 template <int SG>
-__global__ void __launch_bounds__(32 * SG) k_wgrad_sum(const float* __restrict__ part, float* __restrict__ gw, int S, long n) {
-  __shared__ float sm[SG][32];
+__device__ __forceinline__ void wgrad_sum_block(const float* __restrict__ part, float* __restrict__ gw, int S, long n, long block,
+                                                float (*sm)[32]) {
   const int o = threadIdx.x & 31, g = threadIdx.x >> 5;
-  const long idx = static_cast<long>(blockIdx.x) * 32 + o;
+  const long idx = block * 32 + o;
   const int per = (S + SG - 1) / SG, s0 = g * per, s1 = min(S, s0 + per);
   float s = 0.0f;
   if (idx < n)
@@ -22,4 +22,12 @@
   }
 }
 
+template <int SG>
+__global__ void __launch_bounds__(32 * SG) k_wgrad_sum(const float* __restrict__ part, float* __restrict__ gw, int S, long n) {
+  __shared__ float sm[SG][32];
+  wgrad_sum_block<SG>(part, gw, S, n, static_cast<long>(blockIdx.x), sm);
 }
+
+inline bool wgrad_sum_wide(int S) { return S > 64; }
+
+}
diff --git a/unsupervised_depth_opticalflow_egomotion_amd/csrc/ops_decoder.hip b/unsupervised_depth_opticalflow_egomotion_amd/csrc/ops_decoder.hip
--- a/unsupervised_depth_opticalflow_egomotion_amd/csrc/ops_decoder.hip
+++ b/unsupervised_depth_opticalflow_egomotion_amd/csrc/ops_decoder.hip
@@ -1,5 +1,6 @@
 #include "dfe_internal.h"
 #include "dfe_device.h"
+#include "dfe_finish.h"
 #include <hip/hip_runtime.h>
 #include <cstdlib>
 
@@ -399,18 +400,7 @@
 
 __global__ void __launch_bounds__(64) k_glue_bias_final(const float* __restrict__ part, float* __restrict__ gbias,
                                                         int B, int C, int nblk) {
-  const int c = blockIdx.x, lane = threadIdx.x;
-  float s = 0.0f;
-  for (int b = 0; b < B; ++b) {
-    const float* p = part + (static_cast<long>(b) * C + c) * nblk;
-    for (int k = lane; k < nblk; k += 64) s += p[k];
-  }
-  s = dpp_add<0xB1>(s); s = dpp_add<0x4E>(s); s = dpp_add<0x141>(s); s = dpp_add<0x140>(s);
-  const float r0 = __int_as_float(__builtin_amdgcn_readlane(__float_as_int(s), 0));
-  const float r1 = __int_as_float(__builtin_amdgcn_readlane(__float_as_int(s), 16));
-  const float r2 = __int_as_float(__builtin_amdgcn_readlane(__float_as_int(s), 32));
-  const float r3 = __int_as_float(__builtin_amdgcn_readlane(__float_as_int(s), 48));
-  if (lane == 0) gbias[c] = (r0 + r1) + (r2 + r3);
+  bias_final_wave(part, gbias, B, C, nblk, blockIdx.x, threadIdx.x);
 }
 
 __global__ void __launch_bounds__(256) k_cat_pad_bwd_skip(const float* __restrict__ gp, float* __restrict__ gskip,
@@ -463,6 +453,9 @@
   else k_elu_pad_bwd<<<dim3(nb, C, B), 256, 0, st>>>(x, bias, gout, gx, gbias ? partials : nullptr, C, H, W, apply_elu);
   DFE_LAUNCH_CHECK();
   if (gbias) {
+    bool deferred = false;
+    const int qrc = finish_defer(FinishJob{partials, gbias, nullptr, 0, FIN_BIAS, B, C, static_cast<int>(nb)}, st, &deferred);
+    if (qrc != DFE_OK || deferred) return qrc;
     k_glue_bias_final<<<C, 64, 0, st>>>(partials, gbias, B, C, static_cast<int>(nb));
     DFE_LAUNCH_CHECK();
   }
@@ -498,8 +491,13 @@
     }
     DFE_LAUNCH_CHECK();
     if (gbias) {
-      k_glue_bias_final<<<C1, 64, 0, st>>>(partials, gbias, B, C1, static_cast<int>(nb));
-      DFE_LAUNCH_CHECK();
+      bool deferred = false;
+      const int qrc = finish_defer(FinishJob{partials, gbias, nullptr, 0, FIN_BIAS, B, C1, static_cast<int>(nb)}, st, &deferred);
+      if (qrc != DFE_OK) return qrc;
+      if (!deferred) {
+        k_glue_bias_final<<<C1, 64, 0, st>>>(partials, gbias, B, C1, static_cast<int>(nb));
+        DFE_LAUNCH_CHECK();
+      }
     }
   }
   if (gskip && C2 > 0) {
diff --git a/unsupervised_depth_opticalflow_egomotion_amd/csrc/ops_disphead.hip b/unsupervised_depth_opticalflow_egomotion_amd/csrc/ops_disphead.hip
--- a/unsupervised_depth_opticalflow_egomotion_amd/csrc/ops_disphead.hip
+++ b/unsupervised_depth_opticalflow_egomotion_amd/csrc/ops_disphead.hip
@@ -1,13 +1,12 @@
 #include "dfe_internal.h"
 #include "dfe_device.h"
+#include "dfe_finish.h"
 #include <hip/hip_runtime.h>
 
 namespace dfe {
 
 constexpr int DH_COLS = 62;
 constexpr int DH_ROWS = 16;
-constexpr int DH_CI = 16;
-constexpr int FH_CI = 8;
 
 
 template <bool VPAD>
@@ -139,14 +138,6 @@
   return gout[o] * (d * (1.0f - d));
 }
 
-__device__ __forceinline__ float wave_total(float v) {
-  v = dpp_add<0xB1>(v); v = dpp_add<0x4E>(v); v = dpp_add<0x141>(v); v = dpp_add<0x140>(v);
-  const float r0s = __int_as_float(__builtin_amdgcn_readlane(__float_as_int(v), 0));
-  const float r1s = __int_as_float(__builtin_amdgcn_readlane(__float_as_int(v), 16));
-  const float r2s = __int_as_float(__builtin_amdgcn_readlane(__float_as_int(v), 32));
-  const float r3s = __int_as_float(__builtin_amdgcn_readlane(__float_as_int(v), 48));
-  return (r0s + r1s) + (r2s + r3s);
-}
 
 template <int CO, bool SIG, bool VPAD, int CI>
 __global__ void __launch_bounds__(64) k_head_bwd(const float* __restrict__ p, const float* __restrict__ w,
@@ -243,22 +234,7 @@
 template <int CO, int CI>
 __global__ void __launch_bounds__(64) k_head_final(const float* __restrict__ part, float* __restrict__ gw,
                                                    float* __restrict__ gb, int C, int nunits, int nz) {
-  constexpr int NACC = CI * CO * 9 + CO;
-  const int o = blockIdx.x, lane = threadIdx.x;
-  const bool isb = o >= CO * C * 9;
-  int z = 0, idx;
-  if (isb) idx = CI * CO * 9 + (o - CO * C * 9);
-  else {
-    const int co = o / (C * 9), c = (o - co * C * 9) / 9, t = o % 9;
-    z = c / CI;
-    idx = ((c - z * CI) * CO + co) * 9 + t;
-  }
-  float s = 0.0f;
-  for (int u = lane; u < nunits; u += 64) s += part[(static_cast<long>(u) * nz + z) * NACC + idx];
-  const float tot = wave_total(s);
-  if (lane == 0) {
-    if (isb) { if (gb) gb[o - CO * C * 9] = tot; } else if (gw) gw[o] = tot;
-  }
+  head_final_wave<CO, CI>(part, gw, gb, C, nunits, nz, blockIdx.x, threadIdx.x);
 }
 
 }
@@ -303,6 +279,9 @@
   k_head_bwd<1, true, false, DH_CI><<<dim3(ns * nrb, B, nz), 64, 0, st>>>(p, weight, out, gout, gp, partials, C, H, W, ns);
   DFE_LAUNCH_CHECK();
   if (gweight || gbias) {
+    bool deferred = false;
+    const int qrc = finish_defer(FinishJob{partials, gweight, gbias, 0, FIN_HEAD1, C, B * ns * nrb, nz}, st, &deferred);
+    if (qrc != DFE_OK || deferred) return qrc;
     k_head_final<1, DH_CI><<<C * 9 + 1, 64, 0, st>>>(partials, gweight, gbias, C, B * ns * nrb, nz);
     DFE_LAUNCH_CHECK();
   }
@@ -342,6 +321,9 @@
   k_head_bwd<2, false, true, FH_CI><<<dim3(ns * nrb, B, nz), 64, 0, st>>>(x, weight, nullptr, gout, gx, partials, C, H, W, ns);
   DFE_LAUNCH_CHECK();
   if (gweight || gbias) {
+    bool deferred = false;
+    const int qrc = finish_defer(FinishJob{partials, gweight, gbias, 0, FIN_HEAD2, C, B * ns * nrb, nz}, st, &deferred);
+    if (qrc != DFE_OK || deferred) return qrc;
     k_head_final<2, FH_CI><<<2 * C * 9 + 2, 64, 0, st>>>(partials, gweight, gbias, C, B * ns * nrb, nz);
     DFE_LAUNCH_CHECK();
   }
diff --git a/unsupervised_depth_opticalflow_egomotion_amd/csrc/ops_epilogue.hip b/unsupervised_depth_opticalflow_egomotion_amd/csrc/ops_epilogue.hip
--- a/unsupervised_depth_opticalflow_egomotion_amd/csrc/ops_epilogue.hip
+++ b/unsupervised_depth_opticalflow_egomotion_amd/csrc/ops_epilogue.hip
@@ -1,5 +1,6 @@
 #include "dfe_internal.h"
 #include "dfe_device.h"
+#include "dfe_finish.h"
 #include <hip/hip_runtime.h>
 
 namespace dfe {
@@ -73,18 +74,7 @@
 
 __global__ void __launch_bounds__(64) k_bias_grad_final(const float* __restrict__ part, float* __restrict__ gbias,
                                                         int B, int C, int nchunk) {
-  const int c = blockIdx.x, lane = threadIdx.x;
-  float s = 0.0f;
-  for (int b = 0; b < B; ++b) {
-    const float* p = part + (static_cast<long>(b) * C + c) * nchunk;
-    for (int k = lane; k < nchunk; k += 64) s += p[k];
-  }
-  s = dpp_add<0xB1>(s); s = dpp_add<0x4E>(s); s = dpp_add<0x141>(s); s = dpp_add<0x140>(s);
-  const float r0 = __int_as_float(__builtin_amdgcn_readlane(__float_as_int(s), 0));
-  const float r1 = __int_as_float(__builtin_amdgcn_readlane(__float_as_int(s), 16));
-  const float r2 = __int_as_float(__builtin_amdgcn_readlane(__float_as_int(s), 32));
-  const float r3 = __int_as_float(__builtin_amdgcn_readlane(__float_as_int(s), 48));
-  if (lane == 0) gbias[c] = (r0 + r1) + (r2 + r3);
+  bias_final_wave(part, gbias, B, C, nchunk, blockIdx.x, threadIdx.x);
 }
 
 constexpr int EP_MAXL = 8;
@@ -93,18 +83,7 @@
 __global__ void __launch_bounds__(64) k_bias_grad_final_multi(BiasFinalJobs j, int B) {
   int l = 0;
   while (l + 1 < j.n && static_cast<int>(blockIdx.x) >= j.first[l + 1]) ++l;
-  const int c = blockIdx.x - j.first[l], lane = threadIdx.x, C = j.C[l], nchunk = j.nchunk[l];
-  float s = 0.0f;
-  for (int b = 0; b < B; ++b) {
-    const float* p = j.part[l] + (static_cast<long>(b) * C + c) * nchunk;
-    for (int k = lane; k < nchunk; k += 64) s += p[k];
-  }
-  s = dpp_add<0xB1>(s); s = dpp_add<0x4E>(s); s = dpp_add<0x141>(s); s = dpp_add<0x140>(s);
-  const float r0 = __int_as_float(__builtin_amdgcn_readlane(__float_as_int(s), 0));
-  const float r1 = __int_as_float(__builtin_amdgcn_readlane(__float_as_int(s), 16));
-  const float r2 = __int_as_float(__builtin_amdgcn_readlane(__float_as_int(s), 32));
-  const float r3 = __int_as_float(__builtin_amdgcn_readlane(__float_as_int(s), 48));
-  if (lane == 0) j.gbias[l][c] = (r0 + r1) + (r2 + r3);
+  bias_final_wave(j.part[l], j.gbias[l], B, j.C[l], j.nchunk[l], blockIdx.x - j.first[l], threadIdx.x);
 }
 
 template <bool VEC>
@@ -222,6 +201,9 @@
   else k_bias_act_bwd<false><<<g, EP_BLOCK, 0, st>>>(y, gy, gz, part, static_cast<int>(hw), hw, gy_batch_stride, C, slope);
   DFE_LAUNCH_CHECK();
   if (gbias) {
+    bool deferred = false;
+    const int qrc = finish_defer(FinishJob{partials, gbias, nullptr, 0, FIN_BIAS, B, C, nchunk}, st, &deferred);
+    if (qrc != DFE_OK || deferred) return qrc;
     k_bias_grad_final<<<C, 64, 0, st>>>(partials, gbias, B, C, nchunk);
     DFE_LAUNCH_CHECK();
   }
@@ -261,6 +243,9 @@
   else k_bias_act_bwd2<false><<<g, EP_BLOCK, 0, st>>>(y, y_batch_stride, g1, g1_batch_stride, g2, g2_batch_stride, gz, part, C, static_cast<int>(hw), slope);
   DFE_LAUNCH_CHECK();
   if (gbias) {
+    bool deferred = false;
+    const int qrc = finish_defer(FinishJob{partials, gbias, nullptr, 0, FIN_BIAS, B, C, nchunk}, st, &deferred);
+    if (qrc != DFE_OK || deferred) return qrc;
     k_bias_grad_final<<<C, 64, 0, st>>>(partials, gbias, B, C, nchunk);
     DFE_LAUNCH_CHECK();
   }
@@ -281,6 +266,15 @@
     j.nchunk[l] = static_cast<int>((hw + EP_CHUNK - 1) / EP_CHUNK);
     j.first[l + 1] = j.first[l] + C[l];
   }
+  int queued = 0;
+  for (; queued < n; ++queued) {
+    bool deferred = false;
+    const int qrc = finish_defer(FinishJob{j.part[queued], j.gbias[queued], nullptr, 0, FIN_BIAS, B, j.C[queued], j.nchunk[queued]},
+                                 static_cast<hipStream_t>(stream), &deferred);
+    if (qrc != DFE_OK) return qrc;
+    if (!deferred) break;
+  }
+  if (queued == n) return DFE_OK;
   k_bias_grad_final_multi<<<j.first[n], 64, 0, static_cast<hipStream_t>(stream)>>>(j, B);
   DFE_LAUNCH_CHECK();
   return DFE_OK;
diff --git a/unsupervised_depth_opticalflow_egomotion_amd/csrc/ops_finish.hip b/unsupervised_depth_opticalflow_egomotion_amd/csrc/ops_finish.hip
--- /dev/null
+++ b/unsupervised_depth_opticalflow_egomotion_amd/csrc/ops_finish.hip
@@ -0,0 +1,234 @@
+#include "dfe_internal.h"
+#include "dfe_finish.h"
+#include <hip/hip_runtime.h>
+#include <atomic>
+#include <mutex>
+#include <unordered_map>
+#include <vector>
+
+namespace dfe {
+
+constexpr int FQ_MAXJ = 64;
+struct FinishTable { FinishJob job[FQ_MAXJ]; int first[FQ_MAXJ + 1]; int n; };
+
+__device__ __forceinline__ int finish_find(const FinishTable& t, int block) {
+  int lo = 0, hi = t.n - 1;
+  while (lo < hi) {
+    const int mid = (lo + hi + 1) >> 1;
+    if (block >= t.first[mid]) lo = mid; else hi = mid - 1;
+  }
+  return lo;
+}
+
+__global__ void __launch_bounds__(256) k_finish_multi256(const FinishTable t) {
+  __shared__ float sm[8][32];
+  const int l = finish_find(t, blockIdx.x);
+  const int block = blockIdx.x - t.first[l];
+  const float* part = t.job[l].part;
+  float* out = t.job[l].out;
+  const long n = t.job[l].n;
+  const int i0 = t.job[l].i0;
+  if (t.job[l].kind == FIN_SUM8) {
+    wgrad_sum_block<8>(part, out, i0, n, block, sm);
+  } else {
+    const int idx = block * 256 + threadIdx.x;
+    if (idx < n) out[idx] = planeconv_slot_sum(part, static_cast<int>(n), i0, idx);
+  }
+}
+
+__global__ void __launch_bounds__(1024) k_finish_multi1024(const FinishTable t) {
+  __shared__ float sm[WF_LANES * 17];
+  const int l = finish_find(t, blockIdx.x);
+  const int block = blockIdx.x - t.first[l];
+  const float* part = t.job[l].part;
+  float* out = t.job[l].out;
+  const long n = t.job[l].n;
+  const int i0 = t.job[l].i0;
+  if (t.job[l].kind == FIN_SUM32) wgrad_sum_block<32>(part, out, i0, n, block, reinterpret_cast<float(*)[32]>(sm));
+  else wgrad_final_block(part, out, static_cast<int>(n), i0, t.job[l].i1, block, reinterpret_cast<float(*)[17]>(sm));
+}
+
+__global__ void __launch_bounds__(64) k_finish_multi_wave(const FinishTable t) {
+  const int l = finish_find(t, blockIdx.x);
+  const int o = blockIdx.x - t.first[l], lane = threadIdx.x;
+  const float* part = t.job[l].part;
+  float* out = t.job[l].out;
+  const int kind = t.job[l].kind, i0 = t.job[l].i0, i1 = t.job[l].i1, i2 = t.job[l].i2;
+  if (kind == FIN_BIAS) bias_final_wave(part, out, i0, i1, i2, o, lane);
+  else if (kind == FIN_HEAD1) head_final_wave<1, DH_CI>(part, out, t.job[l].out2, i0, i1, i2, o, lane);
+  else head_final_wave<2, FH_CI>(part, out, t.job[l].out2, i0, i1, i2, o, lane);
+}
+
+namespace {
+
+struct StreamQueue {
+  std::vector<FinishJob> jobs;
+  long bytes = 0;
+  long generation = 0;
+  hipEvent_t done = nullptr;
+};
+
+std::mutex g_mu;
+std::unordered_map<hipStream_t, StreamQueue> g_queues;
+std::atomic<int> g_deferred{0};
+long g_threshold = 0;
+long g_launches = 0;
+
+inline int job_family(const FinishJob& j) { return j.kind <= FIN_PLANE ? 0 : j.kind <= FIN_WFINAL ? 1 : 2; }
+
+long job_blocks(const FinishJob& j) {
+  switch (j.kind) {
+    case FIN_SUM8: case FIN_SUM32: return (j.n + 31) / 32;
+    case FIN_PLANE: return (j.n + 255) / 256;
+    case FIN_WFINAL: return (j.n + 15) / 16;
+    case FIN_BIAS: return j.i1;
+    case FIN_HEAD1: return static_cast<long>(j.i0) * 9 + 1;
+    default: return 2L * j.i0 * 9 + 2;
+  }
+}
+
+long job_bytes(const FinishJob& j) {
+  long floats;
+  switch (j.kind) {
+    case FIN_SUM8: case FIN_SUM32: case FIN_PLANE: case FIN_WFINAL: floats = j.i0 * j.n; break;
+    case FIN_BIAS: floats = static_cast<long>(j.i0) * j.i1 * j.i2; break;
+    case FIN_HEAD1: floats = static_cast<long>(j.i1) * j.i2 * (DH_CI * 9 + 1); break;
+    default: floats = static_cast<long>(j.i1) * j.i2 * (FH_CI * 2 * 9 + 2); break;
+  }
+  return 4 * floats;
+}
+
+int launch_table(int family, const FinishTable& t, hipStream_t st) {
+  const unsigned blocks = static_cast<unsigned>(t.first[t.n]);
+  if (family == 0) k_finish_multi256<<<blocks, 256, 0, st>>>(t);
+  else if (family == 1) k_finish_multi1024<<<blocks, 1024, 0, st>>>(t);
+  else k_finish_multi_wave<<<blocks, 64, 0, st>>>(t);
+  ++g_launches;
+  return hipGetLastError() == hipSuccess ? DFE_OK : DFE_ERR_LAUNCH;
+}
+
+int flush_locked(hipStream_t st, StreamQueue& q, bool sums_only = false) {
+  int rc = DFE_OK;
+  for (int family = 0; family < (sums_only ? 2 : 3) && rc == DFE_OK; ++family) {
+    FinishTable t;
+    t.n = 0; t.first[0] = 0;
+    for (const FinishJob& j : q.jobs) {
+      if (job_family(j) != family) continue;
+      const long nb = job_blocks(j);
+      if (t.n == FQ_MAXJ || t.first[t.n] + nb >= (1L << 30)) {
+        rc = launch_table(family, t, st);
+        if (rc != DFE_OK) break;
+        t.n = 0;
+      }
+      t.job[t.n] = j;
+      t.first[t.n + 1] = t.first[t.n] + static_cast<int>(nb);
+      ++t.n;
+    }
+    if (rc == DFE_OK && t.n > 0) rc = launch_table(family, t, st);
+  }
+  if (sums_only && rc == DFE_OK) {
+    size_t kept = 0;
+    for (const FinishJob& j : q.jobs)
+      if (job_family(j) == 2) q.jobs[kept++] = j;
+    q.jobs.resize(kept);
+  } else {
+    q.jobs.clear();
+  }
+  q.bytes = 0;
+  return rc;
+}
+
+}
+
+int finish_defer(const FinishJob& job, hipStream_t st, bool* taken) {
+  *taken = false;
+  if (!g_deferred.load(std::memory_order_relaxed)) return DFE_OK;
+  const long nb = job_blocks(job);
+  if (!job.part || (!job.out && !job.out2)) return DFE_ERR_NULL;
+  if (nb <= 0 || nb >= (1L << 30)) return DFE_ERR_DIMS;
+  std::lock_guard<std::mutex> lock(g_mu);
+  StreamQueue& q = g_queues[st];
+  q.jobs.push_back(job);
+  *taken = true;
+  if (job_family(job) == 2) return DFE_OK;
+  q.bytes += job_bytes(job);
+  if (g_threshold > 0 && q.bytes >= g_threshold) {
+    ++q.generation;
+    return flush_locked(st, q, true);
+  }
+  return DFE_OK;
+}
+
+int finish_wgrad_sum(const float* ws, float* gw, int S, long n, hipStream_t st) {
+  const bool wide = wgrad_sum_wide(S);
+  bool deferred = false;
+  const int rc = finish_defer(FinishJob{ws, gw, nullptr, n, wide ? FIN_SUM32 : FIN_SUM8, S, 0, 0}, st, &deferred);
+  if (rc != DFE_OK || deferred) return rc;
+  if (wide) k_wgrad_sum<32><<<static_cast<unsigned>((n + 31) / 32), 1024, 0, st>>>(ws, gw, S, n);
+  else k_wgrad_sum<8><<<static_cast<unsigned>((n + 31) / 32), 256, 0, st>>>(ws, gw, S, n);
+  return hipGetLastError() == hipSuccess ? DFE_OK : DFE_ERR_LAUNCH;
+}
+
+}
+
+using namespace dfe;
+
+extern "C" int dfe_finish_set_deferred(int on) {
+  g_deferred.store(on ? 1 : 0, std::memory_order_relaxed);
+  return DFE_OK;
+}
+
+extern "C" int dfe_finish_deferred(void) { return g_deferred.load(std::memory_order_relaxed); }
+
+extern "C" int dfe_finish_set_threshold(long bytes) {
+  if (bytes < 0) return DFE_ERR_DIMS;
+  std::lock_guard<std::mutex> lock(g_mu);
+  g_threshold = bytes;
+  return DFE_OK;
+}
+
+extern "C" long dfe_finish_pending(void* stream) {
+  std::lock_guard<std::mutex> lock(g_mu);
+  const auto it = g_queues.find(static_cast<hipStream_t>(stream));
+  return it == g_queues.end() ? 0 : static_cast<long>(it->second.jobs.size());
+}
+
+extern "C" long dfe_finish_generation(void* stream) {
+  std::lock_guard<std::mutex> lock(g_mu);
+  const auto it = g_queues.find(static_cast<hipStream_t>(stream));
+  return it == g_queues.end() ? 0 : it->second.generation;
+}
+
+extern "C" long dfe_finish_pending_total(void) {
+  std::lock_guard<std::mutex> lock(g_mu);
+  long n = 0;
+  for (const auto& kv : g_queues) n += static_cast<long>(kv.second.jobs.size());
+  return n;
+}
+
+extern "C" long dfe_finish_launches(void) {
+  std::lock_guard<std::mutex> lock(g_mu);
+  return g_launches;
+}
+
+extern "C" int dfe_finish_flush(void* stream) {
+  std::lock_guard<std::mutex> lock(g_mu);
+  const auto it = g_queues.find(static_cast<hipStream_t>(stream));
+  if (it == g_queues.end() || it->second.jobs.empty()) return DFE_OK;
+  return flush_locked(it->first, it->second);
+}
+
+extern "C" int dfe_finish_flush_all(void* wait_stream) {
+  hipStream_t waiter = static_cast<hipStream_t>(wait_stream);
+  std::lock_guard<std::mutex> lock(g_mu);
+  for (auto& kv : g_queues) {
+    StreamQueue& q = kv.second;
+    if (q.jobs.empty()) continue;
+    const int rc = flush_locked(kv.first, q);
+    if (rc != DFE_OK) return rc;
+    if (kv.first == waiter) continue;
+    if (!q.done && hipEventCreateWithFlags(&q.done, hipEventDisableTiming) != hipSuccess) return DFE_ERR_LAUNCH;
+    if (hipEventRecord(q.done, kv.first) != hipSuccess || hipStreamWaitEvent(waiter, q.done, 0) != hipSuccess) return DFE_ERR_LAUNCH;
+  }
+  return DFE_OK;
+}
diff --git a/unsupervised_depth_opticalflow_egomotion_amd/csrc/ops_planeconv.hip b/unsupervised_depth_opticalflow_egomotion_amd/csrc/ops_planeconv.hip
--- a/unsupervised_depth_opticalflow_egomotion_amd/csrc/ops_planeconv.hip
+++ b/unsupervised_depth_opticalflow_egomotion_amd/csrc/ops_planeconv.hip
@@ -1,4 +1,5 @@
 #include "dfe_internal.h"
+#include "dfe_finish.h"
 #include <hip/hip_runtime.h>
 #include <algorithm>
 #include <cstdlib>
@@ -131,9 +132,7 @@
                                                           float inv_hw) {
   const int idx = blockIdx.x * 256 + threadIdx.x;
   if (idx >= total) return;
-  float s = part[idx];
-#pragma unroll 4
-  for (int k = 1; k < KS; ++k) s += part[static_cast<long>(k) * total + idx];
+  float s = planeconv_slot_sum(part, total, KS, idx);
   int b = fdiv(idx, inv_nhw);
   int r = idx - b * NHW;
   if (bias) s += bias[fdiv(r, inv_hw)];
@@ -411,6 +410,9 @@
                                               1.0f / static_cast<float>(W + 2));
   DFE_LAUNCH_CHECK();
   const int total = Co * Ci * 9;
+  bool deferred = false;
+  const int qrc = finish_defer(FinishJob{ws, gweight, nullptr, total, FIN_PLANE, static_cast<int>(g.units), 0, 0}, st, &deferred);
+  if (qrc != DFE_OK || deferred) return qrc;
   k_planeconv_finish<<<(total + 255) / 256, 256, 0, st>>>(ws, nullptr, gweight, 0, nullptr, 0, total, total, total,
                                                           static_cast<int>(g.units), 1.0f, 1.0f / static_cast<float>(total),
                                                           1.0f / static_cast<float>(total));
diff --git a/unsupervised_depth_opticalflow_egomotion_amd/csrc/ops_sconv.hip b/unsupervised_depth_opticalflow_egomotion_amd/csrc/ops_sconv.hip
--- a/unsupervised_depth_opticalflow_egomotion_amd/csrc/ops_sconv.hip
+++ b/unsupervised_depth_opticalflow_egomotion_amd/csrc/ops_sconv.hip
@@ -1,6 +1,6 @@
 #include "dfe_internal.h"
 #include "dfe_device.h"
-#include "dfe_wgrad_sum.h"
+#include "dfe_finish.h"
 #include <hip/hip_runtime.h>
 #include <algorithm>
 #include <cstdlib>
@@ -345,8 +345,5 @@
   }
   DFE_LAUNCH_CHECK();
   const long n = static_cast<long>(Co) * Ci * K * K;
-  if (ns > 64) k_wgrad_sum<32><<<static_cast<unsigned>((n + 31) / 32), 1024, 0, st>>>(ws, gweight, ns, n);
-  else k_wgrad_sum<8><<<static_cast<unsigned>((n + 31) / 32), 256, 0, st>>>(ws, gweight, ns, n);
-  DFE_LAUNCH_CHECK();
-  return DFE_OK;
-}
+  return finish_wgrad_sum(ws, gweight, ns, n, st);
+}
diff --git a/unsupervised_depth_opticalflow_egomotion_amd/csrc/ops_wgrad.hip b/unsupervised_depth_opticalflow_egomotion_amd/csrc/ops_wgrad.hip
--- a/unsupervised_depth_opticalflow_egomotion_amd/csrc/ops_wgrad.hip
+++ b/unsupervised_depth_opticalflow_egomotion_amd/csrc/ops_wgrad.hip
@@ -1,4 +1,5 @@
 #include "dfe_internal.h"
+#include "dfe_finish.h"
 #include <hip/hip_runtime.h>
 
 namespace dfe {
@@ -93,30 +94,10 @@
           po[(static_cast<long>(k) * Co + co0 + 16 * o + 4 * kq + r) * Ci + ci0 + 16 * t + m] = acc[o][t][k][r];
 }
 
-constexpr int WF_LANES = 64;
 __global__ void __launch_bounds__(16 * WF_LANES) k_wgrad_final(const float* __restrict__ part, float* __restrict__ gw, int n,
                                                                int nunits, int coci) {
   __shared__ float sm[WF_LANES][17];
-  const int ii = threadIdx.x & 15, ul = threadIdx.x >> 4;
-  const int i = blockIdx.x * 16 + ii;
-  float s0 = 0.0f, s1 = 0.0f, s2 = 0.0f, s3 = 0.0f;
-  if (i < n) {
-    const float* q = part + i;
-    int u = ul;
-    for (; u + 3 * WF_LANES < nunits; u += 4 * WF_LANES) {
-      s0 += q[static_cast<long>(u) * n]; s1 += q[static_cast<long>(u + WF_LANES) * n];
-      s2 += q[static_cast<long>(u + 2 * WF_LANES) * n]; s3 += q[static_cast<long>(u + 3 * WF_LANES) * n];
-    }
-    for (; u < nunits; u += WF_LANES) s0 += q[static_cast<long>(u) * n];
-  }
-  sm[ul][ii] = (s0 + s1) + (s2 + s3);
-  __syncthreads();
-  if (ul == 0 && i < n) {
-    float t = 0.0f;
-    for (int k = 0; k < WF_LANES; ++k) t += sm[k][ii];
-    const int tap = i / coci, cc = i - tap * coci;
-    gw[static_cast<long>(cc) * 9 + tap] = t;
-  }
+  wgrad_final_block(part, gw, n, nunits, coci, blockIdx.x, sm);
 }
 
 }
@@ -173,6 +154,9 @@
   else k_wgrad3x3_thin<1, 1><<<grid, 64, 0, st>>>(p, gy, partials, Ci, Co, H, W, sp.R, sp.nrg, sp.nseg);
   DFE_LAUNCH_CHECK();
   const int n = Co * Ci * 9;
+  bool deferred = false;
+  const int qrc = finish_defer(FinishJob{partials, gweight, nullptr, n, FIN_WFINAL, static_cast<int>(sp.units), Co * Ci, 0}, st, &deferred);
+  if (qrc != DFE_OK || deferred) return qrc;
   k_wgrad_final<<<(n + 15) / 16, 16 * WF_LANES, 0, st>>>(partials, gweight, n, static_cast<int>(sp.units), Co * Ci);
   DFE_LAUNCH_CHECK();
   return DFE_OK;
diff --git a/unsupervised_depth_opticalflow_egomotion_amd/csrc/ops_wino_wgrad.hip b/unsupervised_depth_opticalflow_egomotion_amd/csrc/ops_wino_wgrad.hip
--- a/unsupervised_depth_opticalflow_egomotion_amd/csrc/ops_wino_wgrad.hip
+++ b/unsupervised_depth_opticalflow_egomotion_amd/csrc/ops_wino_wgrad.hip
@@ -1,6 +1,6 @@
 #include "dfe_internal.h"
 #include "dfe_device.h"
-#include "dfe_wgrad_sum.h"
+#include "dfe_finish.h"
 #include <hip/hip_runtime.h>
 #include <algorithm>
 #include <cstdlib>
@@ -318,8 +318,5 @@
 #undef WG_GO
   DFE_LAUNCH_CHECK();
   const long n = static_cast<long>(Co) * Ci * 9;
-  if (p.S > 64) k_wgrad_sum<32><<<static_cast<unsigned>((n + 31) / 32), 1024, 0, st>>>(ws, gweight, p.S, n);
-  else k_wgrad_sum<8><<<static_cast<unsigned>((n + 31) / 32), 256, 0, st>>>(ws, gweight, p.S, n);
-  DFE_LAUNCH_CHECK();
-  return DFE_OK;
-}
+  return finish_wgrad_sum(ws, gweight, p.S, n, st);
+}
diff --git a/unsupervised_depth_opticalflow_egomotion_amd/ddp.py b/unsupervised_depth_opticalflow_egomotion_amd/ddp.py
--- a/unsupervised_depth_opticalflow_egomotion_amd/ddp.py
+++ b/unsupervised_depth_opticalflow_egomotion_amd/ddp.py
@@ -159,6 +159,8 @@
         self._ready.add(k)
         g = self._params[self._members[k][0]].grad
         if g.is_cuda:
+            from . import finish_queue
+            finish_queue.flush_current()
             ev = torch.cuda.Event()
             ev.record()
             self._events[k] = ev
@@ -195,6 +197,8 @@
 
     @torch.no_grad()
     def reduce_gradients(self):
+        from . import finish_queue
+        finish_queue.flush_pending()
         if self.overlap and self._order is None:
             self._agree()
             armed_now = self._order is not None
diff --git a/unsupervised_depth_opticalflow_egomotion_amd/finish_queue.py b/unsupervised_depth_opticalflow_egomotion_amd/finish_queue.py
--- /dev/null
+++ b/unsupervised_depth_opticalflow_egomotion_amd/finish_queue.py
@@ -0,0 +1,135 @@
+import contextlib
+import os
+import threading
+
+import torch
+
+from ._lib import check, get_lib, raw_stream, stream_ptr
+
+DEFAULT_POLICY = "0"
+
+
+def _parse(policy):
+    policy = str(policy).strip().lower()
+    if policy in ("0", "off", "immediate"):
+        return None
+    if policy == "end":
+        return 0
+    return int(float(policy) * (1 << 20))
+
+
+THRESHOLD = _parse(os.environ.get("DFE_FINISH_DEFER", DEFAULT_POLICY))
+
+_lock = threading.Lock()
+_held = {}
+_depth = 0
+_active = False
+_callback_queued = False
+_record = None
+
+
+def set_policy(policy):
+    global THRESHOLD
+    THRESHOLD = _parse(policy)
+
+
+def record_outputs(on=True):
+    global _record
+    old = _record
+    _record = [] if on else None
+    return old
+
+
+def recorded_outputs():
+    return list(_record or [])
+
+
+@contextlib.contextmanager
+def deferred():
+    global _depth, _active, _callback_queued
+    if THRESHOLD is None:
+        yield
+        return
+    lib = get_lib()
+    with _lock:
+        _depth += 1
+        if _depth == 1:
+            check(lib.dfe_finish_set_threshold(THRESHOLD), "dfe_finish_set_threshold")
+            check(lib.dfe_finish_set_deferred(1), "dfe_finish_set_deferred")
+            _active = True
+            _callback_queued = False
+    try:
+        yield
+    finally:
+        with _lock:
+            _depth -= 1
+            last = _depth == 0
+            if last:
+                _active = False
+                check(lib.dfe_finish_set_deferred(0), "dfe_finish_set_deferred")
+        if last:
+            flush_pending()
+
+
+def hold(part, *outs, split_sum=False):
+    global _callback_queued
+    if not _active:
+        return
+    st = raw_stream()
+    generation = get_lib().dfe_finish_generation(st) if split_sum else 0
+    with _lock:
+        if _record is not None:
+            _record.extend(o.data_ptr() for o in outs if o is not None)
+        entry = _held.get(st)
+        if entry is None:
+            entry = _held[st] = [generation, [], []]
+        if split_sum and generation != entry[0]:
+            entry[0] = generation
+            entry[1].clear()
+        else:
+            lst = entry[1 if split_sum else 2]
+            lst.append(part)
+            lst.extend(o.detach() for o in outs if o is not None)
+        if _callback_queued:
+            return
+        try:
+            torch.autograd.Variable._execution_engine.queue_callback(_end_of_backward)
+            _callback_queued = True
+        except RuntimeError:
+            pass
+
+
+def _end_of_backward():
+    global _callback_queued
+    with _lock:
+        _callback_queued = False
+    flush_pending()
+
+
+def flush_current():
+    st = raw_stream()
+    check(get_lib().dfe_finish_flush(st), "dfe_finish_flush")
+    with _lock:
+        entry = _held.get(st)
+        if entry:
+            entry[1].clear()
+            entry[2].clear()
+
+
+def flush_pending():
+    lib = get_lib()
+    if lib.dfe_finish_pending_total() > 0:
+        check(lib.dfe_finish_flush_all(stream_ptr()), "dfe_finish_flush_all")
+    with _lock:
+        for entry in _held.values():
+            entry[1].clear()
+            entry[2].clear()
+
+
+def pending(stream=None):
+    lib = get_lib()
+    return int(lib.dfe_finish_pending_total() if stream is None else lib.dfe_finish_pending(stream))
+
+
+def launches():
+    return int(get_lib().dfe_finish_launches())
diff --git a/unsupervised_depth_opticalflow_egomotion_amd/ops.py b/unsupervised_depth_opticalflow_egomotion_amd/ops.py
--- a/unsupervised_depth_opticalflow_egomotion_amd/ops.py
+++ b/unsupervised_depth_opticalflow_egomotion_amd/ops.py
@@ -6,7 +6,7 @@
 
 import torch
 
-from . import _lib, convs
+from . import _lib, convs, finish_queue
 from ._lib import DfeError, check, f32c, get_lib, ptr, stream_ptr
 
 _ALIGN_CORNERS = False
@@ -577,6 +577,8 @@
             part = torch.empty(lib.dfe_glue_partials_floats(B, C, H, W), device=gout.device)
         check(lib.dfe_elu_pad_bwd(ptr(x) if ctx.apply_elu else None, ptr(bias) if ctx.has_bias else None, ptr(gout), ptr(gx),
                                   ptr(gb), ptr(part), B, C, H, W, ctx.apply_elu, stream_ptr()), "dfe_elu_pad_bwd")
+        if gb is not None:
+            finish_queue.hold(part, gb)
         return gx, gb, None
 
 
@@ -619,6 +621,8 @@
             part = torch.empty(lib.dfe_glue_partials_floats(B, C1, h, w), device=x.device)
         check(lib.dfe_elu_up2_cat_pad_bwd(ptr(x), ptr(bias) if ctx.has_bias else None, ptr(gout), ptr(gx), ptr(gskip), ptr(gb),
                                           ptr(part), B, C1, C2, h, w, stream_ptr()), "dfe_elu_up2_cat_pad_bwd")
+        if gb is not None:
+            finish_queue.hold(part, gb)
         return gx, gb, gskip
 
 
@@ -662,6 +666,8 @@
             part = torch.empty(lib.dfe_bias_act_partials_floats(B, C, H, W), device=y.device, dtype=torch.float32)
         check(lib.dfe_bias_act_bwd(ptr(y), ptr(gy, strided=True), gy.stride(0), ptr(gz), ptr(gb), ptr(part), B, C, H, W, ctx.slope,
                                    stream_ptr()), "dfe_bias_act_bwd")
+        if gb is not None:
+            finish_queue.hold(part, gb)
         return gz, gb, None
 
 
@@ -718,6 +724,7 @@
     if want_w:
         gw = torch.empty_like(w)
         check(lib.dfe_planeconv_wgrad(ptr(gy), ptr(x), ptr(gw), ptr(ws), B, Ci, Co, H, W, stream_ptr()), "dfe_planeconv_wgrad")
+        finish_queue.hold(ws, gw, split_sum=True)
     return gx, gw
 
 
@@ -896,6 +903,8 @@
             part = torch.empty(lib.dfe_bias_act_partials_floats(B, C, H, W), device=y.device, dtype=torch.float32)
         check(lib.dfe_bias_act_bwd(ptr(y), ptr(gy, strided=True), gy.stride(0), ptr(gz), ptr(gb), ptr(part), B, C, H, W, slope,
                                    stream_ptr()), "dfe_bias_act_bwd")
+        if gb is not None:
+            finish_queue.hold(part, gb)
         pad = (d, d) if d > 1 else (P, P)
         gx, gw, _ = convs.raw_backward(gz, x, w, (1, 1), pad, (d, d), ctx.needs_input_grad[0], ctx.needs_input_grad[1])
         return gx, gw, gb, None, None, None
@@ -936,6 +945,7 @@
     ws = torch.empty(n, device=x.device, dtype=torch.float32)
     check(lib.dfe_wino_wgrad3x3(ptr(x, strided=True), x.stride(0), ptr(gy, strided=True), gy.stride(0), ptr(gw), ptr(ws), B, Ci, Co, H, W, P,
                                 stream_ptr()), "dfe_wino_wgrad3x3")
+    finish_queue.hold(ws, gw, split_sum=True)
     return gw
 
 
@@ -963,6 +973,7 @@
     ws = torch.empty(n, device=x.device, dtype=torch.float32)
     check(lib.dfe_sconv_wgrad(ptr(x, strided=True), x.stride(0), ptr(gy, strided=True), gy.stride(0), ptr(gw), ptr(ws), B, Ci, Co, H, W, k, s, P,
                               stream_ptr()), "dfe_sconv_wgrad")
+    finish_queue.hold(ws, gw, split_sum=True)
     return gw
 
 
@@ -990,6 +1001,8 @@
             part = torch.empty(lib.dfe_bias_act_partials_floats(B, C, H, W), device=y.device, dtype=torch.float32)
         check(lib.dfe_bias_act_bwd(ptr(y), ptr(gy), gy.stride(0), ptr(gz), ptr(gb), ptr(part), B, C, H, W, ctx.slope,
                                    stream_ptr()), "dfe_bias_act_bwd")
+        if gb is not None:
+            finish_queue.hold(part, gb)
         gx, gw = planeconv_backward(gz, x, w, ctx.needs_input_grad[0], ctx.needs_input_grad[1])
         return gx, gw, gb, None
 
@@ -1026,6 +1039,8 @@
             part = torch.empty(lib.dfe_bias_act_partials_floats(B, Co, H, W), device=y.device, dtype=torch.float32)
         check(lib.dfe_bias_act_bwd(ptr(y), ptr(gy), gy.stride(0), ptr(gz), ptr(gb), ptr(part), B, Co, H, W, ctx.slope,
                                    stream_ptr()), "dfe_bias_act_bwd")
+        if gb is not None:
+            finish_queue.hold(part, gb)
         gx = torch.empty_like(x) if ctx.needs_input_grad[0] else None
         gw = torch.empty_like(w) if ctx.needs_input_grad[1] else None
         check(lib.dfe_conv1x1_small_bwd(ptr(gz), ptr(x), ptr(w), ptr(gx), ptr(gw), B, Ci, Co, H, W, stream_ptr()),
@@ -1159,6 +1174,8 @@
             outs = (ctypes.c_void_p * n)(*[t[1].data_ptr() for t in pending])
             chans = (ctypes.c_int * n)(*[t[2] for t in pending])
             check(lib.dfe_bias_grad_final_multi(parts, outs, chans, n, B, H, W, st), "dfe_bias_grad_final_multi")
+            for part, gb, _ in pending:
+                finish_queue.hold(part, gb)
         gx, gw[0], _ = cb(gz, x, w[0], bool(need[1]), nw(0))
         out = [None, gx]
         for k in range(6):
@@ -1258,6 +1275,8 @@
         part = torch.empty(lib.dfe_disp_head_partials_floats(B, C, H, W), device=p.device)
         check(lib.dfe_disp_head_bwd(ptr(p), ptr(weight), ptr(out), ptr(gout), ptr(gp), ptr(gw), ptr(gb), ptr(part), B, C, H, W,
                                     stream_ptr()), "dfe_disp_head_bwd")
+        if gw is not None or gb is not None:
+            finish_queue.hold(part, gw, gb)
         return gp, gw, gb
 
 
@@ -1282,6 +1301,8 @@
     part = torch.empty(lib.dfe_flow_head_partials_floats(B, C, H, W), device=x.device, dtype=torch.float32)
     check(lib.dfe_flow_head_bwd(ptr(x), ptr(weight), ptr(gout), ptr(gx), ptr(gw), ptr(gb), ptr(part), B, C, H, W,
                                 stream_ptr()), "dfe_flow_head_bwd")
+    if gw is not None or gb is not None:
+        finish_queue.hold(part, gw, gb)
     return gx, gw, gb
 
 
@@ -1330,6 +1351,7 @@
                 gw = torch.empty_like(weight)
                 part = torch.empty(lib.dfe_wgrad3x3_partials_floats(B, Ci, Co, H, W), device=p.device)
                 check(lib.dfe_wgrad3x3_fwd(ptr(p), ptr(gy), ptr(gw), ptr(part), B, Ci, Co, H, W, stream_ptr()), "dfe_wgrad3x3_fwd")
+                finish_queue.hold(part, gw, split_sum=True)
         return gp, gw
 
 
diff --git a/unsupervised_depth_opticalflow_egomotion_amd/optim.py b/unsupervised_depth_opticalflow_egomotion_amd/optim.py
--- a/unsupervised_depth_opticalflow_egomotion_amd/optim.py
+++ b/unsupervised_depth_opticalflow_egomotion_amd/optim.py
@@ -74,6 +74,8 @@
             with torch.enable_grad():
                 loss = closure()
         lib = get_lib()
+        from . import finish_queue
+        finish_queue.flush_pending()
         for gi, group in enumerate(self.param_groups):
             if group.get("weight_decay", 0) or group.get("amsgrad") or group.get("maximize"):
                 raise NotImplementedError("FusedAdam implements the reference's plain Adam (no weight decay / amsgrad / maximize)")
diff --git a/unsupervised_depth_opticalflow_egomotion_amd/train_step.py b/unsupervised_depth_opticalflow_egomotion_amd/train_step.py
--- a/unsupervised_depth_opticalflow_egomotion_amd/train_step.py
+++ b/unsupervised_depth_opticalflow_egomotion_amd/train_step.py
@@ -62,14 +62,14 @@
 
 
 def train_step(model, optimizer, inputs, cfg, profiler=None):
-    from . import profiling
+    from . import finish_queue, profiling
     optimizer.zero_grad(set_to_none=True)
     with profiling.range("forward"):
         loss_pack, mask_pack = model(inputs)
         loss = total_loss(loss_pack, cfg)
     if profiler is not None:
         profiler.report_process("forward")
-    with profiling.range("backward"):
+    with profiling.range("backward"), finish_queue.deferred():
         loss.backward()
     if profiler is not None:
         profiler.report_process("backward")
```
